# lucidrains/vit-pytorch

Hardware: AMD Instinct MI355X
Metric: images/sec (fwd+bwd) ViT-B/16 224^2 bf16 (higher is better)
Workload: dtype bf16

## Files before the change

### vit_pytorch_amd/csrc/gemm_bf16.hip

```cpp
#include "common.h"
#include <atomic>
#include "gemm_nt_plan.h"
#include <stdlib.h>

namespace {

constexpr int BM = 128, BN = 128;
constexpr int NT_BK = 32;
constexpr int NT_TILE_BYTES = 128 * NT_BK * 2;
constexpr int NT_STAGE_BYTES = 2 * NT_TILE_BYTES;
constexpr int NXCD = 8;

__device__ __forceinline__ int xcd_swizzle(int b, int nwg) {
    const int q = nwg / NXCD, r = nwg % NXCD;
    const int xcd = b % NXCD, idx = b / NXCD;
    return (xcd < r ? xcd * (q + 1) : r * (q + 1) + (xcd - r) * q) + idx;
}

__device__ __forceinline__ void grouped_tile(int wg, int tiles_m, int tiles_n, int gn, int& tm, int& tn) {
    const int per_group = gn * tiles_m;
    const int g = wg / per_group;
    const int r = wg - g * per_group;
    const int rem = tiles_n - g * gn;
    const int w = rem < gn ? rem : gn;
    tm = r / w;
    tn = g * gn + (r - tm * w);
}

__device__ __forceinline__ int swz_f(int x) { return (0x1320 >> (4 * (x & 3))) & 3; }

template <int EPI>
__global__ __launch_bounds__(256) void gemm_nt_kernel(
    const __bf16* __restrict__ A, long long lda, const __bf16* __restrict__ W, long long ldw,
    void* __restrict__ Cv, long long ldc, int M, int N, int K,
    const __bf16* __restrict__ bias, const float* __restrict__ resid, __bf16* __restrict__ aux,
    int tiles_n, int nwg) {
    __shared__ __attribute__((aligned(16))) char lds[2 * NT_STAGE_BYTES];

    const int tid = threadIdx.x;
    const int lane = tid & 63;
    const int wave = tid >> 6;
    const int wm = wave >> 1, wn = wave & 1;
    const int wg = xcd_swizzle(blockIdx.x, nwg);
    const int tm = wg / tiles_n, tn = wg % tiles_n;
    const int m0 = tm * BM, n0 = tn * BN;

    const int srow = lane >> 2;
    const int spos = lane & 3;
    const int schunk = spos ^ swz_f(lane >> 4);
    const __bf16* a_src[2];
    const __bf16* w_src[2];
#pragma unroll
    for (int j = 0; j < 2; ++j) {
        const int rg = wave * 2 + j;
        int ar = m0 + rg * 16 + srow; ar = ar < M ? ar : M - 1;
        int wr = n0 + rg * 16 + srow; wr = wr < N ? wr : N - 1;
        a_src[j] = A + (long long)ar * lda + schunk * 8;
        w_src[j] = W + (long long)wr * ldw + schunk * 8;
    }
    auto stage = [&](int buf, int kt) {
        char* base = lds + buf * NT_STAGE_BYTES;
#pragma unroll
        for (int j = 0; j < 2; ++j) {
            const int rg = wave * 2 + j;
            __builtin_amdgcn_global_load_lds((const void __attribute__((address_space(1)))*)(a_src[j] + kt * NT_BK),
                                             (void __attribute__((address_space(3)))*)(base + rg * 1024), 16, 0, 0);
            __builtin_amdgcn_global_load_lds((const void __attribute__((address_space(1)))*)(w_src[j] + kt * NT_BK),
                                             (void __attribute__((address_space(3)))*)(base + NT_TILE_BYTES + rg * 1024), 16, 0, 0);
        }
    };

    const int fi = lane & 15, fg = lane >> 4;
    const int fpos = fg ^ swz_f(fi >> 2);
    const int a_off = (wm * 64 + fi) * 64 + fpos * 16;
    const int w_off = NT_TILE_BYTES + (wn * 64 + fi) * 64 + fpos * 16;

    f32x4 acc[4][4];
#pragma unroll
    for (int i = 0; i < 4; ++i)
#pragma unroll
        for (int j = 0; j < 4; ++j) acc[i][j] = f32x4{0.f, 0.f, 0.f, 0.f};

    const int nt = K / NT_BK;
    stage(0, 0);
    for (int t = 0; t < nt; ++t) {
        __syncthreads();
        if (t + 1 < nt) stage((t + 1) & 1, t + 1);
        const char* base = lds + (t & 1) * NT_STAGE_BYTES;
        bf16x8 xf[4], wf[4];
#pragma unroll
        for (int f = 0; f < 4; ++f) {
            xf[f] = *reinterpret_cast<const bf16x8*>(base + a_off + f * 1024);
            wf[f] = *reinterpret_cast<const bf16x8*>(base + w_off + f * 1024);
        }
#pragma unroll
        for (int fn = 0; fn < 4; ++fn)
#pragma unroll
            for (int fm = 0; fm < 4; ++fm)
                acc[fn][fm] = __builtin_amdgcn_mfma_f32_16x16x32_bf16(wf[fn], xf[fm], acc[fn][fm], 0, 0, 0);
    }

#pragma unroll
    for (int fm = 0; fm < 4; ++fm) {
        const int m = m0 + wm * 64 + fm * 16 + fi;
        if (m >= M) continue;
#pragma unroll
        for (int fn = 0; fn < 4; ++fn) {
            const int n = n0 + wn * 64 + fn * 16 + 4 * fg;
            if (n >= N) continue;
            f32x4 v = acc[fn][fm];
            const long long o = (long long)m * ldc + n;
            if constexpr (EPI == VITK_EPI_BIAS || EPI == VITK_EPI_BIAS_GELU) {
                v += load4<__bf16>(bias + n);
            }
            if constexpr (EPI == VITK_EPI_NONE || EPI == VITK_EPI_BIAS) {
                store4<__bf16>(reinterpret_cast<__bf16*>(Cv) + o, v);
            } else if constexpr (EPI == VITK_EPI_BIAS_GELU) {
                store4<__bf16>(aux + o, v);
                f32x4 gq;
#pragma unroll
                for (int e = 0; e < 4; ++e) gq[e] = gelu_erf(v[e]);
                store4<__bf16>(reinterpret_cast<__bf16*>(Cv) + o, gq);
            } else if constexpr (EPI == VITK_EPI_RESID) {
                if (bias) v += load4<__bf16>(bias + n);
                v += *reinterpret_cast<const f32x4*>(resid + o);
                *reinterpret_cast<f32x4*>(reinterpret_cast<float*>(Cv) + o) = v;
            } else if constexpr (EPI == VITK_EPI_GELU_BWD) {
                const f32x4 h = load4<__bf16>(aux + o);
#pragma unroll
                for (int e = 0; e < 4; ++e) v[e] *= gelu_erf_grad(h[e]);
                store4<__bf16>(reinterpret_cast<__bf16*>(Cv) + o, v);
            }
        }
    }
}

constexpr int TN_BKM = 32;
constexpr int TN_LD = 288;
constexpr int TN_TILE_BYTES = TN_BKM * TN_LD;
constexpr int TN_STAGE_BYTES = 2 * TN_TILE_BYTES;

__device__ __forceinline__ bf16x8 tr_frag(const char* tile, int off) {
    const s16x4 lo = __builtin_amdgcn_ds_read_tr16_b64_v4i16((s16x4 __attribute__((address_space(3)))*)(tile + off));
    const s16x4 hi = __builtin_amdgcn_ds_read_tr16_b64_v4i16((s16x4 __attribute__((address_space(3)))*)(tile + off + 16 * TN_LD));
    const s16x8 v = {lo[0], lo[1], lo[2], lo[3], hi[0], hi[1], hi[2], hi[3]};
    return __builtin_bit_cast(bf16x8, v);
}

__global__ __launch_bounds__(256) void gemm_tn_kernel(
    const __bf16* __restrict__ dY, long long ldy, const __bf16* __restrict__ X, long long ldx,
    float* __restrict__ ws, int M, int N, int K, int rows_per_split, int tiles_k, int nwg) {
    __shared__ __attribute__((aligned(16))) char lds[2 * TN_STAGE_BYTES];
    const int tid = threadIdx.x;
    const int lane = tid & 63;
    const int wave = tid >> 6;
    const int wn = wave >> 1, wk = wave & 1;
    const int lin = xcd_swizzle(blockIdx.x, (int)gridDim.x);
    const int split = lin / nwg;
    const int wg = lin % nwg;
    const int tn = wg / tiles_k, tk = wg % tiles_k;
    const int n0 = tn * BN, k0 = tk * BM;
    const int mbeg = split * rows_per_split;
    int mend = mbeg + rows_per_split; mend = mend < M ? mend : M;

    int srow[2], scol[2];
#pragma unroll
    for (int j = 0; j < 2; ++j) { const int c = tid + 256 * j; srow[j] = c >> 4; scol[j] = (c & 15) * 8; }
    const bf16x8 zero8 = {0, 0, 0, 0, 0, 0, 0, 0};
    bf16x8 ry[2], rx[2];
    auto gload = [&](int mb) {
#pragma unroll
        for (int j = 0; j < 2; ++j) {
            const int m = mb + srow[j];
            const bool mv = m < mend;
            ry[j] = (mv && n0 + scol[j] < N) ? *reinterpret_cast<const bf16x8*>(dY + (long long)m * ldy + n0 + scol[j]) : zero8;
            rx[j] = (mv && k0 + scol[j] < K) ? *reinterpret_cast<const bf16x8*>(X + (long long)m * ldx + k0 + scol[j]) : zero8;
        }
    };
    auto lstore = [&](int buf) {
        char* base = lds + buf * TN_STAGE_BYTES;
#pragma unroll
        for (int j = 0; j < 2; ++j) {
            *reinterpret_cast<bf16x8*>(base + srow[j] * TN_LD + scol[j] * 2) = ry[j];
            *reinterpret_cast<bf16x8*>(base + TN_TILE_BYTES + srow[j] * TN_LD + scol[j] * 2) = rx[j];
        }
    };

    const int fi = lane & 15, fg = lane >> 4;
    const int tr_off = (4 * fg + (fi >> 2)) * TN_LD + (fi & 3) * 8;
    const int y_off = tr_off + wn * 128;
    const int x_off = TN_TILE_BYTES + tr_off + wk * 128;

    f32x4 acc[4][4];
#pragma unroll
    for (int i = 0; i < 4; ++i)
#pragma unroll
        for (int j = 0; j < 4; ++j) acc[i][j] = f32x4{0.f, 0.f, 0.f, 0.f};

    const int nsteps = (mend - mbeg + TN_BKM - 1) / TN_BKM;
    if (nsteps > 0) {
        gload(mbeg);
        lstore(0);
        __syncthreads();
        for (int t = 0; t < nsteps; ++t) {
            if (t + 1 < nsteps) gload(mbeg + (t + 1) * TN_BKM);
            const char* base = lds + (t & 1) * TN_STAGE_BYTES;
            bf16x8 yf[4], xf[4];
#pragma unroll
            for (int f = 0; f < 4; ++f) {
                yf[f] = tr_frag(base, y_off + f * 32);
                xf[f] = tr_frag(base, x_off + f * 32);
            }
#pragma unroll
            for (int fn = 0; fn < 4; ++fn)
#pragma unroll
                for (int fk = 0; fk < 4; ++fk)
                    acc[fn][fk] = __builtin_amdgcn_mfma_f32_16x16x32_bf16(yf[fn], xf[fk], acc[fn][fk], 0, 0, 0);
            if (t + 1 < nsteps) lstore((t + 1) & 1);
            __syncthreads();
        }
    }
    float* out = ws + (long long)split * N * K;
#pragma unroll
    for (int fn = 0; fn < 4; ++fn)
#pragma unroll
        for (int r = 0; r < 4; ++r) {
            const int n = n0 + wn * 64 + fn * 16 + 4 * fg + r;
            if (n >= N) continue;
#pragma unroll
            for (int fk = 0; fk < 4; ++fk) {
                const int k = k0 + wk * 64 + fk * 16 + fi;
                if (k < K) out[(long long)n * K + k] = acc[fn][fk][r];
            }
        }
}

template <typename OT>
__global__ __launch_bounds__(256) void tn_reduce_kernel(const float* __restrict__ ws, int splits, long long NK, int K,
                                                         OT* __restrict__ out, long long ldo, int accumulate, long long slab_stride) {
    const long long i4 = ((long long)blockIdx.x * 256 + threadIdx.x) * 4;
    if (i4 >= NK) return;
    f32x4 s = *reinterpret_cast<const f32x4*>(ws + i4);
    for (int p = 1; p < splits; ++p) s += *reinterpret_cast<const f32x4*>(ws + (long long)p * slab_stride + i4);
    const long long n = i4 / K, k = i4 % K;
    OT* o = out + n * ldo + k;
    if (accumulate) s += load4<OT>(o);
    store4<OT>(o, s);
}


constexpr int L_BN = 256, L_BK = 64;

constexpr int P_BK = 32, P_STAGES = 4;
constexpr int P_TILE_BYTES = 256 * P_BK * 2;
constexpr int P_STAGE_BYTES = 2 * P_TILE_BYTES;
constexpr int P_LDS_BYTES = P_STAGES * P_STAGE_BYTES;

#define PP_BARRIER() do { __builtin_amdgcn_sched_barrier(0); __builtin_amdgcn_s_barrier(); __builtin_amdgcn_sched_barrier(0); } while (0)

template <int EPI, int FM, int EB = 2, int F8 = 0>
__global__ __launch_bounds__(512) void gemm_nt256pp_kernel(
    const void* __restrict__ Av, long long lda, const void* __restrict__ Wv, long long ldw,
    void* __restrict__ Cv, long long ldc, int M, int N, int K,
    const __bf16* __restrict__ bias, const float* __restrict__ resid, __bf16* __restrict__ aux,
    int tiles_n, int nwg, int group_n, float* __restrict__ csum, float alpha, unsigned drop_t, unsigned drop_seed, float inv_keep,
    const float* __restrict__ alpha_a, const float* __restrict__ alpha_w, F8Out f8) {
    const char* A = reinterpret_cast<const char*>(Av);
    const char* W = reinterpret_cast<const char*>(Wv);
    extern __shared__ __attribute__((aligned(16))) char lds[];
    const int tid = threadIdx.x;
    const int lane = tid & 63;
    const int wave = __builtin_amdgcn_readfirstlane(tid >> 6);
    const int wm = wave >> 2, wn = wave & 3;
    const bool grp_b = wave >= 4;
    const int wg = xcd_swizzle(blockIdx.x, nwg);
    int tm, tn;
    grouped_tile(wg, nwg / tiles_n, tiles_n, group_n, tm, tn);
    constexpr int WROWS = 16 * FM;
    const int m0 = tm * (2 * WROWS), n0 = tn * L_BN;

    const int srow = lane >> 2, spos = lane & 3;
    const int schunk = spos ^ swz_f(lane >> 4);
    const char* a_src[2];
    const char* w_src[2];
#pragma unroll
    for (int j = 0; j < 2; ++j) {
        int ar = m0 + (wave * 2 + j) * 16 + srow; ar = ar < M ? ar : M - 1;
        int wr = n0 + (wave * 2 + j) * 16 + srow; wr = wr < N ? wr : N - 1;
        a_src[j] = A + (long long)ar * lda * EB + schunk * 16;
        w_src[j] = W + (long long)wr * ldw * EB + schunk * 16;
    }
    auto stage_a = [&](int kt) {
        char* base = lds + (kt & 3) * P_STAGE_BYTES + wave * 2048;
#pragma unroll
        for (int j = 0; j < 2; ++j)
            __builtin_amdgcn_global_load_lds((const void __attribute__((address_space(1)))*)(a_src[j] + kt * 64),
                                             (void __attribute__((address_space(3)))*)(base + j * 1024), 16, 0, 0);
    };
    auto stage_w = [&](int kt) {
        char* base = lds + (kt & 3) * P_STAGE_BYTES + P_TILE_BYTES + wave * 2048;
#pragma unroll
        for (int j = 0; j < 2; ++j)
            __builtin_amdgcn_global_load_lds((const void __attribute__((address_space(1)))*)(w_src[j] + kt * 64),
                                             (void __attribute__((address_space(3)))*)(base + j * 1024), 16, 0, 0);
    };
    auto mma = [&](const bf16x8& wfr, const bf16x8& xfr, f32x4 c) -> f32x4 {
        if constexpr (EB == 2) {
            return __builtin_amdgcn_mfma_f32_16x16x32_bf16(wfr, xfr, c, 0, 0, 0);
        } else {
            typedef long l2 __attribute__((ext_vector_type(2)));
            const l2 w2 = __builtin_bit_cast(l2, wfr), x2 = __builtin_bit_cast(l2, xfr);
            if constexpr (F8 & 1) {
                c = __builtin_amdgcn_mfma_f32_16x16x32_fp8_bf8(w2[0], x2[0], c, 0, 0, 0);
                return __builtin_amdgcn_mfma_f32_16x16x32_fp8_bf8(w2[1], x2[1], c, 0, 0, 0);
            } else {
                c = __builtin_amdgcn_mfma_f32_16x16x32_fp8_fp8(w2[0], x2[0], c, 0, 0, 0);
                return __builtin_amdgcn_mfma_f32_16x16x32_fp8_fp8(w2[1], x2[1], c, 0, 0, 0);
            }
        }
    };
    auto mma128 = [&](const bf16x8& w0, const bf16x8& w1, const bf16x8& x0, const bf16x8& x1, f32x4 c) -> f32x4 {
        typedef int i4 __attribute__((ext_vector_type(4)));
        typedef int i8 __attribute__((ext_vector_type(8)));
        const i8 a = __builtin_shufflevector(__builtin_bit_cast(i4, w0), __builtin_bit_cast(i4, w1), 0, 1, 2, 3, 4, 5, 6, 7);
        const i8 b = __builtin_shufflevector(__builtin_bit_cast(i4, x0), __builtin_bit_cast(i4, x1), 0, 1, 2, 3, 4, 5, 6, 7);
        return __builtin_amdgcn_mfma_scale_f32_16x16x128_f8f6f4(a, b, c, 0 , (F8 & 1) ? 1 : 0 , 0, 0, 0, 0);
    };
    static_assert(F8 == 0 || EB == 1, "the e5m2 / K = 128 flavours are fp8 flavours");

    const int fi = lane & 15, fg = lane >> 4;
    const int fpos = fg ^ swz_f(fi >> 2);
    const int a_off = (wm * WROWS + fi) * 64 + fpos * 16;
    const int w_off = P_TILE_BYTES + (wn * 64 + fi) * 64 + fpos * 16;

    f32x4 acc[4][FM];
#pragma unroll
    for (int i = 0; i < 4; ++i)
#pragma unroll
        for (int j = 0; j < FM; ++j) acc[i][j] = f32x4{0.f, 0.f, 0.f, 0.f};

    const int nt = K * EB / 64;
    stage_a(0); stage_w(0);
    if (nt > 1) { stage_a(1); stage_w(1); }
    if (nt > 2) { stage_a(2); stage_w(2); }
    if (nt > 2) asm volatile("s_waitcnt vmcnt(8)" ::: "memory");
    else if (nt > 1) asm volatile("s_waitcnt vmcnt(4)" ::: "memory");
    else asm volatile("s_waitcnt vmcnt(0)" ::: "memory");
    PP_BARRIER();
    if (grp_b) PP_BARRIER();

    if constexpr ((F8 & 2) != 0) {
        bf16x8 hw[4], hx[FM];
        for (int j = 0; j < nt; ++j) {
            const char* base = lds + (j & 3) * P_STAGE_BYTES;
            const bool more = j + 3 < nt;
            const bool odd = (j & 1) != 0;
            bf16x8 wf[4], xf[4];
#pragma unroll
            for (int f = 0; f < 4; ++f) wf[f] = *reinterpret_cast<const bf16x8*>(base + w_off + f * 1024);
#pragma unroll
            for (int f = 0; f < 4; ++f) xf[f] = *reinterpret_cast<const bf16x8*>(base + a_off + f * 1024);
            if (more) stage_a(j + 3);
            asm volatile("s_waitcnt lgkmcnt(0)" ::: "memory");
            PP_BARRIER();
            if (odd) {
                __builtin_amdgcn_s_setprio(1);
#pragma unroll
                for (int fn = 0; fn < 4; ++fn)
#pragma unroll
                    for (int f = 0; f < 4; ++f)
                        acc[fn][f] = mma128(hw[fn], wf[fn], hx[f], xf[f], acc[fn][f]);
                __builtin_amdgcn_s_setprio(0);
            } else {
#pragma unroll
                for (int f = 0; f < 4; ++f) { hw[f] = wf[f]; hx[f] = xf[f]; }
            }
            PP_BARRIER();
#pragma unroll
            for (int f = 0; f < FM - 4; ++f) xf[f] = *reinterpret_cast<const bf16x8*>(base + a_off + (4 + f) * 1024);
            if (more) stage_w(j + 3);
            if (more) asm volatile("s_waitcnt vmcnt(8)" ::: "memory");
            else if (j + 2 < nt) asm volatile("s_waitcnt vmcnt(4)" ::: "memory");
            else asm volatile("s_waitcnt vmcnt(0)" ::: "memory");
            asm volatile("s_waitcnt lgkmcnt(0)" ::: "memory");
            PP_BARRIER();
            if (odd) {
                __builtin_amdgcn_s_setprio(1);
#pragma unroll
                for (int fn = 0; fn < 4; ++fn)
#pragma unroll
                    for (int f = 0; f < FM - 4; ++f)
                        acc[fn][4 + f] = mma128(hw[fn], wf[fn], hx[4 + f], xf[f], acc[fn][4 + f]);
                __builtin_amdgcn_s_setprio(0);
            } else {
#pragma unroll
                for (int f = 0; f < FM - 4; ++f) hx[4 + f] = xf[f];
            }
            PP_BARRIER();
        }
    } else
    for (int j = 0; j < nt; ++j) {
        const char* base = lds + (j & 3) * P_STAGE_BYTES;
        const bool more = j + 3 < nt;
        bf16x8 wf[4], xf[4];
#pragma unroll
        for (int f = 0; f < 4; ++f) wf[f] = *reinterpret_cast<const bf16x8*>(base + w_off + f * 1024);
#pragma unroll
        for (int f = 0; f < 4; ++f) xf[f] = *reinterpret_cast<const bf16x8*>(base + a_off + f * 1024);
        if (more) stage_a(j + 3);
        asm volatile("s_waitcnt lgkmcnt(0)" ::: "memory");
        PP_BARRIER();
        __builtin_amdgcn_s_setprio(1);
#pragma unroll
        for (int fn = 0; fn < 4; ++fn)
#pragma unroll
            for (int f = 0; f < 4; ++f)
                acc[fn][f] = mma(wf[fn], xf[f], acc[fn][f]);
        __builtin_amdgcn_s_setprio(0);
        PP_BARRIER();
#pragma unroll
        for (int f = 0; f < FM - 4; ++f) xf[f] = *reinterpret_cast<const bf16x8*>(base + a_off + (4 + f) * 1024);
        if (more) stage_w(j + 3);
        if (more) asm volatile("s_waitcnt vmcnt(8)" ::: "memory");
        else if (j + 2 < nt) asm volatile("s_waitcnt vmcnt(4)" ::: "memory");
        else asm volatile("s_waitcnt vmcnt(0)" ::: "memory");
        asm volatile("s_waitcnt lgkmcnt(0)" ::: "memory");
        PP_BARRIER();
        __builtin_amdgcn_s_setprio(1);
#pragma unroll
        for (int fn = 0; fn < 4; ++fn)
#pragma unroll
            for (int f = 0; f < FM - 4; ++f)
                acc[fn][4 + f] = mma(wf[fn], xf[f], acc[fn][4 + f]);
        __builtin_amdgcn_s_setprio(0);
        PP_BARRIER();
    }
    if (!grp_b) PP_BARRIER();
    if constexpr (EB == 1) {
        const float al = alpha * (alpha_a ? *alpha_a : 1.0f) * (alpha_w ? *alpha_w : 1.0f);
#pragma unroll
        for (int i = 0; i < 4; ++i)
#pragma unroll
            for (int jj = 0; jj < FM; ++jj) acc[i][jj] *= al;
    }

    __syncthreads();
    char* ep = lds + wave * 16384;
    const int mrow0 = m0 + wm * WROWS, ncol0 = n0 + wn * 64;
    if constexpr (EPI == VITK_EPI_RESID) {
        const int rr = lane >> 4, rc = lane & 15;
        const int ncol = ncol0 + rc * 4;
        f32x4 b4 = {0.f, 0.f, 0.f, 0.f};
        if (bias && ncol < N) b4 = load4<__bf16>(bias + ncol);
        constexpr int NF0 = 4, NF1 = FM - 4;
        f32x4 rpre[2][16];
        auto fetch_resid = [&](int hh) {
            const int nf = hh ? NF1 : NF0;
#pragma unroll
            for (int j = 0; j < 16; ++j) {
                const int m = mrow0 + hh * 64 + j * 4 + rr;
                rpre[hh][j] = f32x4{0.f, 0.f, 0.f, 0.f};
                if (j < nf * 4 && m < M && ncol < N) rpre[hh][j] = *reinterpret_cast<const f32x4*>(resid + (long long)m * ldc + ncol);
            }
        };
        fetch_resid(0);
#pragma unroll
        for (int hh = 0; hh < 2; ++hh) {
            const int nf = hh ? NF1 : NF0;
#pragma unroll
            for (int f4 = 0; f4 < 4; ++f4) {
                if (f4 < nf) {
                    const int row = f4 * 16 + fi;
#pragma unroll
                    for (int fn = 0; fn < 4; ++fn) {
                        const int c16 = fn * 4 + fg;
                        *reinterpret_cast<f32x4*>(ep + row * 256 + ((c16 ^ (row & 15)) * 16)) = acc[fn][hh * 4 + f4 < FM ? hh * 4 + f4 : 0];
                    }
                }
            }
            if (hh == 0) fetch_resid(1);
#pragma unroll
            for (int j = 0; j < 16; ++j) {
                if (j < nf * 4) {
                    const int row = j * 4 + rr;
                    f32x4 v = *reinterpret_cast<const f32x4*>(ep + row * 256 + ((rc ^ (row & 15)) * 16));
                    const int m = mrow0 + hh * 64 + row;
                    if (m < M && ncol < N) {
                        v += b4;
                        if (drop_t) {
                            const unsigned hrow = drop_row((unsigned)m, drop_seed);
#pragma unroll
                            for (int e = 0; e < 4; ++e) v[e] = drop_keep(hrow, (unsigned)(ncol + e), drop_t) ? v[e] * inv_keep : 0.f;
                        }
                        v += rpre[hh][j];
                        *reinterpret_cast<f32x4*>(reinterpret_cast<float*>(Cv) + (long long)m * ldc + ncol) = v;
                    }
                }
            }
        }
    } else {
        f32x4 b4[4];
#pragma unroll
        for (int fn = 0; fn < 4; ++fn) {
            b4[fn] = f32x4{0.f, 0.f, 0.f, 0.f};
            if constexpr (EPI == VITK_EPI_BIAS || EPI == VITK_EPI_BIAS_GELU) {
                const int n = ncol0 + fn * 16 + 4 * fg;
                if (n < N) b4[fn] = load4<__bf16>(bias + n);
            }
        }
        const int rr = lane >> 3, rc = lane & 7;
        const int ncol = ncol0 + rc * 8;
        bf16x8 hpre[2 * FM];
        if constexpr (EPI == VITK_EPI_GELU_BWD) {
#pragma unroll
            for (int j = 0; j < 2 * FM; ++j) {
                const int m = mrow0 + j * 8 + rr;
                hpre[j] = bf16x8{0, 0, 0, 0, 0, 0, 0, 0};
                if (m < M && ncol < N) hpre[j] = *reinterpret_cast<const bf16x8*>(aux + (long long)m * ldc + ncol);
            }
        }
#pragma unroll
        for (int fm = 0; fm < FM; ++fm) {
            const int row = fm * 16 + fi;
#pragma unroll
            for (int fn = 0; fn < 4; ++fn) {
                const int c16 = fn * 2 + (fg >> 1);
                const f32x4 v = acc[fn][fm] + b4[fn];
                const bf16x4 pk = {(__bf16)v[0], (__bf16)v[1], (__bf16)v[2], (__bf16)v[3]};
                *reinterpret_cast<bf16x4*>(ep + row * 128 + ((c16 ^ (row & 7)) * 16) + (((fg & 1) ^ ((row >> 3) & 1)) * 8)) = pk;
            }
        }
        float cs[8] = {0.f, 0.f, 0.f, 0.f, 0.f, 0.f, 0.f, 0.f};
        float f8max = 0.f;
#pragma unroll
        for (int j = 0; j < 2 * FM; ++j) {
            const int row = j * 8 + rr;
            bf16x8 v = *reinterpret_cast<const bf16x8*>(ep + row * 128 + ((rc ^ (row & 7)) * 16));
            if (j & 1) v = bf16x8{v[4], v[5], v[6], v[7], v[0], v[1], v[2], v[3]};
            const int m = mrow0 + row;
            if (m < M && ncol < N) {
                const long long o = (long long)m * ldc + ncol;
                if constexpr (EPI == VITK_EPI_NONE || EPI == VITK_EPI_BIAS) {
                    *reinterpret_cast<bf16x8*>(reinterpret_cast<__bf16*>(Cv) + o) = v;
                } else if constexpr (EPI == VITK_EPI_BIAS_GELU) {
                    *reinterpret_cast<bf16x8*>(aux + o) = v;
                    bf16x8 g8;
#pragma unroll
                    for (int e = 0; e < 8; e += 2) {
                        const f32x2 g2 = gelu_fast2(f32x2{(float)v[e], (float)v[e + 1]});
                        g8[e] = (__bf16)g2[0]; g8[e + 1] = (__bf16)g2[1];
                    }
                    if (drop_t) {
                        const unsigned hrow = drop_row((unsigned)m, drop_seed);
#pragma unroll
                        for (int e = 0; e < 8; ++e)
                            g8[e] = drop_keep(hrow, (unsigned)(ncol + e), drop_t) ? (__bf16)((float)g8[e] * inv_keep) : (__bf16)0.f;
                    }
                    if (Cv) *reinterpret_cast<bf16x8*>(reinterpret_cast<__bf16*>(Cv) + o) = g8;
                    if (f8.p || f8.amax) {
                        const f32x4 lo = {(float)g8[0], (float)g8[1], (float)g8[2], (float)g8[3]};
                        const f32x4 hi = {(float)g8[4], (float)g8[5], (float)g8[6], (float)g8[7]};
                        if (f8.p) {
                            const float sc8 = *f8.scale;
                            unsigned* d8 = reinterpret_cast<unsigned*>(f8.p + o);
                            d8[0] = pack_fp8x4(lo, sc8); d8[1] = pack_fp8x4(hi, sc8);
                        }
                        if (f8.amax) f8max = fmaxf(f8max, fmaxf(absmax4(lo), absmax4(hi)));
                    }
                } else if constexpr (EPI == VITK_EPI_GELU_BWD) {
                    const bf16x8 h8 = hpre[j];
                    bf16x8 g8;
                    float km[8];
                    if (drop_t) {
                        const unsigned hrow = drop_row((unsigned)m, drop_seed);
#pragma unroll
                        for (int e = 0; e < 8; ++e) km[e] = drop_keep(hrow, (unsigned)(ncol + e), drop_t) ? inv_keep : 0.f;
                    } else {
#pragma unroll
                        for (int e = 0; e < 8; ++e) km[e] = 1.f;
                    }
#pragma unroll
                    for (int e = 0; e < 8; e += 2) {
                        const f32x2 g2 = f32x2{(float)v[e], (float)v[e + 1]} * gelu_grad_fast2(f32x2{(float)h8[e], (float)h8[e + 1]}) * f32x2{km[e], km[e + 1]};
                        g8[e] = (__bf16)g2[0]; g8[e + 1] = (__bf16)g2[1];
                        cs[e] += (float)g8[e]; cs[e + 1] += (float)g8[e + 1];
                    }
                    *reinterpret_cast<bf16x8*>(reinterpret_cast<__bf16*>(Cv) + o) = g8;
                    if (f8.p || f8.amax) {
                        const f32x4 lo = {(float)g8[0], (float)g8[1], (float)g8[2], (float)g8[3]};
                        const f32x4 hi = {(float)g8[4], (float)g8[5], (float)g8[6], (float)g8[7]};
                        if (f8.p) {
                            const float sc8 = *f8.scale;
                            unsigned* d8 = reinterpret_cast<unsigned*>(f8.p + o);
                            d8[0] = pack_bf8x4(lo, sc8); d8[1] = pack_bf8x4(hi, sc8);
                        }
                        if (f8.amax) f8max = fmaxf(f8max, fmaxf(absmax4(lo), absmax4(hi)));
                    }
                }
            }
        }
        if constexpr (EPI == VITK_EPI_BIAS_GELU || EPI == VITK_EPI_GELU_BWD) {
            if (f8.amax) {
                f8max = wave_max(f8max);
                __syncthreads();
                float* red = reinterpret_cast<float*>(lds);
                if (lane == 0) red[wave] = f8max;
                __syncthreads();
                if (tid == 0) {
                    float m = red[0];
#pragma unroll
                    for (int k = 1; k < 8; ++k) m = fmaxf(m, red[k]);
                    atomicMax(f8.amax + (blockIdx.x & 63), __builtin_bit_cast(unsigned, m));
                }
            }
        }
        if constexpr (EPI == VITK_EPI_GELU_BWD) {
            if (csum) {
                float* cp = reinterpret_cast<float*>(ep);
#pragma unroll
                for (int e = 0; e < 8; ++e) cp[rr * 64 + rc * 8 + e] = cs[e];
                float t = 0.f;
#pragma unroll
                for (int r8 = 0; r8 < 8; ++r8) t += cp[r8 * 64 + lane];
                const int n = ncol0 + lane;
                if (n < N) csum[(long long)(tm * 2 + wm) * N + n] = t;
            }
        }
    }
}

template <typename Kern>
int set_max_lds(Kern kernel, int bytes) {
    return (int)hipFuncSetAttribute(reinterpret_cast<const void*>(kernel), hipFuncAttributeMaxDynamicSharedMemorySize, bytes);
}

}

namespace {
struct NtPlan { bool large; int fm; };
NtPlan nt_plan(int64_t M, int64_t N, int64_t K, int64_t ldc, const void* aux) {
    NtPlan pl;
    pl.large = (K % L_BK == 0) && M >= 1024 && N >= 256 && (N % 8 == 0) && (ldc % 8 == 0) && (!aux || aligned16(aux));
    pl.fm = 8;
    if (pl.large) {
        const long long tn_ = (N + L_BN - 1) / L_BN;
        const long long t8 = ((M + 255) / 256) * tn_, t7 = ((M + 223) / 224) * tn_;
        const long long cost8 = ((t8 + 255) / 256) * 8, cost7 = ((t7 + 255) / 256) * 7;
        if (cost7 * 10 <= cost8 * 9) pl.fm = 7;
    }
    return pl;
}
int gemm_nt_impl(const void* A, int64_t lda, const void* W, int64_t ldw, void* C, int64_t ldc, int64_t M, int64_t N, int64_t K,
                 int epilogue, const void* bias, const float* resid, void* aux, float* csum, void* stream, bool fp8 = false,
                 float alpha = 1.0f, float drop_p = 0.f, unsigned drop_seed = 0u, const float* alpha_a = nullptr,
                 const float* alpha_w = nullptr, F8Out f8 = F8Out{nullptr, nullptr, nullptr}, int f8kind = 0);
}

extern "C" int vitk_gemm_nt_bf16(const void* A, int64_t lda, const void* W, int64_t ldw, void* C, int64_t ldc, int64_t M,
                                 int64_t N, int64_t K, int epilogue, const void* bias, const float* resid, void* aux,
                                 void* stream) {
    return gemm_nt_impl(A, lda, W, ldw, C, ldc, M, N, K, epilogue, bias, resid, aux, nullptr, stream);
}

extern "C" int vitk_gemm_nt_bf16_drop(const void* A, int64_t lda, const void* W, int64_t ldw, void* C, int64_t ldc, int64_t M, int64_t N,
                                      int64_t K, int epilogue, const void* bias, const float* resid, void* aux, float* colsum_partials,
                                      float drop_p, uint32_t drop_seed, void* stream) {
    if (colsum_partials && (epilogue != VITK_EPI_GELU_BWD || vitk_gemm_nt_colsum_rows(M, N, K, ldc) == 0))
        VITK_FAIL(VITK_E_SHAPE, "gemm_nt_bf16_drop: column sums come with the GELU_BWD epilogue of the 256-row kernel only");
    return gemm_nt_impl(A, lda, W, ldw, C, ldc, M, N, K, epilogue, bias, resid, aux, colsum_partials, stream, false, 1.0f, drop_p, drop_seed);
}

extern "C" int vitk_gemm_nt_fp8_ex(const void* A, int64_t lda, int a_is_fp8, const void* W, int64_t ldw, void* C, int64_t ldc, int64_t M,
                                   int64_t N, int64_t K, int epilogue, const void* bias, const float* resid, void* aux, float alpha,
                                   const float* alpha_a, const float* alpha_w, void* c8, const float* c8_scale, uint32_t* c8_amax64,
                                   void* stream) {
    const F8Out f8{(unsigned char*)c8, c8_scale, (unsigned*)c8_amax64};
    return gemm_nt_impl(A, lda, W, ldw, C, ldc, M, N, K, epilogue, bias, resid, aux, nullptr, stream, a_is_fp8 != 0, alpha, 0.f, 0u,
                        alpha_a, alpha_w, f8);
}

extern "C" int vitk_gemm_nt_fp8(const void* A, int64_t lda, const void* W, int64_t ldw, void* C, int64_t ldc, int64_t M, int64_t N,
                               int64_t K, int epilogue, const void* bias, const float* resid, void* aux, float alpha, void* stream) {
    return gemm_nt_impl(A, lda, W, ldw, C, ldc, M, N, K, epilogue, bias, resid, aux, nullptr, stream, true, alpha);
}

extern "C" int vitk_gemm_nt_fp8_v2(const void* A, int64_t lda, int a_kind, const void* W, int64_t ldw, void* C, int64_t ldc, int64_t M,
                                   int64_t N, int64_t K, int epilogue, const void* bias, const float* resid, void* aux,
                                   float* colsum_partials, float alpha, const float* alpha_a, const float* alpha_w, void* c8,
                                   const float* c8_scale, uint32_t* c8_amax64, int flags, void* stream) {
    if (a_kind < 0 || a_kind > 2) VITK_FAIL(VITK_E_ARG, "gemm_nt_fp8_v2: a_kind is 0 (16-bit), 1 (e4m3) or 2 (e5m2), got %d", a_kind);
    if (flags & ~1) VITK_FAIL(VITK_E_ARG, "gemm_nt_fp8_v2: unknown flags 0x%x", (unsigned)flags);
    if (a_kind == 0 && (flags & 1)) VITK_FAIL(VITK_E_ARG, "gemm_nt_fp8_v2: the K = 128 instruction takes 1-byte operands");
    if ((flags & 1) && (K % 128)) VITK_FAIL(VITK_E_SHAPE, "gemm_nt_fp8_v2: the K = 128 flavour needs K %% 128 == 0 (K = %lld)", (long long)K);
    if (colsum_partials && (epilogue != VITK_EPI_GELU_BWD || vitk_gemm_nt_fp8_colsum_rows(M, N, K, ldc) == 0))
        VITK_FAIL(VITK_E_SHAPE, "gemm_nt_fp8_v2: column sums come with the GELU_BWD epilogue of the 256-row kernel only");
    const F8Out f8{(unsigned char*)c8, c8_scale, (unsigned*)c8_amax64};
    return gemm_nt_impl(A, lda, W, ldw, C, ldc, M, N, K, epilogue, bias, resid, aux, colsum_partials, stream, a_kind != 0, alpha, 0.f, 0u,
                        alpha_a, alpha_w, f8, (a_kind == 2 ? 1 : 0) | ((flags & 1) ? 2 : 0));
}

extern "C" int64_t vitk_gemm_nt_fp8_colsum_rows(int64_t M, int64_t N, int64_t K, int64_t ldc) {
    if (M <= 0 || N <= 0 || K <= 0 || (K % 64)) return 0;
    const NtPlan pl = nt_plan(M, N, K, ldc, nullptr);
    if (!pl.large) return 0;
    return 2 * ((M + 32 * pl.fm - 1) / (32 * pl.fm));
}

static int64_t nt_persist_colsum_rows(const NtpPlan& q, int64_t M, int64_t N, int64_t K, int64_t ldc);
extern "C" int64_t vitk_gemm_nt_colsum_rows(int64_t M, int64_t N, int64_t K, int64_t ldc) {
    if (M <= 0 || N <= 0 || K <= 0) return 0;
    const NtpPlan q = ntp_plan(M, N, K, ldc, nullptr);
    if (q.ok) return nt_persist_colsum_rows(q, M, N, K, ldc);
    const NtPlan pl = nt_plan(M, N, K, ldc, nullptr);
    if (!pl.large) return 0;
    return 2 * ((M + 32 * pl.fm - 1) / (32 * pl.fm));
}

extern "C" int vitk_gemm_nt_plan(int64_t M, int64_t N, int64_t K, int64_t ldc, int32_t* out5) {
    if (!out5) VITK_FAIL(VITK_E_ARG, "gemm_nt_plan: null output");
    for (int i = 0; i < 5; ++i) out5[i] = 0;
    if (M <= 0 || N <= 0 || K <= 0) return 0;
    const NtpPlan q = ntp_plan(M, N, K, ldc, nullptr);
    if (q.ok) { out5[0] = 1; out5[1] = q.tm_main; out5[2] = q.tail_tm; out5[3] = q.grid; out5[4] = q.tiles_n; }
    return 0;
}

extern "C" int vitk_gemm_nt_bf16_gelu_bwd_colsum(const void* A, int64_t lda, const void* W, int64_t ldw, void* C, int64_t ldc,
                                                 int64_t M, int64_t N, int64_t K, void* aux, float* colsum_partials, void* stream) {
    if (!colsum_partials) VITK_FAIL(VITK_E_ARG, "gemm_nt_bf16_gelu_bwd_colsum: null partials");
    if (vitk_gemm_nt_colsum_rows(M, N, K, ldc) == 0 || (aux && !aligned16(aux)))
        VITK_FAIL(VITK_E_SHAPE, "gemm_nt_bf16_gelu_bwd_colsum: shape not served by the 256-row kernel (vitk_gemm_nt_colsum_rows() == 0)");
    return gemm_nt_impl(A, lda, W, ldw, C, ldc, M, N, K, VITK_EPI_GELU_BWD, nullptr, nullptr, aux, colsum_partials, stream);
}

extern "C" int vitk_gemm_nt_bf16_mul_aux_colsum(const void* A, int64_t lda, const void* W, int64_t ldw, void* C, int64_t ldc, int64_t M,
                                                int64_t N, int64_t K, const void* aux, float* colsum_partials, void* stream) {
    if (!aux) VITK_FAIL(VITK_E_ARG, "gemm_nt_bf16_mul_aux_colsum: null pointer");
    if (colsum_partials && vitk_gemm_nt_colsum_rows(M, N, K, ldc) == 0)
        VITK_FAIL(VITK_E_SHAPE, "gemm_nt_bf16_mul_aux_colsum: shape not served by the persistent kernel (vitk_gemm_nt_colsum_rows() == 0)");
    return gemm_nt_impl(A, lda, W, ldw, C, ldc, M, N, K, VITK_EPI_MUL_AUX, nullptr, nullptr, const_cast<void*>(aux), colsum_partials, stream);
}

extern "C" int vitk_gemm_nt_bf16_mul_aux8_colsum(const void* A, int64_t lda, const void* W, int64_t ldw, void* C, int64_t ldc, int64_t M,
                                                 int64_t N, int64_t K, const void* aux8, float* colsum_partials, void* stream) {
    if (!aux8) VITK_FAIL(VITK_E_ARG, "gemm_nt_bf16_mul_aux8_colsum: null pointer");
    if (colsum_partials && vitk_gemm_nt_colsum_rows(M, N, K, ldc) == 0)
        VITK_FAIL(VITK_E_SHAPE, "gemm_nt_bf16_mul_aux8_colsum: shape not served by the persistent kernel (vitk_gemm_nt_colsum_rows() == 0)");
    return gemm_nt_impl(A, lda, W, ldw, C, ldc, M, N, K, VITK_EPI_MUL_AUX8, nullptr, nullptr, const_cast<void*>(aux8), colsum_partials, stream);
}

constexpr unsigned NTW_EPIS = 0xffu;
static int ntw_tiles_m(const NtpPlan& q, int64_t M, int64_t N, int64_t K, int epilogue, int grid = 0) {
    if (epilogue == VITK_EPI_BIAS_GELU_DG8) epilogue = VITK_EPI_BIAS_GELU_DG;
    if (epilogue == VITK_EPI_MUL_AUX8) epilogue = VITK_EPI_MUL_AUX;
    const char* e = vitk_switch("VITK_NT_W128");
    const unsigned mask = e ? (unsigned)strtoul(e, nullptr, 0) : NTW_EPIS;
    if (!q.ok || !((mask >> epilogue) & 1u) || !gemm_ntw_serves(M, N, K)) return 0;
    return gemm_ntw_split(M, N, K, grid > 0 ? grid : q.grid);
}
static int64_t nt_persist_colsum_rows(const NtpPlan& q, int64_t M, int64_t N, int64_t K, int64_t ldc) {
    const int tmw = ntw_tiles_m(q, M, N, K, VITK_EPI_MUL_AUX);
    if (tmw == 0) return ntp_colsum_rows(q);
    const int64_t rest = M - 256LL * tmw;
    return 2LL * tmw + (rest > 0 ? ntp_colsum_rows(ntp_plan(rest, N, K, ldc, nullptr)) : 0);
}
static int nt_persist_dispatch(const NtpPlan& q, const void* A, int64_t lda, const void* W, int64_t ldw, void* C, int64_t ldc, int64_t M, int64_t N,
                               int64_t K, int epilogue, const void* bias, const float* resid, void* aux, float* csum, unsigned drop_t,
                               unsigned drop_seed, float inv_keep, void* stream) {
    const int reserve = vitk_get_cu_reserve();
    int grid_w = q.grid - (reserve + 7) / 8 * 8;
    if (grid_w < q.grid / 4) grid_w = q.grid / 4 / 8 * 8;
    const int tmw = ntw_tiles_m(q, M, N, K, epilogue == VITK_EPI_GELU_BWD ? VITK_EPI_MUL_AUX : epilogue, csum ? 0 : grid_w);
    const int64_t asz = (epilogue == VITK_EPI_BIAS_GELU_DG8 || epilogue == VITK_EPI_MUL_AUX8) ? 1 : 2;
    if (tmw == 0 || (drop_t && !(epilogue == VITK_EPI_GELU_BWD && csum)))
        return gemm_ntp_launch(q, A, lda, W, ldw, C, ldc, M, N, K, epilogue, bias, resid, aux, csum, drop_t, drop_seed, inv_keep, stream);
    const int64_t rows_w = 256LL * tmw, rest = M - rows_w;
    int rc;
    if (drop_t) {
        NtpPlan q1 = q;
        q1.tm_main = tmw; q1.tail_tm = 0; q1.n_main = tmw * q1.tiles_n; q1.n_tail = 0;
        rc = gemm_ntp_launch(q1, A, lda, W, ldw, C, ldc, rows_w, N, K, epilogue, bias, resid, aux, csum, drop_t, drop_seed, inv_keep, stream);
    } else {
        if (256LL * (lda > ldw ? lda : ldw) * 2 + K * 2 >= (1LL << 31)) VITK_FAIL(VITK_E_SHAPE, "gemm_nt_bf16: row stride too large (lda %lld, ldw %lld)", (long long)lda, (long long)ldw);
        rc = gemm_ntw_launch(tmw, grid_w, A, lda, W, ldw, C, ldc, N, K, epilogue, bias, resid, aux, csum, 0, 0, stream);
    }
    if (rc != 0 || rest <= 0) return rc;
    const NtpPlan q2 = ntp_plan(rest, N, K, ldc, aux);
    if (!q2.ok) VITK_FAIL(VITK_E_SHAPE, "gemm_nt_bf16: internal: the row split left %lld rows the persistent kernel does not take", (long long)rest);
    const int64_t csz = epilogue == VITK_EPI_RESID ? 4 : 2;
    return gemm_ntp_launch(q2, (const char*)A + rows_w * lda * 2, lda, W, ldw, (char*)C + rows_w * ldc * csz, ldc, rest, N, K, epilogue, bias,
                           resid ? (const float*)((const char*)resid + rows_w * ldc * csz) : nullptr, aux ? (char*)aux + rows_w * ldc * asz : nullptr,
                           csum ? csum + 2LL * tmw * N : nullptr, drop_t, drop_seed, inv_keep, stream, (unsigned)rows_w);
}

namespace {
int gemm_nt_impl(const void* A, int64_t lda, const void* W, int64_t ldw, void* C, int64_t ldc, int64_t M, int64_t N, int64_t K,
                 int epilogue, const void* bias, const float* resid, void* aux, float* csum, void* stream, bool fp8, float alpha,
                 float drop_p, unsigned drop_seed, const float* alpha_a, const float* alpha_w, F8Out f8, int f8kind) {
    if (f8kind && !fp8) VITK_FAIL(VITK_E_ARG, "gemm_nt: e5m2 / K = 128 flavours need 1-byte operands");
    if ((f8kind & 1) && epilogue != VITK_EPI_NONE && epilogue != VITK_EPI_GELU_BWD)
        VITK_FAIL(VITK_E_ARG, "gemm_nt_fp8: e5m2 operands (gradients) come with the NONE and GELU_BWD epilogues only (got %d)", epilogue);
    if ((f8.p || f8.amax) && epilogue != VITK_EPI_BIAS_GELU && epilogue != VITK_EPI_GELU_BWD)
        VITK_FAIL(VITK_E_ARG, "gemm_nt: the fp8 side output exists in the BIAS_GELU (e4m3) and GELU_BWD (e5m2) epilogues only");
    if (f8.p && (!f8.scale || (ldc & 7))) VITK_FAIL(VITK_E_ARG, "gemm_nt: fp8 side output needs a scale and ldc %% 8 == 0");
    const bool c_optional = fp8 && epilogue == VITK_EPI_BIAS_GELU && f8.p;
    if (!A || !W || (!C && !c_optional)) VITK_FAIL(VITK_E_ARG, "gemm_nt_bf16: null pointer");
    if (!(drop_p >= 0.f && drop_p < 1.f)) VITK_FAIL(VITK_E_ARG, "gemm_nt_bf16: dropout p must be in [0, 1) (got %g)", (double)drop_p);
    const unsigned drop_t = drop_thresh(drop_p);
    const float inv_keep = 1.0f / (1.0f - drop_p);
    if (fp8 && ((lda & 15) || (ldw & 15) || (K % 64)))
        VITK_FAIL(VITK_E_ALIGN, "gemm_nt_fp8: K %% 64 == 0 and lda, ldw %% 16 == 0 required");
    if (M <= 0 || N <= 0 || K <= 0 || (K % NT_BK) || (N & 3) || M > (1 << 30) || N > (1 << 30))
        VITK_FAIL(VITK_E_SHAPE, "gemm_nt_bf16: need K %% 32 == 0 and N %% 4 == 0 (M=%lld N=%lld K=%lld)", (long long)M, (long long)N, (long long)K);
    if ((lda & 7) || (ldw & 7) || (ldc & 3) || !aligned16(A) || !aligned16(W) || !aligned16(C) || (bias && !aligned8(bias)) ||
        (resid && !aligned16(resid)) || (aux && !aligned8(aux)))
        VITK_FAIL(VITK_E_ALIGN, "gemm_nt_bf16: lda/ldw %% 8, ldc %% 4 and 16-byte aligned pointers required");
    if (ldw == 0 && (fp8 || f8.p || f8.amax)) VITK_FAIL(VITK_E_ARG, "gemm_nt: a K-blocked W (ldw == 0) goes with 16-bit operands only");
    if (!fp8 && !f8.p && !f8.amax) {
        const NtpPlan q = ntp_plan(M, N, K, ldc, aux);
        const unsigned epis = vitk_exp("VITK_NTP_EPIS") ? (unsigned)atoi(vitk_exp("VITK_NTP_EPIS")) : 0x1fu;
        const bool dg_out = epilogue == VITK_EPI_BIAS_GELU_DG || epilogue == VITK_EPI_BIAS_GELU_DG8;
        if (dg_out || epilogue == VITK_EPI_MUL_AUX || epilogue == VITK_EPI_MUL_AUX8) {
            if (!q.ok) VITK_FAIL(VITK_E_SHAPE, "gemm_nt_bf16: EPI_BIAS_GELU_DG(8) / EPI_MUL_AUX(8) are served by the persistent kernel only (vitk_gemm_nt_plan() says which shapes)");
            if (!aux || drop_t || (dg_out && !bias)) VITK_FAIL(VITK_E_ARG, "gemm_nt_bf16: EPI_BIAS_GELU_DG(8) needs bias and aux, EPI_MUL_AUX(8) aux; no fused dropout");
            return nt_persist_dispatch(q, A, lda, W, ldw, C, ldc, M, N, K, epilogue, bias, resid, aux, csum, 0u, 0u, 1.0f, stream);
        }
        if (epilogue == VITK_EPI_RESID16) {
            if (!q.ok) VITK_FAIL(VITK_E_SHAPE, "gemm_nt_bf16: EPI_RESID16 is served by the persistent kernel only (vitk_gemm_nt_plan() says which shapes)");
            if (!resid || !aligned8(resid) || drop_t) VITK_FAIL(VITK_E_ARG, "gemm_nt_bf16: EPI_RESID16 needs an 8-byte aligned 16-bit resid and no dropout");
            return nt_persist_dispatch(q, A, lda, W, ldw, C, ldc, M, N, K, epilogue, bias, resid, aux, csum, 0u, 0u, 1.0f, stream);
        }
        if (q.ok && epilogue >= 0 && epilogue <= 4 && (((epis >> epilogue) & 1u) || epilogue == VITK_EPI_GELU_BWD)) {
            switch (epilogue) {
                case VITK_EPI_NONE: break;
                case VITK_EPI_BIAS: if (!bias) VITK_FAIL(VITK_E_ARG, "gemm_nt_bf16: EPI_BIAS needs bias"); break;
                case VITK_EPI_BIAS_GELU: if (!bias || !aux) VITK_FAIL(VITK_E_ARG, "gemm_nt_bf16: EPI_BIAS_GELU needs bias and aux"); break;
                case VITK_EPI_RESID: if (!resid) VITK_FAIL(VITK_E_ARG, "gemm_nt_bf16: EPI_RESID needs resid"); break;
                case VITK_EPI_GELU_BWD: if (!aux) VITK_FAIL(VITK_E_ARG, "gemm_nt_bf16: EPI_GELU_BWD needs aux"); break;
                default: VITK_FAIL(VITK_E_ARG, "gemm_nt_bf16: bad epilogue %d", epilogue);
            }
            if (drop_t && epilogue != VITK_EPI_RESID && epilogue != VITK_EPI_BIAS_GELU && epilogue != VITK_EPI_GELU_BWD)
                VITK_FAIL(VITK_E_SHAPE, "gemm_nt_bf16: fused dropout exists for the RESID / BIAS_GELU / GELU_BWD epilogues only");
            return nt_persist_dispatch(q, A, lda, W, ldw, C, ldc, M, N, K, epilogue, bias, resid, aux, csum, drop_t, drop_seed, inv_keep, stream);
        }
    }
    if (ldw == 0) VITK_FAIL(VITK_E_SHAPE, "gemm_nt_bf16: a K-blocked W (ldw == 0, vitk_pack_w_nt) is read by the persistent kernel only (vitk_gemm_nt_plan() says which shapes it serves)");
    const NtPlan pl = nt_plan(M, N, K, ldc, aux);
    const bool large = pl.large;
    const int fm = pl.fm;
    if (fp8 && !large) VITK_FAIL(VITK_E_SHAPE, "gemm_nt_fp8: served by the 256-row kernel only (M >= 1024, N >= 256, N %% 8 == 0)");
    if ((f8.p || f8.amax) && !large) VITK_FAIL(VITK_E_SHAPE, "gemm_nt: the fp8 side output is served by the 256-row kernel only");
    if (drop_t && (!large || (epilogue != VITK_EPI_RESID && epilogue != VITK_EPI_BIAS_GELU && epilogue != VITK_EPI_GELU_BWD)))
        VITK_FAIL(VITK_E_SHAPE, "gemm_nt_bf16: fused dropout exists in the 256-row kernel for the RESID / BIAS_GELU / GELU_BWD epilogues only");
    const int tbm = large ? 32 * fm : BM, tbn = large ? L_BN : BN;
    const int tiles_m = (int)((M + tbm - 1) / tbm), tiles_n = (int)((N + tbn - 1) / tbn);
    const long long nwg = (long long)tiles_m * tiles_n;
    if (nwg > 0x7fffffffLL) VITK_FAIL(VITK_E_SHAPE, "gemm_nt_bf16: grid too large");
    hipStream_t st = (hipStream_t)stream;
    int group_n = tiles_n;
    if (large && tiles_n > 8) group_n = (tiles_n + (tiles_n + 5) / 6 - 1) / ((tiles_n + 5) / 6);
    if (vitk_exp("VITK_GROUP_N")) group_n = atoi(vitk_exp("VITK_GROUP_N")) > 0 ? atoi(vitk_exp("VITK_GROUP_N")) : tiles_n;
    if (group_n > tiles_n) group_n = tiles_n;
#define NT_LAUNCH_F8(E, F, FK) do { \
            static const int rc8__ = set_max_lds(gemm_nt256pp_kernel<E, F, 1, FK>, P_LDS_BYTES); \
            if (rc8__ != 0) VITK_FAIL(rc8__, "gemm_nt_fp8: cannot enable %d B of LDS", P_LDS_BYTES); \
            hipLaunchKernelGGL((gemm_nt256pp_kernel<E, F, 1, FK>), dim3((unsigned)nwg), dim3(512), P_LDS_BYTES, st, A, (long long)lda, \
                W, (long long)ldw, C, (long long)ldc, (int)M, (int)N, (int)K, (const __bf16*)bias, resid, (__bf16*)aux, tiles_n, (int)nwg, group_n, csum, alpha, drop_t, drop_seed, inv_keep, alpha_a, alpha_w, f8); \
        } while (0)
#define NT_LAUNCH_PP(E, F) do { \
        if (fp8) { \
            if constexpr (E == VITK_EPI_NONE || E == VITK_EPI_GELU_BWD) { \
                if (f8kind == 1) NT_LAUNCH_F8(E, F, 1); else if (f8kind == 3) NT_LAUNCH_F8(E, F, 3); \
                else if (f8kind == 2) NT_LAUNCH_F8(E, F, 2); else NT_LAUNCH_F8(E, F, 0); \
            } else { \
                if (f8kind == 2) NT_LAUNCH_F8(E, F, 2); else NT_LAUNCH_F8(E, F, 0); \
            } \
        } else { \
            static const int rc__ = set_max_lds(gemm_nt256pp_kernel<E, F, 2>, P_LDS_BYTES); \
            if (rc__ != 0) VITK_FAIL(rc__, "gemm_nt_bf16: cannot enable %d B of LDS", P_LDS_BYTES); \
            hipLaunchKernelGGL((gemm_nt256pp_kernel<E, F, 2>), dim3((unsigned)nwg), dim3(512), P_LDS_BYTES, st, A, (long long)lda, \
                W, (long long)ldw, C, (long long)ldc, (int)M, (int)N, (int)K, (const __bf16*)bias, resid, (__bf16*)aux, tiles_n, (int)nwg, group_n, csum, 1.0f, drop_t, drop_seed, inv_keep, nullptr, nullptr, f8); \
        } \
    } while (0)
#define NT_LAUNCH(E) do { \
    if (large && fm == 7) NT_LAUNCH_PP(E, 7); \
    else if (large) NT_LAUNCH_PP(E, 8); \
    else { \
        hipLaunchKernelGGL((gemm_nt_kernel<E>), dim3((unsigned)nwg), dim3(256), 0, st, (const __bf16*)A, (long long)lda, \
            (const __bf16*)W, (long long)ldw, C, (long long)ldc, (int)M, (int)N, (int)K, (const __bf16*)bias, resid, (__bf16*)aux, tiles_n, (int)nwg); \
    } } while (0)
    switch (epilogue) {
        case VITK_EPI_NONE: NT_LAUNCH(VITK_EPI_NONE); break;
        case VITK_EPI_BIAS:
            if (!bias) VITK_FAIL(VITK_E_ARG, "gemm_nt_bf16: EPI_BIAS needs bias");
            NT_LAUNCH(VITK_EPI_BIAS); break;
        case VITK_EPI_BIAS_GELU:
            if (!bias || !aux) VITK_FAIL(VITK_E_ARG, "gemm_nt_bf16: EPI_BIAS_GELU needs bias and aux");
            NT_LAUNCH(VITK_EPI_BIAS_GELU); break;
        case VITK_EPI_RESID:
            if (!resid) VITK_FAIL(VITK_E_ARG, "gemm_nt_bf16: EPI_RESID needs resid");
            NT_LAUNCH(VITK_EPI_RESID); break;
        case VITK_EPI_GELU_BWD:
            if (!aux) VITK_FAIL(VITK_E_ARG, "gemm_nt_bf16: EPI_GELU_BWD needs aux");
            NT_LAUNCH(VITK_EPI_GELU_BWD); break;
        default: VITK_FAIL(VITK_E_ARG, "gemm_nt_bf16: bad epilogue %d", epilogue);
    }
#undef NT_LAUNCH
#undef NT_LAUNCH_PP
#undef NT_LAUNCH_F8
    VITK_CHECK_LAUNCH("gemm_nt_bf16");
    return 0;
}
}


bool gemm_tn_w128_serves(int64_t M, int64_t N, int64_t K, int64_t ldy, int64_t ldx, int64_t splits);
int gemm_tn_w128_launch2(const void* dY0, int64_t ldy0, const void* X0, int64_t ldx0, int64_t N0, int64_t K0, const void* dY1, int64_t ldy1,
                         const void* X1, int64_t ldx1, int64_t N1, int64_t K1, float* ws, int64_t M, int64_t splits, void* stream);
int gemm_tn_w128_launch(const void* dY, int64_t ldy, const void* X, int64_t ldx, float* ws, int64_t M, int64_t N, int64_t K,
                        int64_t splits, void* stream);

static bool tn_large(int64_t M, int64_t N, int64_t K) { return M >= 4096 && N >= 256 && K >= 256; }

static std::atomic<int> g_cu_reserve{0};
extern "C" int vitk_set_cu_reserve(int cus) {
    if (cus < 0 || cus > 192) VITK_FAIL(VITK_E_ARG, "set_cu_reserve: 0 .. 192 (got %d)", cus);
    g_cu_reserve.store(cus);
    return 0;
}
extern "C" int vitk_get_cu_reserve(void) { return g_cu_reserve.load(); }

int64_t tn_pick_splits(int64_t tiles, int64_t M, int cus, long long slab_elems, double us_per_row, int64_t min_rows) {
    const int64_t max_by_rows = (M + min_rows - 1) / min_rows;
    int64_t best = 1;
    double best_c = 1e30;
    for (int64_t s = 1; s <= 64 && s <= max_by_rows; ++s) {
        const int64_t rounds = (tiles * s + cus - 1) / cus;
        const double job = (double)M / (double)s * us_per_row + 8.0;
        const double fold = (double)s * (double)slab_elems * 8.0 / 5.0e6;
        const double c = (double)rounds * job + fold;
        if (c < best_c - 1e-9) { best_c = c; best = s; }
    }
    return best;
}

extern "C" int64_t vitk_gemm_tn_splits(int64_t M, int64_t N, int64_t K) {
    if (tn_large(M, N, K)) {
        const int64_t tiles = ((N + 255) / 256) * ((K + 255) / 256);
        return tn_pick_splits(tiles, M, 256 - g_cu_reserve.load(), (long long)N * K, 0.024, 512);
    }
    const int64_t tiles = ((N + BN - 1) / BN) * ((K + BM - 1) / BM);
    int64_t s = (768 + tiles - 1) / tiles;
    const int64_t max_by_rows = (M + 255) / 256;
    if (s > max_by_rows) s = max_by_rows;
    if (s > 64) s = 64;
    if (s < 1) s = 1;
    return s;
}

extern "C" int vitk_gemm_tn_bf16(const void* dY, int64_t ldy, const void* X, int64_t ldx, void* dW, int odt, int64_t ldo,
                                 int accumulate, int64_t M, int64_t N, int64_t K, float* ws, int64_t splits, void* stream) {
    if (!dY || !X || !dW || !ws) VITK_FAIL(VITK_E_ARG, "gemm_tn_bf16: null pointer");
    if (M <= 0 || N <= 0 || K <= 0 || (N & 7) || (K & 7) || splits < 1 || splits > 65535 || M > (1 << 30))
        VITK_FAIL(VITK_E_SHAPE, "gemm_tn_bf16: need N %% 8 == 0, K %% 8 == 0 (M=%lld N=%lld K=%lld)", (long long)M, (long long)N, (long long)K);
    if ((ldy & 7) || (ldx & 7) || (ldo & 3) || !aligned16(dY) || !aligned16(X) || !aligned16(dW) || !aligned16(ws))
        VITK_FAIL(VITK_E_ALIGN, "gemm_tn_bf16: ldy/ldx %% 8, ldo %% 4 and 16-byte aligned pointers required");
    hipStream_t st = (hipStream_t)stream;
    if (tn_large(M, N, K) && gemm_tn_w128_serves(M, N, K, ldy, ldx, splits)) {
        const int rc = gemm_tn_w128_launch(dY, ldy, X, ldx, ws, M, N, K, splits, stream);
        if (rc != 0) return rc;
    } else {
        const int tiles_n = (int)((N + BN - 1) / BN), tiles_k = (int)((K + BM - 1) / BM);
        const int nwg = tiles_n * tiles_k;
        long long rps = (M + splits - 1) / splits;
        rps = (rps + TN_BKM - 1) / TN_BKM * TN_BKM;
        hipLaunchKernelGGL(gemm_tn_kernel, dim3((unsigned)(nwg * splits)), dim3(256), 0, st, (const __bf16*)dY, (long long)ldy,
                           (const __bf16*)X, (long long)ldx, ws, (int)M, (int)N, (int)K, (int)rps, tiles_k, nwg);
    }
    VITK_CHECK_LAUNCH("gemm_tn_bf16");
    const long long NK = (long long)N * K;
    const unsigned blocks = (unsigned)((NK / 4 + 255) / 256);
    VITK_DISPATCH_DT(odt, OT, hipLaunchKernelGGL((tn_reduce_kernel<OT>), dim3(blocks), dim3(256), 0, st, ws, (int)splits, NK, (int)K,
                                                  (OT*)dW, (long long)ldo, accumulate, NK));
    VITK_CHECK_LAUNCH("gemm_tn_reduce");
    return 0;
}

extern "C" int64_t vitk_gemm_tn_pair_splits(int64_t M, int64_t N0, int64_t K0, int64_t N1, int64_t K1) {
    if (!tn_large(M, N0, K0) || !tn_large(M, N1, K1) || (N0 & 7) || (K0 & 7) || (N1 & 7) || (K1 & 7)) return 0;
    if (vitk_switch("VITK_TN_PAIR") && atoi(vitk_switch("VITK_TN_PAIR")) == 0) return 0;
    const int64_t tiles = ((N0 + 255) / 256) * ((K0 + 255) / 256) + ((N1 + 255) / 256) * ((K1 + 255) / 256);
    const int64_t s = tn_pick_splits(tiles, M, 256 - g_cu_reserve.load(), (long long)N0 * K0 + (long long)N1 * K1, 0.024, 512);
    const int64_t ldmax = (N0 > K0 ? N0 : K0) > (N1 > K1 ? N1 : K1) ? (N0 > K0 ? N0 : K0) : (N1 > K1 ? N1 : K1);
    if (!gemm_tn_w128_serves(M, N0, K0, ldmax, ldmax, s)) return 0;
    return s;
}

extern "C" int vitk_gemm_tn_bf16_pair(const void* dY0, int64_t ldy0, const void* X0, int64_t ldx0, void* dW0, int64_t ldo0, int accumulate0,
                                      int64_t N0, int64_t K0, const void* dY1, int64_t ldy1, const void* X1, int64_t ldx1, void* dW1,
                                      int64_t ldo1, int accumulate1, int64_t N1, int64_t K1, int odt, int64_t M, float* ws, int64_t splits,
                                      void* stream) {
    if (!dY0 || !X0 || !dW0 || !dY1 || !X1 || !dW1 || !ws) VITK_FAIL(VITK_E_ARG, "gemm_tn_bf16_pair: null pointer");
    if (splits < 1 || splits != vitk_gemm_tn_pair_splits(M, N0, K0, N1, K1))
        VITK_FAIL(VITK_E_SHAPE, "gemm_tn_bf16_pair: splits must be vitk_gemm_tn_pair_splits(M, N0, K0, N1, K1) (0 = pair not served)");
    if ((ldy0 & 7) || (ldx0 & 7) || (ldo0 & 3) || (ldy1 & 7) || (ldx1 & 7) || (ldo1 & 3) || !aligned16(dY0) || !aligned16(X0) || !aligned16(dW0) ||
        !aligned16(dY1) || !aligned16(X1) || !aligned16(dW1) || !aligned16(ws))
        VITK_FAIL(VITK_E_ALIGN, "gemm_tn_bf16_pair: ldy/ldx %% 8, ldo %% 4 and 16-byte aligned pointers required");
    if (!gemm_tn_w128_serves(M, N0, K0, ldy0 > ldy1 ? ldy0 : ldy1, ldx0 > ldx1 ? ldx0 : ldx1, splits))
        VITK_FAIL(VITK_E_SHAPE, "gemm_tn_bf16_pair: row strides beyond the kernel's 32-bit offsets");
    const int rc = gemm_tn_w128_launch2(dY0, ldy0, X0, ldx0, N0, K0, dY1, ldy1, X1, ldx1, N1, K1, ws, M, splits, stream);
    if (rc != 0) return rc;
    hipStream_t st = (hipStream_t)stream;
    const long long NK0 = (long long)N0 * K0, NK1 = (long long)N1 * K1, stride = NK0 + NK1;
    VITK_DISPATCH_DT(odt, OT, hipLaunchKernelGGL((tn_reduce_kernel<OT>), dim3((unsigned)((NK0 / 4 + 255) / 256)), dim3(256), 0, st, ws, (int)splits, NK0,
                                                  (int)K0, (OT*)dW0, (long long)ldo0, accumulate0, stride));
    VITK_DISPATCH_DT(odt, OT, hipLaunchKernelGGL((tn_reduce_kernel<OT>), dim3((unsigned)((NK1 / 4 + 255) / 256)), dim3(256), 0, st, ws + NK0, (int)splits, NK1,
                                                  (int)K1, (OT*)dW1, (long long)ldo1, accumulate1, stride));
    VITK_CHECK_LAUNCH("gemm_tn_pair_reduce");
    return 0;
}
```

### vit_pytorch_amd/csrc/gemm_nt_persist.hip

```cpp
#include "common.h"
#include "gemm_nt_plan.h"
#include "gemm_nt_epi.h"
#include <stdlib.h>
#include <atomic>
#include <mutex>
#include <unordered_map>
#include <type_traits>

namespace {

constexpr int Q_TILE_BYTES = 256 * 64;
constexpr int Q_STAGE_BYTES = 2 * Q_TILE_BYTES;
constexpr int Q_LDS_BYTES = 4 * Q_STAGE_BYTES;
constexpr int Q_LDS_MAX = Q_LDS_BYTES + 32768;
constexpr int Q_TK_LINE = 32;
constexpr int Q_TK_SLOT_WORDS = 32 * Q_TK_LINE;

#define QQ_BARRIER() do { __builtin_amdgcn_sched_barrier(0); __builtin_amdgcn_s_barrier(); __builtin_amdgcn_sched_barrier(0); } while (0)

__device__ __forceinline__ int q_swz(int x) { return (0x1320 >> (4 * (x & 3))) & 3; }

__device__ __forceinline__ void q_grouped_tile(int t, int tiles_m, int tiles_n, int gn, int& tm, int& tn) {
    const int per_group = gn * tiles_m;
    const int g = t / per_group;
    const int r = t - g * per_group;
    const int rem = tiles_n - g * gn;
    const int w = rem < gn ? rem : gn;
    tm = r / w;
    tn = g * gn + (r - tm * w);
}

struct NtpArgs {
    const char* A; long long lda;
    const char* W; long long ldw;
    void* C; long long ldc;
    int M, N, K;
    const __bf16* bias; const float* resid; __bf16* aux; float* csum;
    int tiles_n, group_n, tm_main, tail_tm, n_main, n_tail, nt;
    unsigned drop_t, drop_seed; float inv_keep;
    unsigned drop_m0;
    int tail_first;
    unsigned* tickets;
    int dbg;
    long long* stamps;
};

__device__ __forceinline__ unsigned q_satomic_add(unsigned* p, unsigned v) {
    asm volatile("s_atomic_add %0, %1, 0x0 glc\n\ts_waitcnt lgkmcnt(0)" : "+s"(v) : "s"(p) : "memory");
    return v;
}

template <int N_> __device__ __forceinline__ void q_wait_vm() {
    if constexpr (N_ == 0) asm volatile("s_waitcnt vmcnt(0)" ::: "memory");
    else if constexpr (N_ == 4) asm volatile("s_waitcnt vmcnt(4)" ::: "memory");
    else if constexpr (N_ == 8) asm volatile("s_waitcnt vmcnt(8)" ::: "memory");
    else if constexpr (N_ == 12) asm volatile("s_waitcnt vmcnt(12)" ::: "memory");
    else static_assert(N_ < 0, "unsupported vmcnt");
}


template <int EPI, bool DYN>
__global__ __launch_bounds__(512) void gemm_ntp_kernel(const NtpArgs p) {
    extern __shared__ __attribute__((aligned(16))) char lds[];
    constexpr bool F32OUT = (EPI == VITK_EPI_RESID);
    const int tid = threadIdx.x;
    const int lane = tid & 63;
    const int wave = __builtin_amdgcn_readfirstlane(tid >> 6);
    const int wm = wave >> 2, wn = wave & 3;

    const int xcd = blockIdx.x & 7, l0 = blockIdx.x >> 3, L = gridDim.x >> 3;
    auto q_geom = [&](int q, int& ms_, int& cm_, int& ts_, int& ct_) {
        ms_ = (int)(((long long)q * p.n_main) >> 3); cm_ = (int)(((long long)(q + 1) * p.n_main) >> 3) - ms_;
        ts_ = (int)(((long long)q * p.n_tail) >> 3); ct_ = (int)(((long long)(q + 1) * p.n_tail) >> 3) - ts_;
    };
    int ms, cm, ts, ct;
    q_geom(xcd, ms, cm, ts, ct);
    const int count = cm + ct;
    constexpr bool dyn = DYN;
    if (!dyn && l0 >= count) return;
    const int ntiles = dyn ? 0 : (count - l0 + L - 1) / L;
    const int total_steps = ntiles * p.nt;
    const int c_first = p.tail_first ? ct : cm;
    int* const tk_slots = reinterpret_cast<int*>(lds + Q_LDS_BYTES + p.tiles_n * 512);
    int my_q = xcd;
    bool dry = false;
    auto pop_ticket = [&]() -> int {
        if (dry) return -1;
        int q = my_q;
        for (int tries = 0; tries < 8; ++tries) {
            int a, b, c, d;
            q_geom(q, a, b, c, d);
            const unsigned v = q_satomic_add(p.tickets + q * Q_TK_LINE, 1u);
            if ((int)v < b + d) { my_q = q; return (q << 24) | (int)v; }
            q = (q + 1) & 7;
        }
        dry = true;
        return -1;
    };
    auto leave = [&]() {
        if (wave == 0) {
            const unsigned per_xcd = (gridDim.x >> 3) + (((int)gridDim.x & 7) > xcd ? 1u : 0u);
            if (q_satomic_add(p.tickets + (8 + xcd) * Q_TK_LINE, 1u) == per_xcd - 1) {
                if (q_satomic_add(p.tickets + 16 * Q_TK_LINE, 1u) == 7u && lane < 17) p.tickets[lane * Q_TK_LINE] = 0;
            }
        }
    };

    auto decode = [&](int tk, int& m0, int& half, int& n0, int& mt) {
        int qms = ms, qcm = cm, qts = ts, qct = ct, idx = tk;
        if (dyn) { q_geom(tk >> 24, qms, qcm, qts, qct); idx = tk & 0xffffff; }
        int tm, tn;
        bool is_tail; int k;
        if (p.tail_first == 2) {
            const int h1 = (qct + 1) >> 1;
            if (idx < h1) { is_tail = true; k = idx; }
            else if (idx < h1 + qcm) { is_tail = false; k = idx - h1; }
            else { is_tail = true; k = idx - qcm; }
        } else {
            const int first = p.tail_first ? qct : qcm;
            const bool lead = idx < first;
            k = lead ? idx : idx - first;
            is_tail = lead == (p.tail_first != 0);
        }
        if (!is_tail) {
            q_grouped_tile(qms + k, p.tm_main, p.tiles_n, p.group_n, tm, tn);
            m0 = tm * 256; half = 0; mt = tm;
        } else {
            q_grouped_tile(qts + k, p.tail_tm, p.tiles_n, p.group_n, tm, tn);
            m0 = p.tm_main * 256 + tm * 128; half = 1; mt = p.tm_main + tm;
        }
        n0 = tn * 256;
    };
    (void)c_first;

    const int srow = lane >> 2, spos = lane & 3;
    const int schunk = spos ^ q_swz(lane >> 4);
    const char* a_src[2];
    const char* w_src[2];
    int p_idx = l0, p_kt = 0, p_g = 0;
    int p_n = 0;
    bool p_more = true;
    auto next_ticket = [&](int n) -> int {
        return __builtin_amdgcn_readfirstlane(*reinterpret_cast<volatile int*>(tk_slots + (n & 3)));
    };
    auto setup_src = [&](int idx) {
        int m0, half, n0, mt;
        decode(idx, m0, half, n0, mt);
        int mlast = m0 + (half ? 128 : 256);
        mlast = (mlast < p.M ? mlast : p.M) - 1;
#pragma unroll
        for (int j = 0; j < 2; ++j) {
            const int rg = wave * 2 + j;
            int ar = m0 + rg * 16 + srow; ar = ar < mlast ? ar : mlast;
            int wr = n0 + (rg >> 2) * 64 + 4 * srow + (rg & 3); wr = wr < p.N ? wr : p.N - 1;
            a_src[j] = p.A + (long long)ar * p.lda * 2 + schunk * 16;
            w_src[j] = p.W + (long long)wr * p.ldw * 2 + schunk * 16;
            if (p.ldw == 0) w_src[j] = p.W + (long long)(n0 >> 8) * p.nt * Q_TILE_BYTES + rg * 1024 + lane * 16;
        }
    };
    const int w_kstride = p.ldw == 0 ? Q_TILE_BYTES : 64;
    auto issue4 = [&]() __attribute__((always_inline)) {
        char* base = lds + (p_g & 3) * Q_STAGE_BYTES + wave * 2048;
#pragma unroll
        for (int j = 0; j < 2; ++j) {
            __builtin_amdgcn_global_load_lds((const void __attribute__((address_space(1)))*)(a_src[j] + p_kt * 64),
                                             (void __attribute__((address_space(3)))*)(base + j * 1024), 16, 0, 0);
            __builtin_amdgcn_global_load_lds((const void __attribute__((address_space(1)))*)(w_src[j] + p_kt * w_kstride),
                                             (void __attribute__((address_space(3)))*)(base + Q_TILE_BYTES + j * 1024), 16, 0, 0);
        }
    };
    auto advance4 = [&]() __attribute__((always_inline)) {
        ++p_g;
        if (!p_more) return;
        if (++p_kt == p.nt) {
            bool more;
            if (dyn) { p_idx = next_ticket(++p_n); more = p_idx >= 0; }
            else { p_idx += L; more = p_idx < count; }
            if (more) { p_kt = 0; setup_src(p_idx); }
            else { p_more = false; p_kt = p.nt - 1; }
        }
    };

    const char* bias_lds = lds + Q_LDS_BYTES;
    if constexpr (q_has_bias<EPI>()) {
        const int ncols = p.tiles_n * 256;
        for (int i = tid * 8; i < ncols; i += 512 * 8) {
            bf16x8 v = bf16x8{0, 0, 0, 0, 0, 0, 0, 0};
            if (p.bias && i < p.N) v = *reinterpret_cast<const bf16x8*>(p.bias + i);
            *reinterpret_cast<bf16x8*>(lds + Q_LDS_BYTES + i * 2) = v;
        }
        asm volatile("s_waitcnt lgkmcnt(0)" ::: "memory");
    }

    const int fi = lane & 15, fg = lane >> 4;
    const int fpos = fg ^ q_swz(fi >> 2);
    const int a_off8 = (wm * 128 + fi) * 64 + fpos * 16;
    const int a_off4 = (wm * 64 + fi) * 64 + fpos * 16;
    const int w_off = Q_TILE_BYTES + (wn * 64 + fi) * 64 + fpos * 16;

    int c_g = 0;
#ifdef Q_TIMELINE
    const bool tl_on = p.stamps && blockIdx.x == 137 && lane == 0 && wave == (p.dbg >> 8);
    unsigned long long* const tl = reinterpret_cast<unsigned long long*>(lds + Q_LDS_BYTES + 8192);
    int tl_n = 0;
#define Q_TL(tag) do { if (tl_on && tl_n < 2040) { tl[tl_n++] = ((unsigned long long)__builtin_readcyclecounter() << 4) | (unsigned)(tag); } } while (0)
#else
#define Q_TL(tag) do { } while (0)
#endif
    auto run_tile = [&](auto fmw_c, int m0, int n0, int mt) {
        constexpr int FMW = decltype(fmw_c)::value;
        const int a_off = FMW == 8 ? a_off8 : a_off4;
        f32x4 acc[4][FMW];
#pragma unroll
        for (int i = 0; i < 4; ++i)
#pragma unroll
            for (int j = 0; j < FMW; ++j) acc[i][j] = f32x4{0.f, 0.f, 0.f, 0.f};

        {
            bf16x8 f0w[4], f0x[4], f1w[4], f1x[4], xg[4];
            {
                const char* base = lds + (c_g & 3) * Q_STAGE_BYTES;
#pragma unroll
                for (int f = 0; f < 4; ++f) f0w[f] = *reinterpret_cast<const bf16x8*>(base + w_off + f * 1024);
#pragma unroll
                for (int f = 0; f < 4; ++f) f0x[f] = *reinterpret_cast<const bf16x8*>(base + a_off + f * 1024);
                asm volatile("s_waitcnt lgkmcnt(0)" ::: "memory");
                __builtin_amdgcn_sched_barrier(0);
            }
            auto kstep = [&](bf16x8 (&wf)[4], bf16x8 (&xf)[4], bf16x8 (&wn_)[4], bf16x8 (&xn_)[4]) __attribute__((always_inline)) {
                Q_TL(1);
                const char* base = lds + (c_g & 3) * Q_STAGE_BYTES;
                const char* nbase = lds + ((c_g + 1) & 3) * Q_STAGE_BYTES;
                if constexpr (FMW == 8) {
#pragma unroll
                    for (int f = 0; f < 4; ++f) xg[f] = *reinterpret_cast<const bf16x8*>(base + a_off + (4 + f) * 1024);
#pragma unroll
                    for (int fn = 0; fn < 4; ++fn)
#pragma unroll
                        for (int f = 0; f < 4; ++f)
                            acc[fn][f] = __builtin_amdgcn_mfma_f32_16x16x32_bf16(xf[f], wf[fn], acc[fn][f], 0, 0, 0);
#pragma unroll
                    for (int i = 0; i < 4; ++i) { __builtin_amdgcn_sched_group_barrier(0x008, 4, 0); __builtin_amdgcn_sched_group_barrier(0x100, 1, 0); }
                    __builtin_amdgcn_sched_barrier(0);
                    asm volatile("s_waitcnt lgkmcnt(0)" ::: "memory");
                    q_wait_vm<8>();
                    QQ_BARRIER();
#pragma unroll
                    for (int f = 0; f < 4; ++f) wn_[f] = *reinterpret_cast<const bf16x8*>(nbase + w_off + f * 1024);
#pragma unroll
                    for (int f = 0; f < 4; ++f) xn_[f] = *reinterpret_cast<const bf16x8*>(nbase + a_off + f * 1024);
                    issue4();
#pragma unroll
                    for (int fn = 0; fn < 4; ++fn)
#pragma unroll
                        for (int f = 0; f < 4; ++f)
                            acc[fn][4 + f] = __builtin_amdgcn_mfma_f32_16x16x32_bf16(xg[f], wf[fn], acc[fn][4 + f], 0, 0, 0);
                } else {
                    q_wait_vm<8>();
                    QQ_BARRIER();
#pragma unroll
                    for (int f = 0; f < 4; ++f) wn_[f] = *reinterpret_cast<const bf16x8*>(nbase + w_off + f * 1024);
#pragma unroll
                    for (int f = 0; f < 4; ++f) xn_[f] = *reinterpret_cast<const bf16x8*>(nbase + a_off + f * 1024);
                    issue4();
#pragma unroll
                    for (int fn = 0; fn < 4; ++fn)
#pragma unroll
                        for (int f = 0; f < 4; ++f)
                            acc[fn][f] = __builtin_amdgcn_mfma_f32_16x16x32_bf16(xf[f], wf[fn], acc[fn][f], 0, 0, 0);
                }
#pragma unroll
                for (int i = 0; i < 8; ++i) {
                    __builtin_amdgcn_sched_group_barrier(0x008, 1, 0);
                    __builtin_amdgcn_sched_group_barrier(0x100, 1, 0);
                    __builtin_amdgcn_sched_group_barrier(0x008, 1, 0);
                    if (i & 1) __builtin_amdgcn_sched_group_barrier(0x020, 1, 0);
                }
                __builtin_amdgcn_sched_barrier(0);
                asm volatile("s_waitcnt lgkmcnt(0)" ::: "memory");
                __builtin_amdgcn_sched_barrier(0);
                advance4();
                ++c_g;
            };
            int kt = 0;
            for (; kt + 1 < p.nt; kt += 2) { kstep(f0w, f0x, f1w, f1x); kstep(f1w, f1x, f0w, f0x); }
            if (kt < p.nt) kstep(f0w, f0x, f1w, f1x);
        }

        const int mrow0 = m0 + wm * (16 * FMW) + 4 * fg;
        if (p.dbg & 1) {
#pragma unroll
            for (int i = 0; i < 4; ++i)
#pragma unroll
                for (int j = 0; j < FMW; ++j) asm volatile("" :: "v"(acc[i][j]));
            return;
        }
        Q_TL(2);
        const bool interior = (m0 + 32 * FMW <= p.M) && (n0 + 256 <= p.N);
        auto body = [&](auto int_c) {
            constexpr bool INT = decltype(int_c)::value;
            const int ncol4 = n0 + wn * 64 + 4 * fi;
            f32x4 b4 = f32x4{0.f, 0.f, 0.f, 0.f};
            if constexpr (q_has_bias<EPI>()) {
                const bf16x4 bb = *reinterpret_cast<const bf16x4*>(bias_lds + ncol4 * 2);
                b4 = f32x4{(float)bb[0], (float)bb[1], (float)bb[2], (float)bb[3]};
            }
            if constexpr (F32OUT) {
                const bool colok = INT || ncol4 < p.N;
                float* Cf = reinterpret_cast<float*>(p.C);
                if constexpr (INT && Q_EPI_ASM_RESID) {
                    constexpr int D = Q_EPI_DEPTH_RESID;
                    f32x4 r[D][4];
                    const float* rp = p.resid + (long long)mrow0 * p.ldc + ncol4;
                    auto fetch = [&](int f, f32x4 (&dst)[4]) {
#pragma unroll
                        for (int j = 0; j < 4; ++j) q_gload_f32x4(dst[j], rp + (long long)(f * 16 + j) * p.ldc);
                    };
#pragma unroll
                    for (int f = 0; f < D; ++f) fetch(f, r[f]);
                    auto row = [&](auto fc) {
                        constexpr int f = decltype(fc)::value;
                        f32x4 (&rr)[4] = r[f % D];
                        q_wait_regs4<q_epi_younger(f, FMW, D, 4)>(rr[0], rr[1], rr[2], rr[3]);
#pragma unroll
                        for (int j = 0; j < 4; ++j) {
                            const int m = mrow0 + f * 16 + j;
                            f32x4 v = f32x4{acc[0][f][j], acc[1][f][j], acc[2][f][j], acc[3][f][j]} + b4;
                            if (p.drop_t) {
                                const unsigned hrow = drop_row((unsigned)m + p.drop_m0, p.drop_seed);
#pragma unroll
                                for (int e = 0; e < 4; ++e) v[e] = drop_keep(hrow, (unsigned)(ncol4 + e), p.drop_t) ? v[e] * p.inv_keep : 0.f;
                            }
                            v += rr[j];
                            *reinterpret_cast<f32x4*>(Cf + (long long)m * p.ldc + ncol4) = v;
                        }
                        if constexpr (f + D < FMW) fetch(f + D, rr);
                    };
                    row(std::integral_constant<int, 0>{}); row(std::integral_constant<int, 1>{});
                    row(std::integral_constant<int, 2>{}); row(std::integral_constant<int, 3>{});
                    if constexpr (FMW == 8) {
                        row(std::integral_constant<int, 4>{}); row(std::integral_constant<int, 5>{});
                        row(std::integral_constant<int, 6>{}); row(std::integral_constant<int, 7>{});
                    }
                } else {
                    f32x4 r[2][4];
                    auto fetch = [&](int f, f32x4 (&dst)[4]) {
    #pragma unroll
                        for (int j = 0; j < 4; ++j) {
                            int m = mrow0 + f * 16 + j;
                            if (!INT) m = m < p.M ? m : p.M - 1;
                            dst[j] = f32x4{0.f, 0.f, 0.f, 0.f};
                            if (colok) dst[j] = *reinterpret_cast<const f32x4*>(p.resid + (long long)m * p.ldc + ncol4);
                        }
                    };
                    fetch(0, r[0]);
                    fetch(1, r[1]);
    #pragma unroll
                    for (int f = 0; f < FMW; ++f) {
    #pragma unroll
                        for (int j = 0; j < 4; ++j) {
                            const int m = mrow0 + f * 16 + j;
                            f32x4 v = f32x4{acc[0][f][j], acc[1][f][j], acc[2][f][j], acc[3][f][j]} + b4;
                            if (p.drop_t) {
                                const unsigned hrow = drop_row((unsigned)m + p.drop_m0, p.drop_seed);
    #pragma unroll
                                for (int e = 0; e < 4; ++e) v[e] = drop_keep(hrow, (unsigned)(ncol4 + e), p.drop_t) ? v[e] * p.inv_keep : 0.f;
                            }
                            v += r[f & 1][j];
                            if (INT || (m < p.M && colok)) *reinterpret_cast<f32x4*>(Cf + (long long)m * p.ldc + ncol4) = v;
                        }
                        if (f + 2 < FMW) fetch(f + 2, r[f & 1]);
                    }
                }
            } else if constexpr (EPI == VITK_EPI_RESID16) {
                const bool colok = INT || ncol4 < p.N;
                __bf16* Cb = reinterpret_cast<__bf16*>(p.C);
                const __bf16* Rb = reinterpret_cast<const __bf16*>(p.resid);
                bf16x4 r[2][4];
                auto fetch = [&](int f, bf16x4 (&dst)[4]) {
#pragma unroll
                    for (int j = 0; j < 4; ++j) {
                        int m = mrow0 + f * 16 + j;
                        if (!INT) m = m < p.M ? m : p.M - 1;
                        dst[j] = bf16x4{0, 0, 0, 0};
                        if (colok) dst[j] = *reinterpret_cast<const bf16x4*>(Rb + (long long)m * p.ldc + ncol4);
                    }
                };
                fetch(0, r[0]);
                fetch(1, r[1]);
#pragma unroll
                for (int f = 0; f < FMW; ++f) {
#pragma unroll
                    for (int j = 0; j < 4; ++j) {
                        const int m = mrow0 + f * 16 + j;
                        f32x4 v = f32x4{acc[0][f][j], acc[1][f][j], acc[2][f][j], acc[3][f][j]} + b4;
                        const bf16x4 rr = r[f & 1][j];
                        v += f32x4{(float)rr[0], (float)rr[1], (float)rr[2], (float)rr[3]};
                        if (INT || (m < p.M && colok)) store4<__bf16>(Cb + (long long)m * p.ldc + ncol4, v);
                    }
                    if (f + 2 < FMW) fetch(f + 2, r[f & 1]);
                }
            } else {
                const int odd = fi & 1;
                const int ncol8 = n0 + wn * 64 + 8 * (fi >> 1);
                const bool colok = INT || ncol8 < p.N;
                __bf16* Cb = reinterpret_cast<__bf16*>(p.C);
                constexpr bool AUX_IN = q_aux_in<EPI>();
                constexpr bool AUX8 = (EPI == VITK_EPI_MUL_AUX8);
                constexpr bool ASM_PRE = AUX_IN && INT && Q_EPI_ASM_PRE;
                constexpr int DP = ASM_PRE ? Q_EPI_DEPTH_PRE : 2;
                using HPre = std::conditional_t<AUX8, q_u32x2, bf16x8>;
                HPre hpre[DP][2];
                auto fetch_pre = [&](int f, HPre (&dst)[2]) {
#pragma unroll
                    for (int pr = 0; pr < 2; ++pr) {
                        int m = mrow0 + f * 16 + 2 * pr + odd;
                        if constexpr (AUX8) {
                            const unsigned char* a8 = reinterpret_cast<const unsigned char*>(p.aux);
                            if constexpr (ASM_PRE) q_gload_u32x2(dst[pr], a8 + (long long)m * p.ldc + ncol8);
                            else {
                                if (!INT) m = m < p.M ? m : p.M - 1;
                                dst[pr] = q_u32x2{0u, 0u};
                                if (colok) dst[pr] = *reinterpret_cast<const q_u32x2*>(a8 + (long long)m * p.ldc + ncol8);
                            }
                        } else if constexpr (ASM_PRE) q_gload_bf16x8(dst[pr], p.aux + (long long)m * p.ldc + ncol8);
                        else {
                            if (!INT) m = m < p.M ? m : p.M - 1;
                            dst[pr] = bf16x8{0, 0, 0, 0, 0, 0, 0, 0};
                            if (colok) dst[pr] = *reinterpret_cast<const bf16x8*>(p.aux + (long long)m * p.ldc + ncol8);
                        }
                    }
                };
                if constexpr (AUX_IN) {
#pragma unroll
                    for (int f = 0; f < DP; ++f) fetch_pre(f, hpre[f]);
                }
                float cs[8];
#pragma unroll
                for (int e = 0; e < 8; ++e) cs[e] = 0.f;
                auto frow = [&](auto fc) {
                    constexpr int f = decltype(fc)::value;
                    if constexpr (ASM_PRE) q_wait_regs2<q_epi_younger(f, FMW, DP, 2)>(hpre[f % DP][0], hpre[f % DP][1]);
#pragma unroll
                    for (int pr = 0; pr < 2; ++pr) {
                        const int j0 = 2 * pr;
                        const unsigned a0 = q_pack2b<q_has_bias<EPI>()>(acc[0][f][j0], acc[1][f][j0], b4[0], b4[1]);
                        const unsigned a1 = q_pack2b<q_has_bias<EPI>()>(acc[2][f][j0], acc[3][f][j0], b4[2], b4[3]);
                        const unsigned c0 = q_pack2b<q_has_bias<EPI>()>(acc[0][f][j0 + 1], acc[1][f][j0 + 1], b4[0], b4[1]);
                        const unsigned c1 = q_pack2b<q_has_bias<EPI>()>(acc[2][f][j0 + 1], acc[3][f][j0 + 1], b4[2], b4[3]);
                        const unsigned r0 = q_dpp_xor1(odd ? a0 : c0), r1 = q_dpp_xor1(odd ? a1 : c1);
                        const unsigned k0 = odd ? c0 : a0, k1 = odd ? c1 : a1;
                        const q_u32x4 w4 = odd ? q_u32x4{r0, r1, k0, k1} : q_u32x4{k0, k1, r0, r1};
                        const bf16x8 v = __builtin_bit_cast(bf16x8, w4);
                        const int m = mrow0 + f * 16 + j0 + odd;
                        const bool ok = INT || (m < p.M && colok);
                        const long long o = (long long)m * p.ldc + ncol8;
                        if constexpr (EPI == VITK_EPI_NONE || EPI == VITK_EPI_BIAS) {
                            if (ok) *reinterpret_cast<bf16x8*>(Cb + o) = v;
                        } else if constexpr (EPI == VITK_EPI_BIAS_GELU) {
                            if (ok) *reinterpret_cast<bf16x8*>(p.aux + o) = v;
                            bf16x8 g8 = q_narrow8(q_gelu8(q_widen8(v)));
                            if (p.drop_t) {
                                const unsigned hrow = drop_row((unsigned)m + p.drop_m0, p.drop_seed);
#pragma unroll
                                for (int e = 0; e < 8; ++e)
                                    g8[e] = drop_keep(hrow, (unsigned)(ncol8 + e), p.drop_t) ? (__bf16)((float)g8[e] * p.inv_keep) : (__bf16)0.f;
                            }
                            if (ok) *reinterpret_cast<bf16x8*>(Cb + o) = g8;
                        } else if constexpr (EPI == VITK_EPI_BIAS_GELU_DG || EPI == VITK_EPI_BIAS_GELU_DG8) {
                            q_f32x8 gl, dgl;
                            q_gelu_both8(q_widen8(v), gl, dgl);
                            if constexpr (EPI == VITK_EPI_BIAS_GELU_DG8) {
                                if (ok) *reinterpret_cast<q_u32x2*>(reinterpret_cast<unsigned char*>(p.aux) + o) = q_dg_encode8(dgl);
                            } else {
                                if (ok) *reinterpret_cast<bf16x8*>(p.aux + o) = q_narrow8(dgl);
                            }
                            if (ok) *reinterpret_cast<bf16x8*>(Cb + o) = q_narrow8(gl);
                        } else if constexpr (AUX_IN) {
                            q_f32x8 fac;
                            if constexpr (AUX8) fac = q_dg_decode8(hpre[f % DP][pr]);
                            else if constexpr (EPI == VITK_EPI_MUL_AUX) fac = q_widen8(hpre[f % DP][pr]);
                            else fac = q_gelu_grad8(q_widen8(hpre[f % DP][pr]));
                            q_f32x8 g = q_widen8(v) * fac;
                            if (p.drop_t) {
                                const unsigned hrow = drop_row((unsigned)m + p.drop_m0, p.drop_seed);
#pragma unroll
                                for (int e = 0; e < 8; ++e) g[e] *= drop_keep(hrow, (unsigned)(ncol8 + e), p.drop_t) ? p.inv_keep : 0.f;
                            }
                            const bf16x8 g8 = q_narrow8(g);
                            if (ok) {
                                *reinterpret_cast<bf16x8*>(Cb + o) = g8;
                                q_cs_add8(cs, g8);
                            }
                        }
                    }
                    if constexpr (AUX_IN) {
                        if constexpr (f + DP < FMW) fetch_pre(f + DP, hpre[f % DP]);
                    }
                };
                frow(std::integral_constant<int, 0>{}); frow(std::integral_constant<int, 1>{});
                frow(std::integral_constant<int, 2>{}); frow(std::integral_constant<int, 3>{});
                if constexpr (FMW == 8) {
                    frow(std::integral_constant<int, 4>{}); frow(std::integral_constant<int, 5>{});
                    frow(std::integral_constant<int, 6>{}); frow(std::integral_constant<int, 7>{});
                }
                if constexpr (AUX_IN) {
                    if (p.csum) {
#pragma unroll
                        for (int e = 0; e < 8; ++e) {
                            float v = cs[e];
                            v += __builtin_bit_cast(float, q_dpp_xor1(__builtin_bit_cast(unsigned, v)));
                            unsigned u = __builtin_bit_cast(unsigned, v);
                            auto a = __builtin_amdgcn_permlane16_swap(u, u, false, false);
                            v = __builtin_bit_cast(float, (unsigned)a[0]) + __builtin_bit_cast(float, (unsigned)a[1]);
                            u = __builtin_bit_cast(unsigned, v);
                            auto b = __builtin_amdgcn_permlane32_swap(u, u, false, false);
                            cs[e] = __builtin_bit_cast(float, (unsigned)b[0]) + __builtin_bit_cast(float, (unsigned)b[1]);
                        }
                        if (fg == 0 && !odd && colok) {
                            float* cp = p.csum + (long long)(2 * mt + wm) * p.N + ncol8;
                            *reinterpret_cast<f32x4*>(cp) = f32x4{cs[0], cs[1], cs[2], cs[3]};
                            *reinterpret_cast<f32x4*>(cp + 4) = f32x4{cs[4], cs[5], cs[6], cs[7]};
                        }
                    }
                }
            }
        };
        if (interior) body(std::integral_constant<bool, true>{});
        else body(std::integral_constant<bool, false>{});
        Q_TL(3);
    };

    if (dyn) {
        if (wave == 0) {
            int t0, t1;
            const unsigned v = q_satomic_add(p.tickets + xcd * Q_TK_LINE, 2u);
            if ((int)v + 1 < count) { t0 = (xcd << 24) | (int)v; t1 = t0 + 1; }
            else if ((int)v < count) { t0 = (xcd << 24) | (int)v; t1 = pop_ticket(); }
            else { t0 = pop_ticket(); t1 = t0 >= 0 ? pop_ticket() : -1; }
            if (lane == 0) { tk_slots[0] = t0; tk_slots[1] = t1; }
        }
        __syncthreads();
        p_idx = next_ticket(0);
        if (p_idx < 0) { leave(); return; }
    }
    setup_src(p_idx);
    issue4(); advance4(); issue4(); advance4(); issue4(); advance4(); issue4(); advance4();
    q_wait_vm<12>();
    QQ_BARRIER();

    if (dyn) {
        int n = 0;
        for (int cur = next_ticket(0); cur >= 0; cur = next_ticket(++n)) {
            int m0, half, n0, mt;
            decode(cur, m0, half, n0, mt);
            if (half) run_tile(std::integral_constant<int, 4>{}, m0, n0, mt);
            else run_tile(std::integral_constant<int, 8>{}, m0, n0, mt);
            if (wave == 0) {
                const int t = pop_ticket();
                if (lane == 0) tk_slots[(n + 2) & 3] = t;
            }
        }
        leave();
    } else {
        for (int idx = l0; idx < count; idx += L) {
            int m0, half, n0, mt;
            decode(idx, m0, half, n0, mt);
            if (half) run_tile(std::integral_constant<int, 4>{}, m0, n0, mt);
            else run_tile(std::integral_constant<int, 8>{}, m0, n0, mt);
        }
    }
    q_wait_vm<0>();
#ifdef Q_TIMELINE
    if (tl_on) {
        p.stamps[0] = tl_n;
        for (int i = 0; i < tl_n; ++i) p.stamps[1 + i] = (long long)tl[i];
    }
#endif
}

__device__ unsigned q_ticket_pool[64 * Q_TK_SLOT_WORDS];
unsigned* q_ticket_slot(hipStream_t st) {
    static std::mutex mu;
    static unsigned* bases[64] = {};
    static std::atomic<unsigned> seq{0};
    int dev = 0;
    if (hipGetDevice(&dev) != hipSuccess || dev < 0 || dev >= 64) return nullptr;
    unsigned* base;
    {
        std::lock_guard<std::mutex> g(mu);
        if (!bases[dev]) {
            void* ptr = nullptr;
            if (hipGetSymbolAddress(&ptr, HIP_SYMBOL(q_ticket_pool)) != hipSuccess) return nullptr;
            bases[dev] = (unsigned*)ptr;
        }
        base = bases[dev];
    }
    (void)st;
    return base + (seq.fetch_add(1) & 63) * Q_TK_SLOT_WORDS;
}

template <typename Kern>
int q_set_max_lds(Kern kernel, int bytes) {
    return (int)hipFuncSetAttribute(reinterpret_cast<const void*>(kernel), hipFuncAttributeMaxDynamicSharedMemorySize, bytes);
}

int q_num_cus() {
    static const int n = [] {
        int dev = 0, v = 0;
        if (hipGetDevice(&dev) != hipSuccess) return 256;
        if (hipDeviceGetAttribute(&v, hipDeviceAttributeMultiprocessorCount, dev) != hipSuccess || v < 8) return 256;
        return v;
    }();
    return n;
}

long long q_makespan(int n_main, int n_tail, int L, long long c_full, long long c_half) {
    long long worst = 0;
    for (int x = 0; x < 8; ++x) {
        const int cm = (int)(((long long)(x + 1) * n_main) >> 3) - (int)(((long long)x * n_main) >> 3);
        const int ct = (int)(((long long)(x + 1) * n_tail) >> 3) - (int)(((long long)x * n_tail) >> 3);
        const int cnt = cm + ct;
        for (int l = 0; l < L && l < cnt; ++l) {
            const int nall = (cnt - l + L - 1) / L;
            const int nm = l < cm ? (cm - l + L - 1) / L : 0;
            const long long c = nm * c_full + (nall - nm) * c_half;
            if (c > worst) worst = c;
        }
    }
    return worst;
}

}

NtpPlan ntp_plan(int64_t M, int64_t N, int64_t K, int64_t ldc, const void* aux) {
    NtpPlan pl{};
    pl.ok = (K % 32 == 0) && M >= 1024 && N >= 256 && (N % 8 == 0) && (ldc % 8 == 0) && (!aux || aligned16(aux)) &&
            M < (1 << 30) && N <= 16128  && !vitk_exp("VITK_NO_PERSIST");
    if (!pl.ok) return pl;
    struct Key { int64_t m, n, k; bool operator==(const Key& o) const { return m == o.m && n == o.n && k == o.k; } };
    struct KeyHash { size_t operator()(const Key& k) const { return (size_t)(k.m * 1000003 + k.n * 10007 + k.k); } };
    static std::mutex mu;
    static std::unordered_map<Key, NtpPlan, KeyHash> cache;
    const Key key{M, N, K};
    {
        std::lock_guard<std::mutex> g(mu);
        auto it = cache.find(key);
        if (it != cache.end()) return it->second;
    }
    pl.tiles_n = (int)((N + 255) / 256);
    pl.group_n = pl.tiles_n;
    if (pl.tiles_n > 8) pl.group_n = (pl.tiles_n + (pl.tiles_n + 5) / 6 - 1) / ((pl.tiles_n + 5) / 6);
    if (vitk_exp("VITK_GROUP_N")) pl.group_n = atoi(vitk_exp("VITK_GROUP_N")) > 0 ? atoi(vitk_exp("VITK_GROUP_N")) : pl.tiles_n;
    if (pl.group_n > pl.tiles_n) pl.group_n = pl.tiles_n;
    pl.nt = (int)(K / 32);
    pl.grid = q_num_cus() / 8 * 8;
    const int L = pl.grid / 8;
    const long long e_full = vitk_exp("VITK_NTP_EFULL") ? atoll(vitk_exp("VITK_NTP_EFULL")) : 16;
    const long long e_half = vitk_exp("VITK_NTP_EHALF") ? atoll(vitk_exp("VITK_NTP_EHALF")) : 12;
    const long long c_full = 4LL * pl.nt + e_full, c_half = 2LL * pl.nt + e_half;
    const int full_tm = (int)(M / 256);
    int best_tm = (int)((M + 255) / 256), best_tail = 0;
    long long best = q_makespan(best_tm * pl.tiles_n, 0, L, c_full, c_half);
    const int dmax = full_tm < 512 ? full_tm : 512;
    for (int d = 0; d <= dmax; ++d) {
        const int tm_main = full_tm - d;
        const int64_t rows_tail = M - 256LL * tm_main;
        if (rows_tail <= 0) continue;
        const int tail_tm = (int)((rows_tail + 127) / 128);
        const long long c = q_makespan(tm_main * pl.tiles_n, tail_tm * pl.tiles_n, L, c_full, c_half);
        if (c < best) { best = c; best_tm = tm_main; best_tail = tail_tm; }
    }
    if (vitk_exp("VITK_NTP_TAIL")) {
        const int d = atoi(vitk_exp("VITK_NTP_TAIL"));
        if (d < 0) { best_tm = (int)((M + 255) / 256); best_tail = 0; }
        else {
            best_tm = full_tm - d < 0 ? 0 : full_tm - d;
            best_tail = (int)((M - 256LL * best_tm + 127) / 128);
        }
    }
    pl.tm_main = best_tm;
    pl.tail_tm = best_tail;
    pl.n_main = pl.tm_main * pl.tiles_n;
    pl.n_tail = pl.tail_tm * pl.tiles_n;
    {
        std::lock_guard<std::mutex> g(mu);
        cache.emplace(key, pl);
    }
    return pl;
}

int gemm_ntp_launch(const NtpPlan& pl, const void* A, int64_t lda, const void* W, int64_t ldw, void* C, int64_t ldc, int64_t M,
                    int64_t N, int64_t K, int epilogue, const void* bias, const float* resid, void* aux, float* csum, unsigned drop_t,
                    unsigned drop_seed, float inv_keep, void* stream, unsigned drop_m0) {
    NtpArgs a;
    a.drop_t = drop_t; a.drop_seed = drop_seed; a.inv_keep = inv_keep; a.drop_m0 = drop_m0;
    a.A = (const char*)A; a.lda = lda; a.W = (const char*)W; a.ldw = ldw; a.C = C; a.ldc = ldc;
    a.M = (int)M; a.N = (int)N; a.K = (int)K;
    a.bias = (const __bf16*)bias; a.resid = resid; a.aux = (__bf16*)aux; a.csum = csum;
    a.tiles_n = pl.tiles_n; a.group_n = pl.group_n; a.tm_main = pl.tm_main; a.tail_tm = pl.tail_tm;
    a.n_main = pl.n_main; a.n_tail = pl.n_tail; a.nt = pl.nt;
    static const int tail_env = vitk_exp("VITK_NTP_TAIL_LAST") ? (atoi(vitk_exp("VITK_NTP_TAIL_LAST")) ? 0 : 1) : -1;
    a.tail_first = tail_env >= 0 ? tail_env : ((epilogue == VITK_EPI_BIAS_GELU || epilogue == VITK_EPI_BIAS_GELU_DG || epilogue == VITK_EPI_BIAS_GELU_DG8) ? 0 : 1);
    const char* st_env = vitk_switch("VITK_NTP_STATIC");
    const char* dy_env = vitk_switch("VITK_NTP_DYNAMIC");
    const bool want_dyn = (dy_env && dy_env[0] == '1') || vitk_get_cu_reserve() > 0;
    a.tickets = (pl.nt >= 8 && want_dyn && !(st_env && st_env[0] == '1')) ? q_ticket_slot((hipStream_t)stream) : nullptr;
    if (a.tickets) a.tail_first = vitk_exp("VITK_NTP_DYN_ORDER") ? atoi(vitk_exp("VITK_NTP_DYN_ORDER")) : 0;
    a.dbg = vitk_exp("VITK_NTP_DBG") ? atoi(vitk_exp("VITK_NTP_DBG")) : 0;
    a.stamps = vitk_exp("VITK_NTP_STAMPS") ? (long long*)strtoull(vitk_exp("VITK_NTP_STAMPS"), nullptr, 0) : nullptr;
#ifdef Q_TIMELINE
    const int lds_bytes = Q_LDS_MAX;
#else
    const int lds_bytes = Q_LDS_BYTES + pl.tiles_n * 512 + 16;
#endif
    hipStream_t st = (hipStream_t)stream;
#define NTP_LAUNCH1(E, Dn) do { \
            static const int rc__ = q_set_max_lds(gemm_ntp_kernel<E, Dn>, Q_LDS_MAX); \
            if (rc__ != 0) VITK_FAIL(rc__, "gemm_nt_bf16: cannot enable %d B of LDS", Q_LDS_MAX); \
            hipLaunchKernelGGL((gemm_ntp_kernel<E, Dn>), dim3((unsigned)pl.grid), dim3(512), lds_bytes, st, a); \
        } while (0)
#define NTP_LAUNCH(E) do { \
        if (a.tickets) NTP_LAUNCH1(E, true); \
        else NTP_LAUNCH1(E, false); \
    } while (0)
    switch (epilogue) {
        case VITK_EPI_NONE: NTP_LAUNCH(VITK_EPI_NONE); break;
        case VITK_EPI_BIAS: NTP_LAUNCH(VITK_EPI_BIAS); break;
        case VITK_EPI_BIAS_GELU: NTP_LAUNCH(VITK_EPI_BIAS_GELU); break;
        case VITK_EPI_RESID: NTP_LAUNCH(VITK_EPI_RESID); break;
        case VITK_EPI_GELU_BWD: NTP_LAUNCH(VITK_EPI_GELU_BWD); break;
        case VITK_EPI_BIAS_GELU_DG: NTP_LAUNCH(VITK_EPI_BIAS_GELU_DG); break;
        case VITK_EPI_MUL_AUX: NTP_LAUNCH(VITK_EPI_MUL_AUX); break;
        case VITK_EPI_BIAS_GELU_DG8: NTP_LAUNCH(VITK_EPI_BIAS_GELU_DG8); break;
        case VITK_EPI_MUL_AUX8: NTP_LAUNCH(VITK_EPI_MUL_AUX8); break;
        case VITK_EPI_RESID16: NTP_LAUNCH(VITK_EPI_RESID16); break;
        default: VITK_FAIL(VITK_E_ARG, "gemm_nt_bf16: bad epilogue %d", epilogue);
    }
#undef NTP_LAUNCH
#undef NTP_LAUNCH1
    VITK_CHECK_LAUNCH("gemm_nt_bf16 (persistent)");
    return 0;
}

namespace {
__device__ __forceinline__ void pack_w_chunk(const __bf16* __restrict__ W, long long ldw, int N, int K, char* __restrict__ out, bool TR, long long chunk) {
    const int rows = TR ? K : N, red = TR ? N : K;
    const int nt = red >> 5;
    const long long total = (long long)((rows + 255) >> 8) * nt * 1024;
    if (chunk >= total) return;
    const int spos = (int)(chunk & 3), R = (int)((chunk >> 2) & 255);
    const long long blk = chunk >> 10;
    const int kt = (int)(blk % nt), tn = (int)(blk / nt);
    int n = tn * 256 + (R >> 6) * 64 + 4 * (R & 15) + ((R >> 4) & 3);
    n = n < rows ? n : rows - 1;
    const int k0 = kt * 32 + 8 * (spos ^ q_swz(R >> 2));
    bf16x8 v;
    if (!TR) v = *reinterpret_cast<const bf16x8*>(W + (long long)n * ldw + k0);
    else {
#pragma unroll
        for (int e = 0; e < 8; ++e) v[e] = W[(long long)(k0 + e) * ldw + n];
    }
    *reinterpret_cast<bf16x8*>(out + chunk * 16) = v;
}
template <bool TR>
__global__ __launch_bounds__(256) void pack_w_kernel(const __bf16* __restrict__ W, long long ldw, int N, int K, char* __restrict__ out) {
    pack_w_chunk(W, ldw, N, K, out, TR, (long long)blockIdx.x * 256 + threadIdx.x);
}
}

namespace {
constexpr int PM_MAX = 96;
struct PackMany { const __bf16* W[PM_MAX]; char* out[PM_MAX]; int ldw[PM_MAX], N[PM_MAX], K[PM_MAX]; int blk0[PM_MAX + 1]; int count; unsigned tr[PM_MAX / 32]; };
__global__ __launch_bounds__(256) void pack_w_many_kernel(PackMany a) {
    int lo = 0, hi = a.count;
    while (hi - lo > 1) { const int mid = (lo + hi) >> 1; if ((int)blockIdx.x >= a.blk0[mid]) lo = mid; else hi = mid; }
    const bool tr = (a.tr[lo >> 5] >> (lo & 31)) & 1u;
    pack_w_chunk(a.W[lo], a.ldw[lo], a.N[lo], a.K[lo], a.out[lo], tr, (long long)((int)blockIdx.x - a.blk0[lo]) * 256 + threadIdx.x);
}
}

extern "C" int64_t vitk_pack_w_nt_bytes(int64_t rows, int64_t red) {
    if (rows <= 0 || red <= 0 || (red & 31)) return 0;
    return ((rows + 255) / 256) * 256 * red * 2;
}

extern "C" int vitk_pack_w_nt(const void* W, int64_t ldw, int64_t N, int64_t K, void* out, void* out_t, void* stream) {
    if (!W || (!out && !out_t)) VITK_FAIL(VITK_E_ARG, "pack_w_nt: null pointer");
    if (N <= 0 || K <= 0 || ldw < K || (ldw & 7) || N > (1 << 24) || K > (1 << 24)) VITK_FAIL(VITK_E_SHAPE, "pack_w_nt: bad shape N=%lld K=%lld ldw=%lld", (long long)N, (long long)K, (long long)ldw);
    if ((out && (K & 31)) || (out_t && (N & 31))) VITK_FAIL(VITK_E_SHAPE, "pack_w_nt: the reduction dimension must be a multiple of 32");
    if (!aligned16(W) || (out && !aligned16(out)) || (out_t && !aligned16(out_t))) VITK_FAIL(VITK_E_ALIGN, "pack_w_nt: 16-byte aligned pointers required");
    hipStream_t st = (hipStream_t)stream;
    if (out) {
        const long long chunks = vitk_pack_w_nt_bytes(N, K) / 16;
        hipLaunchKernelGGL((pack_w_kernel<false>), dim3((unsigned)((chunks + 255) / 256)), dim3(256), 0, st, (const __bf16*)W, (long long)ldw, (int)N, (int)K, (char*)out);
    }
    if (out_t) {
        const long long chunks = vitk_pack_w_nt_bytes(K, N) / 16;
        hipLaunchKernelGGL((pack_w_kernel<true>), dim3((unsigned)((chunks + 255) / 256)), dim3(256), 0, st, (const __bf16*)W, (long long)ldw, (int)N, (int)K, (char*)out_t);
    }
    VITK_CHECK_LAUNCH("pack_w_nt");
    return 0;
}

extern "C" int vitk_pack_w_nt_many(const void* const* W, const int64_t* ldw, const int64_t* N, const int64_t* K, void* const* out,
                                   void* const* out_t, int64_t count, void* stream) {
    if (count <= 0) return 0;
    if (!W || !ldw || !N || !K || !out || !out_t) VITK_FAIL(VITK_E_ARG, "pack_w_nt_many: null table");
    hipStream_t st = (hipStream_t)stream;
    PackMany a;
    a.count = 0; a.blk0[0] = 0;
    for (int i = 0; i < PM_MAX / 32; ++i) a.tr[i] = 0u;
    auto flush = [&]() -> int {
        if (a.count == 0) return 0;
        hipLaunchKernelGGL(pack_w_many_kernel, dim3((unsigned)a.blk0[a.count]), dim3(256), 0, st, a);
        VITK_CHECK_LAUNCH("pack_w_nt_many");
        a.count = 0; a.blk0[0] = 0;
        for (int i = 0; i < PM_MAX / 32; ++i) a.tr[i] = 0u;
        return 0;
    };
    for (int64_t t = 0; t < count; ++t) {
        if (!W[t] || (!out[t] && !out_t[t])) VITK_FAIL(VITK_E_ARG, "pack_w_nt_many: null pointer in row %lld", (long long)t);
        if (N[t] <= 0 || K[t] <= 0 || ldw[t] < K[t] || (ldw[t] & 7) || N[t] > (1 << 24) || K[t] > (1 << 24))
            VITK_FAIL(VITK_E_SHAPE, "pack_w_nt_many: bad shape N=%lld K=%lld ldw=%lld", (long long)N[t], (long long)K[t], (long long)ldw[t]);
        if ((out[t] && (K[t] & 31)) || (out_t[t] && (N[t] & 31))) VITK_FAIL(VITK_E_SHAPE, "pack_w_nt_many: the reduction dimension must be a multiple of 32");
        if (!aligned16(W[t]) || (out[t] && !aligned16(out[t])) || (out_t[t] && !aligned16(out_t[t]))) VITK_FAIL(VITK_E_ALIGN, "pack_w_nt_many: 16-byte aligned pointers required");
        for (int tr = 0; tr < 2; ++tr) {
            void* o = tr ? out_t[t] : out[t];
            if (!o) continue;
            const long long chunks = (tr ? vitk_pack_w_nt_bytes(K[t], N[t]) : vitk_pack_w_nt_bytes(N[t], K[t])) / 16;
            const long long blocks = (chunks + 255) / 256;
            if (a.count == PM_MAX || a.blk0[a.count] + blocks > 0x3fffffff) { if (int rc = flush()) return rc; }
            const int j = a.count;
            a.W[j] = (const __bf16*)W[t]; a.out[j] = (char*)o; a.ldw[j] = (int)ldw[t]; a.N[j] = (int)N[t]; a.K[j] = (int)K[t];
            if (tr) a.tr[j >> 5] |= 1u << (j & 31);
            a.blk0[j + 1] = a.blk0[j] + (int)blocks;
            ++a.count;
        }
    }
    return flush();
}
```

### vit_pytorch_amd/csrc/gemm_nt_plan.h

```cpp
#pragma once
#include <stdint.h>

struct NtpPlan {
    bool ok;
    int tiles_n;
    int group_n;
    int tm_main;
    int tail_tm;
    int n_main, n_tail;
    int nt;
    int grid;
};

NtpPlan ntp_plan(int64_t M, int64_t N, int64_t K, int64_t ldc, const void* aux);
static inline int64_t ntp_colsum_rows(const NtpPlan& pl) { return 2 * ((int64_t)pl.tm_main + pl.tail_tm); }

int gemm_ntp_launch(const NtpPlan& pl, const void* A, int64_t lda, const void* W, int64_t ldw, void* C, int64_t ldc, int64_t M,
                    int64_t N, int64_t K, int epilogue, const void* bias, const float* resid, void* aux, float* csum, unsigned drop_t, unsigned drop_seed,
                    float inv_keep, void* stream, unsigned drop_m0 = 0);

bool gemm_ntw_serves(int64_t M, int64_t N, int64_t K);
int gemm_ntw_split(int64_t M, int64_t N, int64_t K, int grid);
int gemm_ntw_launch(int tiles_m, int grid, const void* A, int64_t lda, const void* W, int64_t ldw, void* C, int64_t ldc,
                    int64_t N, int64_t K, int epilogue, const void* bias, const void* resid, void* aux, float* csum, int abl, int dbg, void* stream);
```

### vit_pytorch_amd/csrc/gemm_nt_w128.hip

```cpp
#include "common.h"
#include "gemm_nt_plan.h"
#include "gemm_nt_epi.h"
#include <stdlib.h>
#include <type_traits>

#ifdef VITK_HALF_IS_F16
#define NTW_MFMA_ASM "v_mfma_f32_16x16x32_f16"
#else
#define NTW_MFMA_ASM "v_mfma_f32_16x16x32_bf16"
#endif

namespace {

constexpr int V_TILE = 256 * 64;
constexpr int V_STAGE = 2 * V_TILE;
constexpr int V_RING = 4 * V_STAGE;
constexpr int V_LDS_MAX = V_RING + 32768;
constexpr int X_ASLOT = 256 * 128;
constexpr int X_WBASE = 3 * X_ASLOT;
constexpr int X_LDS = X_WBASE + 4 * V_TILE;

#define V_PIN() __builtin_amdgcn_sched_barrier(0)

__device__ __forceinline__ int v_swz(int x) { return (0x1320 >> (4 * (x & 3))) & 3; }

__device__ __forceinline__ void v_grouped_tile(int t, int tiles_m, int tiles_n, int gn, int& tm, int& tn) {
    const int per_group = gn * tiles_m;
    const int g = t / per_group;
    const int r = t - g * per_group;
    const int rem = tiles_n - g * gn;
    const int w = rem < gn ? rem : gn;
    tm = r / w;
    tn = g * gn + (r - tm * w);
}

struct NtwArgs {
    const char* A; long long lda;
    const char* W; long long ldw;
    void* C; long long ldc;
    int M, N, K;
    const __bf16* bias; const void* resid; __bf16* aux; float* csum;
    int tiles_n, group_n, tiles_m, n_tiles, nt;
    int dbg;
};

template <int OFF> __device__ __forceinline__ bf16x8 v_rd(unsigned lds_addr) {
    bf16x8 v;
    asm volatile("ds_read_b128 %0, %1 offset:%2" : "=v"(v) : "v"(lds_addr), "n"(OFF) : "memory");
    return v;
}
#ifdef NTW_PROBE
typedef float v_f32x16 __attribute__((ext_vector_type(16)));
#ifdef VITK_HALF_IS_F16
#define NTW_MFMA32_ASM "v_mfma_f32_32x32x16_f16"
#else
#define NTW_MFMA32_ASM "v_mfma_f32_32x32x16_bf16"
#endif
__device__ __forceinline__ void v_mfma32(v_f32x16& c, const bf16x8& a, const bf16x8& b) {
    asm volatile("" NTW_MFMA32_ASM " %0, %1, %2, %0" : "+a"(c) : "v"(a), "v"(b));
}
#endif
template <bool Z> __device__ __forceinline__ void v_mfma(f32x4& c, const bf16x8& a, const bf16x8& b) {
    if constexpr (Z) asm volatile("" NTW_MFMA_ASM " %0, %1, %2, 0" : "=a"(c) : "v"(a), "v"(b));
    else asm volatile("" NTW_MFMA_ASM " %0, %1, %2, %0" : "+a"(c) : "v"(a), "v"(b));
}

__device__ __forceinline__ void v_gload_bf16x4(bf16x4& d, const __bf16* p) { asm volatile("global_load_dwordx2 %0, %1, off" : "=v"(d) : "v"(p) : "memory"); }

template <int EPI, int ABL, int AW>
__global__ __launch_bounds__(256) void gemm_ntw_kernel(const NtwArgs p) {
    extern __shared__ __attribute__((aligned(16))) char lds[];
    constexpr bool F32OUT = (EPI == VITK_EPI_RESID);
    const int tid = threadIdx.x;
    const int lane = tid & 63;
    const int wave = __builtin_amdgcn_readfirstlane(tid >> 6);
    const int wm = wave >> 1, wn = wave & 1;

    const int xcd = blockIdx.x & 7, l0 = blockIdx.x >> 3, L = gridDim.x >> 3;
    const int ms = (int)(((long long)xcd * p.n_tiles) >> 3), count = (int)(((long long)(xcd + 1) * p.n_tiles) >> 3) - ms;
    if (l0 >= count) return;
    if ((p.dbg >> 8) && (l0 & 1)) { for (int i = (p.dbg >> 8) & 0xff; i > 0; --i) __builtin_amdgcn_s_sleep(127); }
    auto decode = [&](int idx, int& m0, int& n0, int& mt) {
        int tn;
        v_grouped_tile(ms + idx, p.tiles_m, p.tiles_n, p.group_n, mt, tn);
        m0 = mt * 256; n0 = tn * 256;
    };

    const int srow = lane >> 2, spos = lane & 3;
    const int schunk = spos ^ v_swz(lane >> 4);
    int avo[4], wvo[4];
#pragma unroll
    for (int j = 0; j < 4; ++j) {
        if constexpr (AW) avo[j] = (int)(((long long)(64 * wave + (lane >> 3)) * p.lda + (((lane & 7) ^ (4 * (j & 1) + (lane >> 4))) * 8)) * 2);
        else avo[j] = (int)(((long long)(64 * wave + 16 * j + srow) * p.lda + schunk * 8) * 2);
        wvo[j] = p.ldw == 0 ? (4 * wave + j) * 1024 + lane * 16 : (int)(((long long)(64 * wave + 4 * srow + j) * p.ldw + schunk * 8) * 2);
    }
    const int a_rows8 = (int)(p.lda * 16);
    const int w_kstride = p.ldw == 0 ? V_TILE : 64;
    __amdgpu_buffer_rsrc_t a_rs, w_rs;
    int a_so = 0, w_so = 0;
    auto setup_a = [&](int idx) __attribute__((always_inline)) {
        if (idx < count) {
            int m0, n0, mt;
            decode(idx, m0, n0, mt);
            const long long abytes = (255LL * p.lda + p.K) * 2;
            a_rs = __builtin_amdgcn_make_buffer_rsrc((void*)(p.A + (long long)m0 * p.lda * 2), 0, (int)abytes, 0x00020000);
        } else a_rs = __builtin_amdgcn_make_buffer_rsrc((void*)p.A, 0, 0, 0x00020000);
        a_so = 0;
    };
    auto setup_w = [&](int idx) __attribute__((always_inline)) {
        if (idx < count) {
            int m0, n0, mt;
            decode(idx, m0, n0, mt);
            if (p.ldw == 0) {
                w_rs = __builtin_amdgcn_make_buffer_rsrc((void*)(p.W + (long long)(n0 >> 8) * p.nt * V_TILE), 0, p.nt * V_TILE, 0x00020000);
            } else {
                const long long wbytes = (255LL * p.ldw + p.K) * 2;
                w_rs = __builtin_amdgcn_make_buffer_rsrc((void*)(p.W + (long long)n0 * p.ldw * 2), 0, (int)wbytes, 0x00020000);
            }
        } else w_rs = __builtin_amdgcn_make_buffer_rsrc((void*)p.W, 0, 0, 0x00020000);
        w_so = 0;
    };
    auto setup_src = [&](int idx) { setup_a(idx); setup_w(idx); };
    auto dma = [&](int stg, int q) __attribute__((always_inline)) {
        char* dst = lds + stg * V_STAGE + (q >= 4 ? V_TILE : 0) + (wave * 4 + (q & 3)) * 1024;
        if (q < 4) __builtin_amdgcn_raw_ptr_buffer_load_lds(a_rs, (void __attribute__((address_space(3)))*)dst, 16, avo[q & 3], a_so, 0, 0);
        else __builtin_amdgcn_raw_ptr_buffer_load_lds(w_rs, (void __attribute__((address_space(3)))*)dst, 16, wvo[q & 3], w_so, 0, 0);
    };
    auto advance = [&]() __attribute__((always_inline)) { a_so += 64; w_so += w_kstride; };
    auto next_src = [&](int idx) __attribute__((always_inline)) { setup_src(idx); };
    auto dma_a = [&](int slot, int i) __attribute__((always_inline)) {
        char* dst = lds + slot * X_ASLOT + (wave * 8 + i) * 1024;
        __builtin_amdgcn_raw_ptr_buffer_load_lds(a_rs, (void __attribute__((address_space(3)))*)dst, 16, avo[i & 1], a_so + i * a_rows8, 0, 0);
    };
    auto dma_w = [&](int stg, int j) __attribute__((always_inline)) {
        char* dst = lds + X_WBASE + stg * V_TILE + (wave * 4 + j) * 1024;
        __builtin_amdgcn_raw_ptr_buffer_load_lds(w_rs, (void __attribute__((address_space(3)))*)dst, 16, wvo[j], w_so, 0, 0);
    };

    const char* bias_lds = lds + V_RING;
    if constexpr (q_has_bias<EPI>() && !AW) {
        const int ncols = p.tiles_n * 256;
        for (int i = tid * 8; i < ncols; i += 256 * 8) {
            bf16x8 v = bf16x8{0, 0, 0, 0, 0, 0, 0, 0};
            if (p.bias && i < p.N) v = *reinterpret_cast<const bf16x8*>(p.bias + i);
            *reinterpret_cast<bf16x8*>(lds + V_RING + i * 2) = v;
        }
        asm volatile("s_waitcnt lgkmcnt(0)" ::: "memory");
    }

    const unsigned lds_base = (unsigned)(uintptr_t)((__attribute__((address_space(3))) char*)lds);
    unsigned a_rd, w_rd;
    unsigned a_rd1 = 0;
    {
        const int fi = lane & 15, fg = lane >> 4;
        const int fpos = fg ^ v_swz(fi >> 2);
        if constexpr (AW) {
            const int xpos = fg ^ ((fi >> 1) & 7);
            a_rd = lds_base + (wm * 128 + fi) * 128 + xpos * 16;
            a_rd1 = lds_base + (wm * 128 + fi) * 128 + (xpos ^ 4) * 16;
            w_rd = lds_base + X_WBASE + (wn * 128 + fi) * 64 + fpos * 16;
        } else {
            a_rd = lds_base + (wm * 128 + fi) * 64 + fpos * 16;
            w_rd = lds_base + V_TILE + (wn * 128 + fi) * 64 + fpos * 16;
        }
    }
    constexpr int A_FRAG = AW ? 2048 : 1024;
    int sp = 0;

    int stg = 0;
    bf16x8 xa[8], wa[8], xb[8], wb[8];
    f32x4 acc[8][8];
#ifdef NTW_PROBE
    v_f32x16 acc32[16];
    if constexpr (ABL & 8) {
#pragma unroll
        for (int i = 0; i < 16; ++i) acc32[i] = v_f32x16{0.f, 0.f, 0.f, 0.f, 0.f, 0.f, 0.f, 0.f, 0.f, 0.f, 0.f, 0.f, 0.f, 0.f, 0.f, 0.f};
    }
#endif

#ifdef NTW_PROBE
#define V_MFMA32(G, I_, XC, WC) do { if constexpr (!(ABL & 4) && (ABL & 8)) v_mfma32(acc32[(2 * (G) + (I_)) & 15], XC[(G) >> 1], WC[((G) & 1) * 4 + (I_)]); } while (0)
#else
#define V_MFMA32(G, I_, XC, WC) do { } while (0)
#endif
#define V_GROUP(G, Z, XC, WC, XN, WN) do { \
        constexpr int fm_ = (G) >> 1, h_ = ((G) & 1) * 4; \
        if constexpr (!(ABL & 4) && !(ABL & 8)) v_mfma<Z>(acc[h_ + 0][fm_], XC[fm_], WC[h_ + 0]); \
        V_MFMA32(G, 0, XC, WC); \
        if constexpr (!(ABL & 2)) { if constexpr ((G) < 8) XN[(G)] = v_rd<(G) * A_FRAG>(rdA); else WN[(G) - 8] = v_rd<((G) - 8) * 1024>(rdW); } \
        if constexpr (!(ABL & 4) && !(ABL & 8)) v_mfma<Z>(acc[h_ + 1][fm_], XC[fm_], WC[h_ + 1]); \
        if constexpr (!(ABL & 4) && !(ABL & 8)) v_mfma<Z>(acc[h_ + 2][fm_], XC[fm_], WC[h_ + 2]); \
        if constexpr (!(ABL & 1) && ((G) & 1)) { V_PIN(); if constexpr (AW) { if constexpr ((G) < 8) dma_a(dslot_, di0_ + ((G) >> 1)); else dma_w(stg, ((G) >> 1) - 4); } else dma(stg, (G) >> 1); V_PIN(); } \
        V_MFMA32(G, 1, XC, WC); \
        if constexpr (!(ABL & 4) && !(ABL & 8)) v_mfma<Z>(acc[h_ + 3][fm_], XC[fm_], WC[h_ + 3]); \
    } while (0)
#define V_STEP(Z, XC, WC, XN, WN, WAIT, H) do { \
        const unsigned soff_ = ((stg + 1) & 3) * (AW ? V_TILE : V_STAGE); \
        const int sp1_ = sp == 2 ? 0 : sp + 1; \
        const int dslot_ = (H) ? sp : (sp == 0 ? 2 : sp - 1); \
        constexpr int di0_ = (H) ? 0 : 4; \
        const unsigned rdA = AW ? ((H) ? a_rd + sp1_ * X_ASLOT : a_rd1 + sp * X_ASLOT) : a_rd + soff_; \
        const unsigned rdW = w_rd + soff_; \
        __builtin_amdgcn_s_setprio(1); \
        V_GROUP(0, Z, XC, WC, XN, WN); V_GROUP(1, Z, XC, WC, XN, WN); V_GROUP(2, Z, XC, WC, XN, WN); V_GROUP(3, Z, XC, WC, XN, WN); \
        V_GROUP(4, Z, XC, WC, XN, WN); V_GROUP(5, Z, XC, WC, XN, WN); V_GROUP(6, Z, XC, WC, XN, WN); V_GROUP(7, Z, XC, WC, XN, WN); \
        V_GROUP(8, Z, XC, WC, XN, WN); V_GROUP(9, Z, XC, WC, XN, WN); V_GROUP(10, Z, XC, WC, XN, WN); V_GROUP(11, Z, XC, WC, XN, WN); \
        V_GROUP(12, Z, XC, WC, XN, WN); V_GROUP(13, Z, XC, WC, XN, WN); V_GROUP(14, Z, XC, WC, XN, WN); V_GROUP(15, Z, XC, WC, XN, WN); \
        __builtin_amdgcn_s_setprio(0); \
        asm volatile("s_waitcnt lgkmcnt(0)" ::: "memory");       \
        if constexpr (!(ABL & 1)) { WAIT; } \
        V_PIN(); \
        __builtin_amdgcn_s_barrier();            \
        V_PIN(); \
        if constexpr (!(ABL & 1)) { if constexpr (AW) { w_so += w_kstride; if constexpr (!(H)) a_so += 128; } else advance(); } \
        if constexpr (AW && (H)) sp = sp1_; \
        stg = (stg + 1) & 3; \
    } while (0)
#define V_WAIT16 asm volatile("s_waitcnt vmcnt(16)" ::: "memory")
    bf16x4 bq[2] = {bf16x4{0, 0, 0, 0}, bf16x4{0, 0, 0, 0}};
    auto epilogue = [&](int m0, int n0, int mt) __attribute__((always_inline)) {
        constexpr int NR = 16;
#ifdef NTW_PROBE
        if constexpr (ABL & 8) {
#pragma unroll
            for (int i = 0; i < 16; ++i) asm volatile("" :: "a"(acc32[i]));
            return;
        }
#endif
        if (p.dbg & 1) {
#pragma unroll
            for (int i = 0; i < 8; ++i)
#pragma unroll
                for (int j = 0; j < 8; ++j) asm volatile("" :: "a"(acc[i][j]));
            return;
        }
        int elane;
        asm volatile("v_mbcnt_lo_u32_b32 %0, -1, 0\n\tv_mbcnt_hi_u32_b32 %0, -1, %0" : "=v"(elane));
        int fi = elane & 15, fg = elane >> 4, ewm = wm, ewn = wn;
        asm volatile("" : "+v"(fi), "+v"(fg), "+s"(ewm), "+s"(ewn));
        const int mrow0 = m0 + ewm * 128 + 4 * fg;
        const int ncolw = n0 + ewn * 128;
        const long long obase4 = (long long)mrow0 * p.ldc + ncolw + 4 * fi;
        f32x4 b4[2] = {f32x4{0.f, 0.f, 0.f, 0.f}, f32x4{0.f, 0.f, 0.f, 0.f}};
        if constexpr (q_has_bias<EPI>()) {
            if constexpr (AW) asm volatile("" : "+v"(bq[0]), "+v"(bq[1]));
#pragma unroll
            for (int qq = 0; qq < 2; ++qq) {
                bf16x4 bb;
                if constexpr (AW) bb = bq[qq];
                else bb = *reinterpret_cast<const bf16x4*>(bias_lds + (ncolw + qq * 64 + 4 * fi) * 2);
                b4[qq] = f32x4{(float)bb[0], (float)bb[1], (float)bb[2], (float)bb[3]};
            }
        }
        if constexpr (F32OUT) {
            float* Cf = reinterpret_cast<float*>(p.C);
            const float* Rf = reinterpret_cast<const float*>(p.resid);
            constexpr int D = 4;
            f32x4 r[D][4];
            auto fetch = [&](int rr_, f32x4 (&dst)[4]) __attribute__((always_inline)) {
                const int f = rr_ >> 1, qq = rr_ & 1;
                long long orow = obase4 + (long long)(f * 16) * p.ldc + qq * 64;
                asm volatile("" : "+v"(orow));
                const float* rp = Rf + orow;
#pragma unroll
                for (int j = 0; j < 4; ++j) q_gload_f32x4(dst[j], rp + (long long)j * p.ldc);
            };
#pragma unroll
            for (int i = 0; i < D; ++i) fetch(i, r[i]);
            auto row = [&](auto rc) __attribute__((always_inline)) {
                constexpr int R_ = decltype(rc)::value;
                constexpr int f = R_ >> 1, qq = R_ & 1;
                V_PIN();
                asm volatile("" : "+a"(acc[4 * qq + 0][f]), "+a"(acc[4 * qq + 1][f]), "+a"(acc[4 * qq + 2][f]), "+a"(acc[4 * qq + 3][f]));
                f32x4 (&rr)[4] = r[R_ % D];
                q_wait_regs4<q_epi_younger(R_, NR, D, 4)>(rr[0], rr[1], rr[2], rr[3]);
                long long ocp = obase4 + (long long)(f * 16) * p.ldc + qq * 64;
                asm volatile("" : "+v"(ocp));
                float* cp = Cf + ocp;
#pragma unroll
                for (int j = 0; j < 4; ++j) {
                    f32x4 v = f32x4{acc[4 * qq + 0][f][j], acc[4 * qq + 1][f][j], acc[4 * qq + 2][f][j], acc[4 * qq + 3][f][j]} + b4[qq];
                    v += rr[j];
                    *reinterpret_cast<f32x4*>(cp + (long long)j * p.ldc) = v;
                }
                if constexpr (R_ + D < NR) fetch(R_ + D, rr);
            };
            row(std::integral_constant<int, 0>{}); row(std::integral_constant<int, 1>{}); row(std::integral_constant<int, 2>{}); row(std::integral_constant<int, 3>{});
            row(std::integral_constant<int, 4>{}); row(std::integral_constant<int, 5>{}); row(std::integral_constant<int, 6>{}); row(std::integral_constant<int, 7>{});
            row(std::integral_constant<int, 8>{}); row(std::integral_constant<int, 9>{}); row(std::integral_constant<int, 10>{}); row(std::integral_constant<int, 11>{});
            row(std::integral_constant<int, 12>{}); row(std::integral_constant<int, 13>{}); row(std::integral_constant<int, 14>{}); row(std::integral_constant<int, 15>{});
        } else if constexpr (EPI == VITK_EPI_RESID16) {
            __bf16* Cb = reinterpret_cast<__bf16*>(p.C);
            const __bf16* Rb = reinterpret_cast<const __bf16*>(p.resid);
            constexpr int D = 6;
            bf16x4 r[D][4];
            auto fetch = [&](int rr_, bf16x4 (&dst)[4]) __attribute__((always_inline)) {
                const int f = rr_ >> 1, qq = rr_ & 1;
                long long orow = obase4 + (long long)(f * 16) * p.ldc + qq * 64;
                asm volatile("" : "+v"(orow));
                const __bf16* rp = Rb + orow;
#pragma unroll
                for (int j = 0; j < 4; ++j) v_gload_bf16x4(dst[j], rp + (long long)j * p.ldc);
            };
#pragma unroll
            for (int i = 0; i < D; ++i) fetch(i, r[i]);
            auto row = [&](auto rc) __attribute__((always_inline)) {
                constexpr int R_ = decltype(rc)::value;
                constexpr int f = R_ >> 1, qq = R_ & 1;
                V_PIN();
                asm volatile("" : "+a"(acc[4 * qq + 0][f]), "+a"(acc[4 * qq + 1][f]), "+a"(acc[4 * qq + 2][f]), "+a"(acc[4 * qq + 3][f]));
                bf16x4 (&rr)[4] = r[R_ % D];
                q_wait_regs4<q_epi_younger(R_, NR, D, 4)>(rr[0], rr[1], rr[2], rr[3]);
                long long ocp = obase4 + (long long)(f * 16) * p.ldc + qq * 64;
                asm volatile("" : "+v"(ocp));
                __bf16* cp = Cb + ocp;
#pragma unroll
                for (int j = 0; j < 4; ++j) {
                    f32x4 v = f32x4{acc[4 * qq + 0][f][j], acc[4 * qq + 1][f][j], acc[4 * qq + 2][f][j], acc[4 * qq + 3][f][j]} + b4[qq];
                    const bf16x4 q4 = rr[j];
                    v += f32x4{(float)q4[0], (float)q4[1], (float)q4[2], (float)q4[3]};
                    store4<__bf16>(cp + (long long)j * p.ldc, v);
                }
                if constexpr (R_ + D < NR) fetch(R_ + D, rr);
            };
            row(std::integral_constant<int, 0>{}); row(std::integral_constant<int, 1>{}); row(std::integral_constant<int, 2>{}); row(std::integral_constant<int, 3>{});
            row(std::integral_constant<int, 4>{}); row(std::integral_constant<int, 5>{}); row(std::integral_constant<int, 6>{}); row(std::integral_constant<int, 7>{});
            row(std::integral_constant<int, 8>{}); row(std::integral_constant<int, 9>{}); row(std::integral_constant<int, 10>{}); row(std::integral_constant<int, 11>{});
            row(std::integral_constant<int, 12>{}); row(std::integral_constant<int, 13>{}); row(std::integral_constant<int, 14>{}); row(std::integral_constant<int, 15>{});
        } else {
            const int odd = fi & 1;
            __bf16* Cb = reinterpret_cast<__bf16*>(p.C);
            const long long obase = (long long)(mrow0 + odd) * p.ldc + ncolw + 8 * (fi >> 1);
            constexpr bool AUX_IN = q_aux_in<EPI>();
            constexpr bool AUX8 = (EPI == VITK_EPI_MUL_AUX8);
            constexpr int DP = AUX8 ? 4 : 6;
            using HPre = std::conditional_t<AUX8, q_u32x2, bf16x8>;
            HPre hpre[DP][2];
            auto fetch_pre = [&](int rr_, HPre (&dst)[2]) __attribute__((always_inline)) {
                const int f = rr_ >> 1, qq = rr_ & 1;
                long long oa = obase + (long long)(f * 16) * p.ldc + qq * 64;
                asm volatile("" : "+v"(oa));
#pragma unroll
                for (int pr = 0; pr < 2; ++pr) {
                    if constexpr (AUX8) q_gload_u32x2(dst[pr], reinterpret_cast<const unsigned char*>(p.aux) + oa + (long long)(2 * pr) * p.ldc);
                    else q_gload_bf16x8(dst[pr], p.aux + oa + (long long)(2 * pr) * p.ldc);
                }
            };
            if constexpr (AUX_IN) {
#pragma unroll
                for (int i = 0; i < DP; ++i) fetch_pre(i, hpre[i]);
            }
            float cs[2][8];
#pragma unroll
            for (int e = 0; e < 8; ++e) { cs[0][e] = 0.f; cs[1][e] = 0.f; }
            auto frow = [&](auto rc) __attribute__((always_inline)) {
                constexpr int R_ = decltype(rc)::value;
                constexpr int f = R_ >> 1, qq = R_ & 1;
                V_PIN();
                asm volatile("" : "+a"(acc[4 * qq + 0][f]), "+a"(acc[4 * qq + 1][f]), "+a"(acc[4 * qq + 2][f]), "+a"(acc[4 * qq + 3][f]));
                if constexpr (AUX_IN) q_wait_regs2<q_epi_younger(R_, NR, DP, 2)>(hpre[R_ % DP][0], hpre[R_ % DP][1]);
                long long o0 = obase + (long long)(f * 16) * p.ldc + qq * 64;
                asm volatile("" : "+v"(o0));
#pragma unroll
                for (int pr = 0; pr < 2; ++pr) {
                    const int j0 = 2 * pr;
                    const f32x4 bq = b4[qq];
                    const unsigned a0 = q_pack2b<q_has_bias<EPI>()>(acc[4 * qq + 0][f][j0], acc[4 * qq + 1][f][j0], bq[0], bq[1]);
                    const unsigned a1 = q_pack2b<q_has_bias<EPI>()>(acc[4 * qq + 2][f][j0], acc[4 * qq + 3][f][j0], bq[2], bq[3]);
                    const unsigned c0 = q_pack2b<q_has_bias<EPI>()>(acc[4 * qq + 0][f][j0 + 1], acc[4 * qq + 1][f][j0 + 1], bq[0], bq[1]);
                    const unsigned c1 = q_pack2b<q_has_bias<EPI>()>(acc[4 * qq + 2][f][j0 + 1], acc[4 * qq + 3][f][j0 + 1], bq[2], bq[3]);
                    const unsigned r0 = q_dpp_xor1(odd ? a0 : c0), r1 = q_dpp_xor1(odd ? a1 : c1);
                    const unsigned k0 = odd ? c0 : a0, k1 = odd ? c1 : a1;
                    const q_u32x4 w4 = odd ? q_u32x4{r0, r1, k0, k1} : q_u32x4{k0, k1, r0, r1};
                    const bf16x8 v = __builtin_bit_cast(bf16x8, w4);
                    const long long o = o0 + (long long)j0 * p.ldc;
                    if constexpr (EPI == VITK_EPI_NONE || EPI == VITK_EPI_BIAS) {
                        *reinterpret_cast<bf16x8*>(Cb + o) = v;
                    } else if constexpr (EPI == VITK_EPI_BIAS_GELU) {
                        *reinterpret_cast<bf16x8*>(p.aux + o) = v;
                        *reinterpret_cast<bf16x8*>(Cb + o) = q_narrow8(q_gelu8(q_widen8(v)));
                    } else if constexpr (EPI == VITK_EPI_BIAS_GELU_DG || EPI == VITK_EPI_BIAS_GELU_DG8) {
                        q_f32x8 gl, dgl;
#ifdef NTW_PROBE
                        if (p.dbg & 32) { gl = q_widen8(v); dgl = gl; } else
#endif
                        q_gelu_both8(q_widen8(v), gl, dgl);
#ifdef NTW_PROBE
                        if (p.dbg & 64) { const bf16x8 t0 = q_narrow8(gl); const q_u32x2 t1 = q_dg_encode8(dgl); asm volatile("" :: "v"(t0), "v"(t1)); continue; }
#endif
                        if constexpr (EPI == VITK_EPI_BIAS_GELU_DG8) *reinterpret_cast<q_u32x2*>(reinterpret_cast<unsigned char*>(p.aux) + o) = q_dg_encode8(dgl);
                        else *reinterpret_cast<bf16x8*>(p.aux + o) = q_narrow8(dgl);
                        *reinterpret_cast<bf16x8*>(Cb + o) = q_narrow8(gl);
                    } else if constexpr (AUX_IN) {
                        q_f32x8 fac;
                        if constexpr (AUX8) fac = q_dg_decode8(hpre[R_ % DP][pr]);
                        else if constexpr (EPI == VITK_EPI_MUL_AUX) fac = q_widen8(hpre[R_ % DP][pr]);
                        else fac = q_gelu_grad8(q_widen8(hpre[R_ % DP][pr]));
                        const q_f32x8 g = q_widen8(v) * fac;
                        const bf16x8 g8 = q_narrow8(g);
#ifdef NTW_PROBE
                        if (p.dbg & 64) asm volatile("" :: "v"(g8)); else
#endif
                        *reinterpret_cast<bf16x8*>(Cb + o) = g8;
                        q_cs_add8(cs[qq], g8);
                    }
                }
                if constexpr (AUX_IN) {
                    if constexpr (R_ + DP < NR) fetch_pre(R_ + DP, hpre[R_ % DP]);
                }
            };
            frow(std::integral_constant<int, 0>{}); frow(std::integral_constant<int, 1>{}); frow(std::integral_constant<int, 2>{}); frow(std::integral_constant<int, 3>{});
            frow(std::integral_constant<int, 4>{}); frow(std::integral_constant<int, 5>{}); frow(std::integral_constant<int, 6>{}); frow(std::integral_constant<int, 7>{});
            frow(std::integral_constant<int, 8>{}); frow(std::integral_constant<int, 9>{}); frow(std::integral_constant<int, 10>{}); frow(std::integral_constant<int, 11>{});
            frow(std::integral_constant<int, 12>{}); frow(std::integral_constant<int, 13>{}); frow(std::integral_constant<int, 14>{}); frow(std::integral_constant<int, 15>{});
            if constexpr (AUX_IN) {
                if (p.csum) {
#pragma unroll
                    for (int qq = 0; qq < 2; ++qq) {
#pragma unroll
                        for (int e = 0; e < 8; ++e) {
                            float v = cs[qq][e];
                            v += __builtin_bit_cast(float, q_dpp_xor1(__builtin_bit_cast(unsigned, v)));
                            unsigned u = __builtin_bit_cast(unsigned, v);
                            auto a = __builtin_amdgcn_permlane16_swap(u, u, false, false);
                            v = __builtin_bit_cast(float, (unsigned)a[0]) + __builtin_bit_cast(float, (unsigned)a[1]);
                            u = __builtin_bit_cast(unsigned, v);
                            auto b = __builtin_amdgcn_permlane32_swap(u, u, false, false);
                            cs[qq][e] = __builtin_bit_cast(float, (unsigned)b[0]) + __builtin_bit_cast(float, (unsigned)b[1]);
                        }
                        if (fg == 0 && !odd) {
                            float* cp = p.csum + (long long)(2 * mt + ewm) * p.N + ncolw + qq * 64 + 8 * (fi >> 1);
                            *reinterpret_cast<f32x4*>(cp) = f32x4{cs[qq][0], cs[qq][1], cs[qq][2], cs[qq][3]};
                            *reinterpret_cast<f32x4*>(cp + 4) = f32x4{cs[qq][4], cs[qq][5], cs[qq][6], cs[qq][7]};
                        }
                    }
                }
            }
        }
    };

    setup_src(l0);
    if constexpr (!(ABL & 1)) {
        if constexpr (AW) {
#pragma unroll
            for (int pr = 0; pr < 2; ++pr) {
#pragma unroll
                for (int i = 0; i < 8; ++i) dma_a(pr, i);
                a_so += 128;
#pragma unroll
                for (int k = 0; k < 2; ++k) {
#pragma unroll
                    for (int j = 0; j < 4; ++j) dma_w(2 * pr + k, j);
                    w_so += w_kstride;
                }
            }
#pragma unroll
            for (int i = 0; i < 4; ++i) dma_a(2, i);
            asm volatile("s_waitcnt vmcnt(20)" ::: "memory");
        } else {
#pragma unroll
            for (int s = 0; s < 4; ++s) {
#pragma unroll
                for (int q = 0; q < 8; ++q) dma(s, q);
                advance();
            }
            asm volatile("s_waitcnt vmcnt(16)" ::: "memory");
        }
    }
    V_PIN();
    __builtin_amdgcn_s_barrier();
    V_PIN();
    {
        const unsigned rdA = a_rd, rdW = w_rd;
        xa[0] = v_rd<0 * A_FRAG>(rdA); xa[1] = v_rd<1 * A_FRAG>(rdA); xa[2] = v_rd<2 * A_FRAG>(rdA); xa[3] = v_rd<3 * A_FRAG>(rdA);
        xa[4] = v_rd<4 * A_FRAG>(rdA); xa[5] = v_rd<5 * A_FRAG>(rdA); xa[6] = v_rd<6 * A_FRAG>(rdA); xa[7] = v_rd<7 * A_FRAG>(rdA);
        wa[0] = v_rd<0 * 1024>(rdW); wa[1] = v_rd<1 * 1024>(rdW); wa[2] = v_rd<2 * 1024>(rdW); wa[3] = v_rd<3 * 1024>(rdW);
        wa[4] = v_rd<4 * 1024>(rdW); wa[5] = v_rd<5 * 1024>(rdW); wa[6] = v_rd<6 * 1024>(rdW); wa[7] = v_rd<7 * 1024>(rdW);
        asm volatile("s_waitcnt lgkmcnt(0)" ::: "memory");
    }
    V_PIN();
    __builtin_amdgcn_s_barrier();
    V_PIN();
    if constexpr (ABL & 2) {
#pragma unroll
        for (int f = 0; f < 8; ++f) { xb[f] = xa[f]; wb[f] = wa[f]; }
    }

    constexpr int ST_ROW = (F32OUT || EPI == VITK_EPI_RESID16 || q_two_outputs<EPI>()) ? 4 : 2;
    constexpr int VM_RELAX = 16 + 16 * ST_ROW > 63 ? 63 : 16 + 16 * ST_ROW;
    constexpr bool RELAX_OK = (EPI == VITK_EPI_NONE || (EPI == VITK_EPI_BIAS && !AW));
    bool relax = false;
#define V_WAITR do { \
        if (relax) asm volatile("s_waitcnt vmcnt(%0)" :: "n"(VM_RELAX) : "memory"); \
        else asm volatile("s_waitcnt vmcnt(16)" ::: "memory"); \
    } while (0)

    for (int idx = l0; idx < count; idx += L) {
        int m0, n0, mt;
        decode(idx, m0, n0, mt);
        if constexpr (AW && q_has_bias<EPI>()) {
            if (p.bias) {
                const __bf16* bp = p.bias + n0 + wn * 128 + 4 * (lane & 15);
                v_gload_bf16x4(bq[0], bp);
                v_gload_bf16x4(bq[1], bp + 64);
            }
        }
        V_STEP(true, xa, wa, xb, wb, V_WAITR, 0);
        V_STEP(false, xb, wb, xa, wa, V_WAITR, 1);
        if constexpr (AW) {
            for (int kt = 2; kt + 6 < p.nt; kt += 2) {
                V_STEP(false, xa, wa, xb, wb, V_WAIT16, 0);
                V_STEP(false, xb, wb, xa, wa, V_WAIT16, 1);
            }
            V_STEP(false, xa, wa, xb, wb, V_WAIT16, 0);
            setup_a(idx + L);
            V_STEP(false, xb, wb, xa, wa, V_WAIT16, 1);
            setup_w(idx + L);
            V_STEP(false, xa, wa, xb, wb, V_WAIT16, 0);
            V_STEP(false, xb, wb, xa, wa, V_WAIT16, 1);
            V_STEP(false, xa, wa, xb, wb, V_WAIT16, 0);
            V_STEP(false, xb, wb, xa, wa, V_WAIT16, 1);
        } else {
            for (int kt = 2; kt + 4 < p.nt; kt += 2) {
                V_STEP(false, xa, wa, xb, wb, V_WAIT16, 0);
                V_STEP(false, xb, wb, xa, wa, V_WAIT16, 1);
            }
            next_src(idx + L);
            V_STEP(false, xa, wa, xb, wb, V_WAIT16, 0);
            V_STEP(false, xb, wb, xa, wa, V_WAIT16, 1);
            V_STEP(false, xa, wa, xb, wb, V_WAIT16, 0);
            V_STEP(false, xb, wb, xa, wa, V_WAIT16, 1);
        }
        asm volatile("s_nop 15\n\ts_nop 15" ::: "memory");
        V_PIN();
        epilogue(m0, n0, mt);
        relax = (RELAX_OK || (p.dbg & 16)) && !(p.dbg & 3);
    }
    asm volatile("s_waitcnt vmcnt(0)" ::: "memory");
#undef V_WAITR
#undef V_WAIT16
#undef V_STEP
#undef V_GROUP
#undef V_MFMA32
}

template <typename Kern>
int v_set_max_lds(Kern kernel, int bytes) {
    return (int)hipFuncSetAttribute(reinterpret_cast<const void*>(kernel), hipFuncAttributeMaxDynamicSharedMemorySize, bytes);
}

}

bool gemm_ntw_serves(int64_t M, int64_t N, int64_t K) {
    return !((K % 64) || K < 256 || (N % 256) || M < 256 || N > 16128 || (K / 32) * (long long)V_TILE >= (1LL << 31));
}

int gemm_ntw_split(int64_t M, int64_t N, int64_t K, int grid) {
    const long long tiles_n = N / 256;
    const long long tm_cap = (M % 256 == 0) ? M / 256 : (M - 1024) / 256;
    if (tm_cap <= 0) return 0;
    double second_launch = 14.0 / (0.72 * (double)(K / 32) + 6.0);
    if (const char* e = vitk_exp("VITK_NTW_SPLIT")) second_launch = e[0] == 'r' ? 0.15 : (e[0] == 'n' ? 100.0 : second_launch);
    auto legal = [&](long long tm) { const long long rest = M - 256 * tm; return tm > 0 && tm <= tm_cap && (rest == 0 || rest >= 1024); };
    auto cost = [&](long long tm) -> double {
        const long long rest = M - 256 * tm;
        double c = (double)((tm * tiles_n + grid - 1) / grid);
        if (rest > 0) c += second_launch + 0.6 * (double)((((rest + 127) / 128) * tiles_n + grid - 1) / grid);
        return c;
    };
    long long best_tm = 0;
    double best = 1e30;
    auto consider = [&](long long tm) { if (legal(tm)) { const double c = cost(tm); if (c < best) { best = c; best_tm = tm; } } };
    consider(tm_cap);
    if (M % 256 == 0 && tm_cap > 4) consider(tm_cap - 4);
    const long long k = (tm_cap * tiles_n) / grid;
    if (k >= 1) { long long tm = (k * grid) / tiles_n; consider(tm); while (tm > 0 && !legal(tm)) --tm; consider(tm); }
    if (vitk_exp("VITK_NTW_TM")) { const long long v = atoll(vitk_exp("VITK_NTW_TM")); if (v == 0 || legal(v)) best_tm = v; }
    return (int)best_tm;
}

int gemm_ntw_launch(int tiles_m, int grid, const void* A, int64_t lda, const void* W, int64_t ldw, void* C, int64_t ldc,
                    int64_t N, int64_t K, int epilogue, const void* bias, const void* resid, void* aux, float* csum, int abl, int dbg, void* stream) {
    NtwArgs a;
    a.A = (const char*)A; a.lda = lda; a.W = (const char*)W; a.ldw = ldw; a.C = C; a.ldc = ldc;
    a.M = 256 * tiles_m; a.N = (int)N; a.K = (int)K;
    a.bias = (const __bf16*)bias; a.resid = resid; a.aux = (__bf16*)aux; a.csum = csum;
    a.tiles_n = (int)(N / 256); a.tiles_m = tiles_m; a.n_tiles = a.tiles_m * a.tiles_n; a.nt = (int)(K / 32);
    a.group_n = a.tiles_n;
    if (a.tiles_n > 8) a.group_n = K <= 768 ? 4 : (a.tiles_n + (a.tiles_n + 5) / 6 - 1) / ((a.tiles_n + 5) / 6);
    if (vitk_exp("VITK_GROUP_N")) { const int g = atoi(vitk_exp("VITK_GROUP_N")); a.group_n = g > 0 && g < a.tiles_n ? g : a.tiles_n; }
    a.dbg = dbg;
    if (const char* e = vitk_exp("VITK_NTW_RELAX")) a.dbg |= e[0] == 'a' ? 16 : (e[0] == 'n' ? 2 : 0);
    const int lds_bytes = V_RING + a.tiles_n * 512 + 16;
    hipStream_t st = (hipStream_t)stream;
    if (tiles_m <= 0 || grid < 8) VITK_FAIL(VITK_E_ARG, "gemm_nt_bf16 (w128): nothing to do");
    const char* aw_e = vitk_switch("VITK_NTW_A128");
    const bool a128 = !(aw_e && aw_e[0] == '0');
#define NTW_LAUNCH1(E, AB) do { \
        if (a128) { \
            static const int rc1__ = v_set_max_lds(gemm_ntw_kernel<E, AB, 1>, X_LDS); \
            if (rc1__ != 0) VITK_FAIL(rc1__, "gemm_nt_bf16 (w128): cannot enable %d B of LDS", X_LDS); \
            hipLaunchKernelGGL((gemm_ntw_kernel<E, AB, 1>), dim3((unsigned)grid), dim3(256), X_LDS, st, a); \
        } else { \
            static const int rc__ = v_set_max_lds(gemm_ntw_kernel<E, AB, 0>, V_LDS_MAX); \
            if (rc__ != 0) VITK_FAIL(rc__, "gemm_nt_bf16 (w128): cannot enable %d B of LDS", V_LDS_MAX); \
            hipLaunchKernelGGL((gemm_ntw_kernel<E, AB, 0>), dim3((unsigned)grid), dim3(256), lds_bytes, st, a); \
        } \
    } while (0)
#ifdef NTW_PROBE
#define NTW_LAUNCH_ALL(E) do { \
        switch (abl) { \
            case 0: NTW_LAUNCH1(E, 0); break; case 1: NTW_LAUNCH1(E, 1); break; case 2: NTW_LAUNCH1(E, 2); break; case 3: NTW_LAUNCH1(E, 3); break; \
            case 4: NTW_LAUNCH1(E, 4); break; case 5: NTW_LAUNCH1(E, 5); break; case 6: NTW_LAUNCH1(E, 6); break; case 7: NTW_LAUNCH1(E, 7); break; \
            case 8: NTW_LAUNCH1(E, 8); break; case 10: NTW_LAUNCH1(E, 10); break; case 11: NTW_LAUNCH1(E, 11); break; \
            default: VITK_FAIL(VITK_E_ARG, "gemm_nt_bf16 (w128): bad ablation %d", abl); \
        } } while (0)
#define NTW_LAUNCH(E) do { if (abl == 0) NTW_LAUNCH1(E, 0); else if (abl == 7) NTW_LAUNCH1(E, 7); else VITK_FAIL(VITK_E_ARG, "gemm_nt_bf16 (w128): ablation %d exists for EPI_NONE only", abl); } while (0)
#else
#define NTW_LAUNCH(E) do { if (abl) VITK_FAIL(VITK_E_ARG, "gemm_nt_bf16 (w128): ablations exist in tools/nt_probe.hip only"); NTW_LAUNCH1(E, 0); } while (0)
#define NTW_LAUNCH_ALL(E) NTW_LAUNCH(E)
#endif
    switch (epilogue) {
        case VITK_EPI_NONE: NTW_LAUNCH_ALL(VITK_EPI_NONE); break;
#ifndef NTW_PROBE_LEAN
        case VITK_EPI_BIAS: NTW_LAUNCH(VITK_EPI_BIAS); break;
        case VITK_EPI_BIAS_GELU: NTW_LAUNCH(VITK_EPI_BIAS_GELU); break;
        case VITK_EPI_RESID: NTW_LAUNCH(VITK_EPI_RESID); break;
        case VITK_EPI_GELU_BWD: NTW_LAUNCH(VITK_EPI_GELU_BWD); break;
        case VITK_EPI_BIAS_GELU_DG: NTW_LAUNCH(VITK_EPI_BIAS_GELU_DG); break;
        case VITK_EPI_MUL_AUX: NTW_LAUNCH(VITK_EPI_MUL_AUX); break;
        case VITK_EPI_BIAS_GELU_DG8: NTW_LAUNCH(VITK_EPI_BIAS_GELU_DG8); break;
        case VITK_EPI_MUL_AUX8: NTW_LAUNCH(VITK_EPI_MUL_AUX8); break;
        case VITK_EPI_RESID16: NTW_LAUNCH(VITK_EPI_RESID16); break;
#endif
        default: VITK_FAIL(VITK_E_ARG, "gemm_nt_bf16 (w128): bad epilogue %d", epilogue);
    }
#undef NTW_LAUNCH_ALL
#undef NTW_LAUNCH
#undef NTW_LAUNCH1
    VITK_CHECK_LAUNCH("gemm_nt_bf16 (w128)");
    return 0;
}
```

Measured before the change: 8801.

## Cover GEMM rows with mixed 256-row and 128-row tiles in one persistent launch

Adds a half-height (128-row) tile path to the w128 persistent NT GEMM kernel, so a single launch can cover all of M with full 256-row tiles plus 128-row tail tiles. A makespan model picks how many full tiles to split into halves to balance work across XCDs, and the previous second launch for leftover rows is dropped. It also prefetches the next tile's LDS read bases across the tile boundary. GELU-forward epilogues are excluded. The cost is a more complex kernel with more register pressure, plus a heuristic cost model that could choose a poor split.

```diff
diff --git a/vit_pytorch_amd/csrc/gemm_bf16.hip b/vit_pytorch_amd/csrc/gemm_bf16.hip
--- a/vit_pytorch_amd/csrc/gemm_bf16.hip
+++ b/vit_pytorch_amd/csrc/gemm_bf16.hip
@@ -750,15 +750,24 @@
 }
 
 constexpr unsigned NTW_EPIS = 0xffu;
-static int ntw_tiles_m(const NtpPlan& q, int64_t M, int64_t N, int64_t K, int epilogue, int grid = 0) {
+static bool ntw_takes(const NtpPlan& q, int64_t M, int64_t N, int64_t K, int epilogue) {
     if (epilogue == VITK_EPI_BIAS_GELU_DG8) epilogue = VITK_EPI_BIAS_GELU_DG;
     if (epilogue == VITK_EPI_MUL_AUX8) epilogue = VITK_EPI_MUL_AUX;
     const char* e = vitk_switch("VITK_NT_W128");
     const unsigned mask = e ? (unsigned)strtoul(e, nullptr, 0) : NTW_EPIS;
-    if (!q.ok || !((mask >> epilogue) & 1u) || !gemm_ntw_serves(M, N, K)) return 0;
+    return q.ok && ((mask >> epilogue) & 1u) && gemm_ntw_serves(M, N, K);
+}
+static int ntw_tiles_m(const NtpPlan& q, int64_t M, int64_t N, int64_t K, int epilogue, int grid = 0) {
+    if (!ntw_takes(q, M, N, K, epilogue)) return 0;
     return gemm_ntw_split(M, N, K, grid > 0 ? grid : q.grid);
 }
+static NtwPlan ntw_cover(const NtpPlan& q, int64_t M, int64_t N, int64_t K, int epilogue, int grid) {
+    if (!ntw_takes(q, M, N, K, epilogue) || M % 256) return NtwPlan{0, 0};
+    return gemm_ntw_cover(M, N, K, grid);
+}
 static int64_t nt_persist_colsum_rows(const NtpPlan& q, int64_t M, int64_t N, int64_t K, int64_t ldc) {
+    const NtwPlan cv = ntw_cover(q, M, N, K, VITK_EPI_MUL_AUX, q.grid);
+    if (cv.tm_main + cv.tail_tm > 0) return 2 * (M / 256);
     const int tmw = ntw_tiles_m(q, M, N, K, VITK_EPI_MUL_AUX);
     if (tmw == 0) return ntp_colsum_rows(q);
     const int64_t rest = M - 256LL * tmw;
@@ -770,7 +779,21 @@
     const int reserve = vitk_get_cu_reserve();
     int grid_w = q.grid - (reserve + 7) / 8 * 8;
     if (grid_w < q.grid / 4) grid_w = q.grid / 4 / 8 * 8;
-    const int tmw = ntw_tiles_m(q, M, N, K, epilogue == VITK_EPI_GELU_BWD ? VITK_EPI_MUL_AUX : epilogue, csum ? 0 : grid_w);
+    const int epi_sw = epilogue == VITK_EPI_GELU_BWD ? VITK_EPI_MUL_AUX : epilogue;
+    const bool gelu_fwd = epilogue == VITK_EPI_BIAS_GELU || epilogue == VITK_EPI_BIAS_GELU_DG || epilogue == VITK_EPI_BIAS_GELU_DG8;
+    const NtwPlan cv = gelu_fwd ? NtwPlan{0, 0} : ntw_cover(q, M, N, K, epi_sw, grid_w);
+    if (cv.tm_main + cv.tail_tm > 0) {
+        if (!drop_t) {
+            if (256LL * (lda > ldw ? lda : ldw) * 2 + K * 2 >= (1LL << 31)) VITK_FAIL(VITK_E_SHAPE, "gemm_nt_bf16: row stride too large (lda %lld, ldw %lld)", (long long)lda, (long long)ldw);
+            return gemm_ntw_launch(cv.tm_main, grid_w, A, lda, W, ldw, C, ldc, N, K, epilogue, bias, resid, aux, csum, 0, 0, stream, cv.tail_tm);
+        }
+        if (!(epilogue == VITK_EPI_GELU_BWD && csum))
+            return gemm_ntp_launch(q, A, lda, W, ldw, C, ldc, M, N, K, epilogue, bias, resid, aux, csum, drop_t, drop_seed, inv_keep, stream);
+        NtpPlan q1 = q;
+        q1.tm_main = (int)(M / 256); q1.tail_tm = 0; q1.n_main = q1.tm_main * q1.tiles_n; q1.n_tail = 0;
+        return gemm_ntp_launch(q1, A, lda, W, ldw, C, ldc, M, N, K, epilogue, bias, resid, aux, csum, drop_t, drop_seed, inv_keep, stream);
+    }
+    const int tmw = ntw_tiles_m(q, M, N, K, epi_sw, csum ? 0 : grid_w);
     const int64_t asz = (epilogue == VITK_EPI_BIAS_GELU_DG8 || epilogue == VITK_EPI_MUL_AUX8) ? 1 : 2;
     if (tmw == 0 || (drop_t && !(epilogue == VITK_EPI_GELU_BWD && csum)))
         return gemm_ntp_launch(q, A, lda, W, ldw, C, ldc, M, N, K, epilogue, bias, resid, aux, csum, drop_t, drop_seed, inv_keep, stream);
diff --git a/vit_pytorch_amd/csrc/gemm_nt_persist.hip b/vit_pytorch_amd/csrc/gemm_nt_persist.hip
--- a/vit_pytorch_amd/csrc/gemm_nt_persist.hip
+++ b/vit_pytorch_amd/csrc/gemm_nt_persist.hip
@@ -615,22 +615,6 @@
     return n;
 }
 
-long long q_makespan(int n_main, int n_tail, int L, long long c_full, long long c_half) {
-    long long worst = 0;
-    for (int x = 0; x < 8; ++x) {
-        const int cm = (int)(((long long)(x + 1) * n_main) >> 3) - (int)(((long long)x * n_main) >> 3);
-        const int ct = (int)(((long long)(x + 1) * n_tail) >> 3) - (int)(((long long)x * n_tail) >> 3);
-        const int cnt = cm + ct;
-        for (int l = 0; l < L && l < cnt; ++l) {
-            const int nall = (cnt - l + L - 1) / L;
-            const int nm = l < cm ? (cm - l + L - 1) / L : 0;
-            const long long c = nm * c_full + (nall - nm) * c_half;
-            if (c > worst) worst = c;
-        }
-    }
-    return worst;
-}
-
 }
 
 NtpPlan ntp_plan(int64_t M, int64_t N, int64_t K, int64_t ldc, const void* aux) {
diff --git a/vit_pytorch_amd/csrc/gemm_nt_plan.h b/vit_pytorch_amd/csrc/gemm_nt_plan.h
--- a/vit_pytorch_amd/csrc/gemm_nt_plan.h
+++ b/vit_pytorch_amd/csrc/gemm_nt_plan.h
@@ -19,7 +19,40 @@
                     int64_t N, int64_t K, int epilogue, const void* bias, const float* resid, void* aux, float* csum, unsigned drop_t, unsigned drop_seed,
                     float inv_keep, void* stream, unsigned drop_m0 = 0);
 
+static inline long long q_makespan(int n_main, int n_tail, int L, long long c_full, long long c_half) {
+    long long worst = 0;
+    for (int x = 0; x < 8; ++x) {
+        const int cm = (int)(((long long)(x + 1) * n_main) >> 3) - (int)(((long long)x * n_main) >> 3);
+        const int ct = (int)(((long long)(x + 1) * n_tail) >> 3) - (int)(((long long)x * n_tail) >> 3);
+        const int cnt = cm + ct;
+        for (int l = 0; l < L && l < cnt; ++l) {
+            const int nall = (cnt - l + L - 1) / L;
+            const int nm = l < cm ? (cm - l + L - 1) / L : 0;
+            const long long c = nm * c_full + (nall - nm) * c_half;
+            if (c > worst) worst = c;
+        }
+    }
+    return worst;
+}
+
+struct NtwPlan { int tm_main, tail_tm; };
+constexpr double NTW_HALF_COST = 0.8;
+static inline long long ntw_cost_full_ns(int64_t K) { return (long long)(720.0 * (double)(K / 32) + 6000.0); }
+static inline long long ntw_cost_half_ns(int64_t K) { return (long long)(NTW_HALF_COST * (double)ntw_cost_full_ns(K)); }
+static inline NtwPlan ntw_half_plan(int64_t M, int64_t N, int64_t K, int grid) {
+    const int tiles_n = (int)(N / 256), full_tm = (int)(M / 256), L = grid / 8;
+    const long long cf = ntw_cost_full_ns(K), ch = ntw_cost_half_ns(K);
+    NtwPlan best{full_tm, 0};
+    long long best_c = q_makespan(full_tm * tiles_n, 0, L, cf, ch);
+    for (int d = 1; d <= full_tm; ++d) {
+        const long long c = q_makespan((full_tm - d) * tiles_n, 2 * d * tiles_n, L, cf, ch);
+        if (c < best_c) { best_c = c; best = NtwPlan{full_tm - d, 2 * d}; }
+    }
+    return best;
+}
 bool gemm_ntw_serves(int64_t M, int64_t N, int64_t K);
 int gemm_ntw_split(int64_t M, int64_t N, int64_t K, int grid);
+NtwPlan gemm_ntw_cover(int64_t M, int64_t N, int64_t K, int grid);
 int gemm_ntw_launch(int tiles_m, int grid, const void* A, int64_t lda, const void* W, int64_t ldw, void* C, int64_t ldc,
-                    int64_t N, int64_t K, int epilogue, const void* bias, const void* resid, void* aux, float* csum, int abl, int dbg, void* stream);
+                    int64_t N, int64_t K, int epilogue, const void* bias, const void* resid, void* aux, float* csum, int abl, int dbg, void* stream,
+                    int tail_tm = 0);
diff --git a/vit_pytorch_amd/csrc/gemm_nt_w128.hip b/vit_pytorch_amd/csrc/gemm_nt_w128.hip
--- a/vit_pytorch_amd/csrc/gemm_nt_w128.hip
+++ b/vit_pytorch_amd/csrc/gemm_nt_w128.hip
@@ -2,7 +2,9 @@
 #include "gemm_nt_plan.h"
 #include "gemm_nt_epi.h"
 #include <stdlib.h>
+#include <mutex>
 #include <type_traits>
+#include <unordered_map>
 
 #ifdef VITK_HALF_IS_F16
 #define NTW_MFMA_ASM "v_mfma_f32_16x16x32_f16"
@@ -41,6 +43,7 @@
     int M, N, K;
     const __bf16* bias; const void* resid; __bf16* aux; float* csum;
     int tiles_n, group_n, tiles_m, n_tiles, nt;
+    int tail_tm, n_tail;
     int dbg;
 };
 
@@ -67,9 +70,10 @@
 
 __device__ __forceinline__ void v_gload_bf16x4(bf16x4& d, const __bf16* p) { asm volatile("global_load_dwordx2 %0, %1, off" : "=v"(d) : "v"(p) : "memory"); }
 
-template <int EPI, int ABL, int AW>
-__global__ __launch_bounds__(256) void gemm_ntw_kernel(const NtwArgs p) {
+template <int EPI, int ABL, int AW, bool HT>
+__device__ __forceinline__ void ntw_body(const NtwArgs& p) {
     extern __shared__ __attribute__((aligned(16))) char lds[];
+    constexpr bool HT_ = HT && AW == 1 && ABL == 0;
     constexpr bool F32OUT = (EPI == VITK_EPI_RESID);
     const int tid = threadIdx.x;
     const int lane = tid & 63;
@@ -77,12 +81,21 @@
     const int wm = wave >> 1, wn = wave & 1;
 
     const int xcd = blockIdx.x & 7, l0 = blockIdx.x >> 3, L = gridDim.x >> 3;
-    const int ms = (int)(((long long)xcd * p.n_tiles) >> 3), count = (int)(((long long)(xcd + 1) * p.n_tiles) >> 3) - ms;
+    const int ms = (int)(((long long)xcd * p.n_tiles) >> 3), cm = (int)(((long long)(xcd + 1) * p.n_tiles) >> 3) - ms;
+    const int ts = HT_ ? (int)(((long long)xcd * p.n_tail) >> 3) : 0, ct = HT_ ? (int)(((long long)(xcd + 1) * p.n_tail) >> 3) - ts : 0;
+    const int count = cm + ct, tb = ts - cm;
     if (l0 >= count) return;
     if ((p.dbg >> 8) && (l0 & 1)) { for (int i = (p.dbg >> 8) & 0xff; i > 0; --i) __builtin_amdgcn_s_sleep(127); }
-    auto decode = [&](int idx, int& m0, int& n0, int& mt) {
+    auto decode = [&](int idx, int& m0, int& n0, int& mt, int& hh) {
         int tn;
-        v_grouped_tile(ms + idx, p.tiles_m, p.tiles_n, p.group_n, mt, tn);
+        if (!HT_ || idx < cm) {
+            v_grouped_tile(ms + idx, p.tiles_m, p.tiles_n, p.group_n, mt, tn);
+            hh = -1;
+        } else {
+            int u;
+            v_grouped_tile(tb + idx, p.tail_tm, p.tiles_n, p.group_n, u, tn);
+            mt = p.tiles_m + (u >> 1); hh = u & 1;
+        }
         m0 = mt * 256; n0 = tn * 256;
     };
 
@@ -101,17 +114,18 @@
     int a_so = 0, w_so = 0;
     auto setup_a = [&](int idx) __attribute__((always_inline)) {
         if (idx < count) {
-            int m0, n0, mt;
-            decode(idx, m0, n0, mt);
-            const long long abytes = (255LL * p.lda + p.K) * 2;
-            a_rs = __builtin_amdgcn_make_buffer_rsrc((void*)(p.A + (long long)m0 * p.lda * 2), 0, (int)abytes, 0x00020000);
+            int m0, n0, mt, hh;
+            decode(idx, m0, n0, mt, hh);
+            const long long abytes = ((hh < 0 ? 255LL : 127LL) * p.lda + p.K) * 2;
+            const long long r0 = m0 + (hh > 0 ? 128 : 0);
+            a_rs = __builtin_amdgcn_make_buffer_rsrc((void*)(p.A + r0 * p.lda * 2), 0, (int)abytes, 0x00020000);
         } else a_rs = __builtin_amdgcn_make_buffer_rsrc((void*)p.A, 0, 0, 0x00020000);
         a_so = 0;
     };
     auto setup_w = [&](int idx) __attribute__((always_inline)) {
         if (idx < count) {
-            int m0, n0, mt;
-            decode(idx, m0, n0, mt);
+            int m0, n0, mt, hh;
+            decode(idx, m0, n0, mt, hh);
             if (p.ldw == 0) {
                 w_rs = __builtin_amdgcn_make_buffer_rsrc((void*)(p.W + (long long)(n0 >> 8) * p.nt * V_TILE), 0, p.nt * V_TILE, 0x00020000);
             } else {
@@ -165,6 +179,7 @@
             w_rd = lds_base + V_TILE + (wn * 128 + fi) * 64 + fpos * 16;
         }
     }
+    const int a_hoff = -wm * 16384, w_hoff = (64 * wave - 128 * wn) * 64;
     constexpr int A_FRAG = AW ? 2048 : 1024;
     int sp = 0;
 
@@ -188,25 +203,46 @@
         constexpr int fm_ = (G) >> 1, h_ = ((G) & 1) * 4; \
         if constexpr (!(ABL & 4) && !(ABL & 8)) v_mfma<Z>(acc[h_ + 0][fm_], XC[fm_], WC[h_ + 0]); \
         V_MFMA32(G, 0, XC, WC); \
-        if constexpr (!(ABL & 2)) { if constexpr ((G) < 8) XN[(G)] = v_rd<(G) * A_FRAG>(rdA); else WN[(G) - 8] = v_rd<((G) - 8) * 1024>(rdW); } \
+        if constexpr (!(ABL & 2)) { \
+            if constexpr ((G) < 8) XN[(G)] = v_rd<(G) * A_FRAG>(rdA); \
+            else if constexpr (NX_ && (G) >= 12) WN[(G) - 8] = v_rd<((G) - 12) * 1024>(rdW2); \
+            else WN[(G) - 8] = v_rd<((G) - 8) * 1024>(rdW); } \
         if constexpr (!(ABL & 4) && !(ABL & 8)) v_mfma<Z>(acc[h_ + 1][fm_], XC[fm_], WC[h_ + 1]); \
         if constexpr (!(ABL & 4) && !(ABL & 8)) v_mfma<Z>(acc[h_ + 2][fm_], XC[fm_], WC[h_ + 2]); \
         if constexpr (!(ABL & 1) && ((G) & 1)) { V_PIN(); if constexpr (AW) { if constexpr ((G) < 8) dma_a(dslot_, di0_ + ((G) >> 1)); else dma_w(stg, ((G) >> 1) - 4); } else dma(stg, (G) >> 1); V_PIN(); } \
         V_MFMA32(G, 1, XC, WC); \
         if constexpr (!(ABL & 4) && !(ABL & 8)) v_mfma<Z>(acc[h_ + 3][fm_], XC[fm_], WC[h_ + 3]); \
     } while (0)
-#define V_STEP(Z, XC, WC, XN, WN, WAIT, H) do { \
+#define V_HGROUP(G, Z, XC, WC, XN, WN) do { \
+        v_mfma<Z>(acc[0][(G)], XC[(G)], WC[0]); \
+        XN[(G)] = v_rd<(G) * A_FRAG>(rdA); \
+        v_mfma<Z>(acc[1][(G)], XC[(G)], WC[1]); \
+        if constexpr (!((G) & 1)) WN[(G) >> 1] = v_rd<((G) >> 1) * 1024>(rdW); \
+        else if constexpr (NX_) WN[4 + ((G) >> 1)] = v_rd<((G) >> 1) * 1024>(rdW2); \
+        v_mfma<Z>(acc[2][(G)], XC[(G)], WC[2]); \
+        V_PIN(); if constexpr ((G) < 4) dma_a(dslot_, di0_ + (G)); else dma_w(stg, (G) - 4); V_PIN(); \
+        v_mfma<Z>(acc[3][(G)], XC[(G)], WC[3]); \
+    } while (0)
+#define V_STEP_(Z, XC, WC, XN, WN, WAIT, H, HALF, NX, ARD, ARD1, WRD, WRD2) do { \
         const unsigned soff_ = ((stg + 1) & 3) * (AW ? V_TILE : V_STAGE); \
         const int sp1_ = sp == 2 ? 0 : sp + 1; \
         const int dslot_ = (H) ? sp : (sp == 0 ? 2 : sp - 1); \
         constexpr int di0_ = (H) ? 0 : 4; \
-        const unsigned rdA = AW ? ((H) ? a_rd + sp1_ * X_ASLOT : a_rd1 + sp * X_ASLOT) : a_rd + soff_; \
-        const unsigned rdW = w_rd + soff_; \
+        constexpr bool NX_ = (NX); \
+        const unsigned rdA = AW ? ((H) ? (ARD) + sp1_ * X_ASLOT : (ARD1) + sp * X_ASLOT) : (ARD) + soff_; \
+        const unsigned rdW = (WRD) + soff_; \
+        const unsigned rdW2 = (WRD2) + soff_; \
+        (void)rdW2; \
         __builtin_amdgcn_s_setprio(1); \
-        V_GROUP(0, Z, XC, WC, XN, WN); V_GROUP(1, Z, XC, WC, XN, WN); V_GROUP(2, Z, XC, WC, XN, WN); V_GROUP(3, Z, XC, WC, XN, WN); \
-        V_GROUP(4, Z, XC, WC, XN, WN); V_GROUP(5, Z, XC, WC, XN, WN); V_GROUP(6, Z, XC, WC, XN, WN); V_GROUP(7, Z, XC, WC, XN, WN); \
-        V_GROUP(8, Z, XC, WC, XN, WN); V_GROUP(9, Z, XC, WC, XN, WN); V_GROUP(10, Z, XC, WC, XN, WN); V_GROUP(11, Z, XC, WC, XN, WN); \
-        V_GROUP(12, Z, XC, WC, XN, WN); V_GROUP(13, Z, XC, WC, XN, WN); V_GROUP(14, Z, XC, WC, XN, WN); V_GROUP(15, Z, XC, WC, XN, WN); \
+        if constexpr (HALF) { \
+            V_HGROUP(0, Z, XC, WC, XN, WN); V_HGROUP(1, Z, XC, WC, XN, WN); V_HGROUP(2, Z, XC, WC, XN, WN); V_HGROUP(3, Z, XC, WC, XN, WN); \
+            V_HGROUP(4, Z, XC, WC, XN, WN); V_HGROUP(5, Z, XC, WC, XN, WN); V_HGROUP(6, Z, XC, WC, XN, WN); V_HGROUP(7, Z, XC, WC, XN, WN); \
+        } else { \
+            V_GROUP(0, Z, XC, WC, XN, WN); V_GROUP(1, Z, XC, WC, XN, WN); V_GROUP(2, Z, XC, WC, XN, WN); V_GROUP(3, Z, XC, WC, XN, WN); \
+            V_GROUP(4, Z, XC, WC, XN, WN); V_GROUP(5, Z, XC, WC, XN, WN); V_GROUP(6, Z, XC, WC, XN, WN); V_GROUP(7, Z, XC, WC, XN, WN); \
+            V_GROUP(8, Z, XC, WC, XN, WN); V_GROUP(9, Z, XC, WC, XN, WN); V_GROUP(10, Z, XC, WC, XN, WN); V_GROUP(11, Z, XC, WC, XN, WN); \
+            V_GROUP(12, Z, XC, WC, XN, WN); V_GROUP(13, Z, XC, WC, XN, WN); V_GROUP(14, Z, XC, WC, XN, WN); V_GROUP(15, Z, XC, WC, XN, WN); \
+        } \
         __builtin_amdgcn_s_setprio(0); \
         asm volatile("s_waitcnt lgkmcnt(0)" ::: "memory");       \
         if constexpr (!(ABL & 1)) { WAIT; } \
@@ -217,10 +253,13 @@
         if constexpr (AW && (H)) sp = sp1_; \
         stg = (stg + 1) & 3; \
     } while (0)
+#define V_STEP(Z, XC, WC, XN, WN, WAIT, H) V_STEP_(Z, XC, WC, XN, WN, WAIT, H, false, false, a_rd, a_rd1, w_rd, w_rd)
+#define V_HSTEP(Z, XC, WC, XN, WN, WAIT, H) V_STEP_(Z, XC, WC, XN, WN, WAIT, H, true, false, a_rdh, a_rd1h, w_rdh, w_rdh)
 #define V_WAIT16 asm volatile("s_waitcnt vmcnt(16)" ::: "memory")
     bf16x4 bq[2] = {bf16x4{0, 0, 0, 0}, bf16x4{0, 0, 0, 0}};
-    auto epilogue = [&](int m0, int n0, int mt) __attribute__((always_inline)) {
-        constexpr int NR = 16;
+    auto epilogue = [&](int m0, int n0, int mt, int erow, int ecol, auto qn) __attribute__((always_inline)) {
+        constexpr int QN = decltype(qn)::value;
+        constexpr int NR = 8 * QN;
 #ifdef NTW_PROBE
         if constexpr (ABL & 8) {
 #pragma unroll
@@ -237,16 +276,16 @@
         }
         int elane;
         asm volatile("v_mbcnt_lo_u32_b32 %0, -1, 0\n\tv_mbcnt_hi_u32_b32 %0, -1, %0" : "=v"(elane));
-        int fi = elane & 15, fg = elane >> 4, ewm = wm, ewn = wn;
-        asm volatile("" : "+v"(fi), "+v"(fg), "+s"(ewm), "+s"(ewn));
+        int fi = elane & 15, fg = elane >> 4, ewm = erow, ewc = ecol;
+        asm volatile("" : "+v"(fi), "+v"(fg), "+s"(ewm), "+s"(ewc));
         const int mrow0 = m0 + ewm * 128 + 4 * fg;
-        const int ncolw = n0 + ewn * 128;
+        const int ncolw = n0 + ewc;
         const long long obase4 = (long long)mrow0 * p.ldc + ncolw + 4 * fi;
         f32x4 b4[2] = {f32x4{0.f, 0.f, 0.f, 0.f}, f32x4{0.f, 0.f, 0.f, 0.f}};
         if constexpr (q_has_bias<EPI>()) {
             if constexpr (AW) asm volatile("" : "+v"(bq[0]), "+v"(bq[1]));
 #pragma unroll
-            for (int qq = 0; qq < 2; ++qq) {
+            for (int qq = 0; qq < QN; ++qq) {
                 bf16x4 bb;
                 if constexpr (AW) bb = bq[qq];
                 else bb = *reinterpret_cast<const bf16x4*>(bias_lds + (ncolw + qq * 64 + 4 * fi) * 2);
@@ -259,7 +298,7 @@
             constexpr int D = 4;
             f32x4 r[D][4];
             auto fetch = [&](int rr_, f32x4 (&dst)[4]) __attribute__((always_inline)) {
-                const int f = rr_ >> 1, qq = rr_ & 1;
+                const int f = rr_ / QN, qq = rr_ % QN;
                 long long orow = obase4 + (long long)(f * 16) * p.ldc + qq * 64;
                 asm volatile("" : "+v"(orow));
                 const float* rp = Rf + orow;
@@ -270,7 +309,7 @@
             for (int i = 0; i < D; ++i) fetch(i, r[i]);
             auto row = [&](auto rc) __attribute__((always_inline)) {
                 constexpr int R_ = decltype(rc)::value;
-                constexpr int f = R_ >> 1, qq = R_ & 1;
+                constexpr int f = R_ / QN, qq = R_ % QN;
                 V_PIN();
                 asm volatile("" : "+a"(acc[4 * qq + 0][f]), "+a"(acc[4 * qq + 1][f]), "+a"(acc[4 * qq + 2][f]), "+a"(acc[4 * qq + 3][f]));
                 f32x4 (&rr)[4] = r[R_ % D];
@@ -288,15 +327,17 @@
             };
             row(std::integral_constant<int, 0>{}); row(std::integral_constant<int, 1>{}); row(std::integral_constant<int, 2>{}); row(std::integral_constant<int, 3>{});
             row(std::integral_constant<int, 4>{}); row(std::integral_constant<int, 5>{}); row(std::integral_constant<int, 6>{}); row(std::integral_constant<int, 7>{});
-            row(std::integral_constant<int, 8>{}); row(std::integral_constant<int, 9>{}); row(std::integral_constant<int, 10>{}); row(std::integral_constant<int, 11>{});
-            row(std::integral_constant<int, 12>{}); row(std::integral_constant<int, 13>{}); row(std::integral_constant<int, 14>{}); row(std::integral_constant<int, 15>{});
+            if constexpr (QN == 2) {
+                row(std::integral_constant<int, 8>{}); row(std::integral_constant<int, 9>{}); row(std::integral_constant<int, 10>{}); row(std::integral_constant<int, 11>{});
+                row(std::integral_constant<int, 12>{}); row(std::integral_constant<int, 13>{}); row(std::integral_constant<int, 14>{}); row(std::integral_constant<int, 15>{});
+            }
         } else if constexpr (EPI == VITK_EPI_RESID16) {
             __bf16* Cb = reinterpret_cast<__bf16*>(p.C);
             const __bf16* Rb = reinterpret_cast<const __bf16*>(p.resid);
             constexpr int D = 6;
             bf16x4 r[D][4];
             auto fetch = [&](int rr_, bf16x4 (&dst)[4]) __attribute__((always_inline)) {
-                const int f = rr_ >> 1, qq = rr_ & 1;
+                const int f = rr_ / QN, qq = rr_ % QN;
                 long long orow = obase4 + (long long)(f * 16) * p.ldc + qq * 64;
                 asm volatile("" : "+v"(orow));
                 const __bf16* rp = Rb + orow;
@@ -307,7 +348,7 @@
             for (int i = 0; i < D; ++i) fetch(i, r[i]);
             auto row = [&](auto rc) __attribute__((always_inline)) {
                 constexpr int R_ = decltype(rc)::value;
-                constexpr int f = R_ >> 1, qq = R_ & 1;
+                constexpr int f = R_ / QN, qq = R_ % QN;
                 V_PIN();
                 asm volatile("" : "+a"(acc[4 * qq + 0][f]), "+a"(acc[4 * qq + 1][f]), "+a"(acc[4 * qq + 2][f]), "+a"(acc[4 * qq + 3][f]));
                 bf16x4 (&rr)[4] = r[R_ % D];
@@ -326,8 +367,10 @@
             };
             row(std::integral_constant<int, 0>{}); row(std::integral_constant<int, 1>{}); row(std::integral_constant<int, 2>{}); row(std::integral_constant<int, 3>{});
             row(std::integral_constant<int, 4>{}); row(std::integral_constant<int, 5>{}); row(std::integral_constant<int, 6>{}); row(std::integral_constant<int, 7>{});
-            row(std::integral_constant<int, 8>{}); row(std::integral_constant<int, 9>{}); row(std::integral_constant<int, 10>{}); row(std::integral_constant<int, 11>{});
-            row(std::integral_constant<int, 12>{}); row(std::integral_constant<int, 13>{}); row(std::integral_constant<int, 14>{}); row(std::integral_constant<int, 15>{});
+            if constexpr (QN == 2) {
+                row(std::integral_constant<int, 8>{}); row(std::integral_constant<int, 9>{}); row(std::integral_constant<int, 10>{}); row(std::integral_constant<int, 11>{});
+                row(std::integral_constant<int, 12>{}); row(std::integral_constant<int, 13>{}); row(std::integral_constant<int, 14>{}); row(std::integral_constant<int, 15>{});
+            }
         } else {
             const int odd = fi & 1;
             __bf16* Cb = reinterpret_cast<__bf16*>(p.C);
@@ -338,7 +381,7 @@
             using HPre = std::conditional_t<AUX8, q_u32x2, bf16x8>;
             HPre hpre[DP][2];
             auto fetch_pre = [&](int rr_, HPre (&dst)[2]) __attribute__((always_inline)) {
-                const int f = rr_ >> 1, qq = rr_ & 1;
+                const int f = rr_ / QN, qq = rr_ % QN;
                 long long oa = obase + (long long)(f * 16) * p.ldc + qq * 64;
                 asm volatile("" : "+v"(oa));
 #pragma unroll
@@ -356,7 +399,7 @@
             for (int e = 0; e < 8; ++e) { cs[0][e] = 0.f; cs[1][e] = 0.f; }
             auto frow = [&](auto rc) __attribute__((always_inline)) {
                 constexpr int R_ = decltype(rc)::value;
-                constexpr int f = R_ >> 1, qq = R_ & 1;
+                constexpr int f = R_ / QN, qq = R_ % QN;
                 V_PIN();
                 asm volatile("" : "+a"(acc[4 * qq + 0][f]), "+a"(acc[4 * qq + 1][f]), "+a"(acc[4 * qq + 2][f]), "+a"(acc[4 * qq + 3][f]));
                 if constexpr (AUX_IN) q_wait_regs2<q_epi_younger(R_, NR, DP, 2)>(hpre[R_ % DP][0], hpre[R_ % DP][1]);
@@ -412,12 +455,14 @@
             };
             frow(std::integral_constant<int, 0>{}); frow(std::integral_constant<int, 1>{}); frow(std::integral_constant<int, 2>{}); frow(std::integral_constant<int, 3>{});
             frow(std::integral_constant<int, 4>{}); frow(std::integral_constant<int, 5>{}); frow(std::integral_constant<int, 6>{}); frow(std::integral_constant<int, 7>{});
-            frow(std::integral_constant<int, 8>{}); frow(std::integral_constant<int, 9>{}); frow(std::integral_constant<int, 10>{}); frow(std::integral_constant<int, 11>{});
-            frow(std::integral_constant<int, 12>{}); frow(std::integral_constant<int, 13>{}); frow(std::integral_constant<int, 14>{}); frow(std::integral_constant<int, 15>{});
+            if constexpr (QN == 2) {
+                frow(std::integral_constant<int, 8>{}); frow(std::integral_constant<int, 9>{}); frow(std::integral_constant<int, 10>{}); frow(std::integral_constant<int, 11>{});
+                frow(std::integral_constant<int, 12>{}); frow(std::integral_constant<int, 13>{}); frow(std::integral_constant<int, 14>{}); frow(std::integral_constant<int, 15>{});
+            }
             if constexpr (AUX_IN) {
                 if (p.csum) {
 #pragma unroll
-                    for (int qq = 0; qq < 2; ++qq) {
+                    for (int qq = 0; qq < QN; ++qq) {
 #pragma unroll
                         for (int e = 0; e < 8; ++e) {
                             float v = cs[qq][e];
@@ -472,11 +517,12 @@
     __builtin_amdgcn_s_barrier();
     V_PIN();
     {
-        const unsigned rdA = a_rd, rdW = w_rd;
+        const bool h0 = HT_ && l0 >= cm;
+        const unsigned rdA = a_rd + (h0 ? a_hoff : 0), rdW = w_rd + (h0 ? w_hoff : 0), rdW2 = h0 ? rdW : w_rd + 4096;
         xa[0] = v_rd<0 * A_FRAG>(rdA); xa[1] = v_rd<1 * A_FRAG>(rdA); xa[2] = v_rd<2 * A_FRAG>(rdA); xa[3] = v_rd<3 * A_FRAG>(rdA);
         xa[4] = v_rd<4 * A_FRAG>(rdA); xa[5] = v_rd<5 * A_FRAG>(rdA); xa[6] = v_rd<6 * A_FRAG>(rdA); xa[7] = v_rd<7 * A_FRAG>(rdA);
         wa[0] = v_rd<0 * 1024>(rdW); wa[1] = v_rd<1 * 1024>(rdW); wa[2] = v_rd<2 * 1024>(rdW); wa[3] = v_rd<3 * 1024>(rdW);
-        wa[4] = v_rd<4 * 1024>(rdW); wa[5] = v_rd<5 * 1024>(rdW); wa[6] = v_rd<6 * 1024>(rdW); wa[7] = v_rd<7 * 1024>(rdW);
+        wa[4] = v_rd<0 * 1024>(rdW2); wa[5] = v_rd<1 * 1024>(rdW2); wa[6] = v_rd<2 * 1024>(rdW2); wa[7] = v_rd<3 * 1024>(rdW2);
         asm volatile("s_waitcnt lgkmcnt(0)" ::: "memory");
     }
     V_PIN();
@@ -489,23 +535,67 @@
 
     constexpr int ST_ROW = (F32OUT || EPI == VITK_EPI_RESID16 || q_two_outputs<EPI>()) ? 4 : 2;
     constexpr int VM_RELAX = 16 + 16 * ST_ROW > 63 ? 63 : 16 + 16 * ST_ROW;
+    constexpr int VM_RELAX_H = 16 + 8 * ST_ROW > 63 ? 63 : 16 + 8 * ST_ROW;
     constexpr bool RELAX_OK = (EPI == VITK_EPI_NONE || (EPI == VITK_EPI_BIAS && !AW));
-    bool relax = false;
+    int relax = 0;
 #define V_WAITR do { \
-        if (relax) asm volatile("s_waitcnt vmcnt(%0)" :: "n"(VM_RELAX) : "memory"); \
+        if (relax == 1) asm volatile("s_waitcnt vmcnt(%0)" :: "n"(VM_RELAX) : "memory"); \
+        else if (relax == 2) asm volatile("s_waitcnt vmcnt(%0)" :: "n"(VM_RELAX_H) : "memory"); \
         else asm volatile("s_waitcnt vmcnt(16)" ::: "memory"); \
     } while (0)
 
     for (int idx = l0; idx < count; idx += L) {
-        int m0, n0, mt;
-        decode(idx, m0, n0, mt);
-        if constexpr (AW && q_has_bias<EPI>()) {
-            if (p.bias) {
-                const __bf16* bp = p.bias + n0 + wn * 128 + 4 * (lane & 15);
-                v_gload_bf16x4(bq[0], bp);
-                v_gload_bf16x4(bq[1], bp + 64);
-            }
-        }
+        int m0, n0, mt, hh;
+        decode(idx, m0, n0, mt, hh);
+        const bool half = HT_ && hh >= 0;
+        auto load_bias = [&](bool hf) __attribute__((always_inline)) {
+            if constexpr (AW && q_has_bias<EPI>()) {
+                if (p.bias) {
+                    const __bf16* bp = p.bias + n0 + (hf ? 64 * wave : 128 * wn) + 4 * (lane & 15);
+                    v_gload_bf16x4(bq[0], bp);
+                    v_gload_bf16x4(bq[1], bp + (hf ? 0 : 64));
+                }
+            }
+        };
+        unsigned nA = 0, nW = 0, nW2 = 0;
+        auto next_bases = [&]() __attribute__((always_inline)) {
+            const bool nh = HT_ && idx + L < count && idx + L >= cm;
+            nA = a_rd + (nh ? a_hoff : 0); nW = w_rd + (nh ? w_hoff : 0); nW2 = nh ? nW : w_rd + 4096;
+            asm volatile("" : "+v"(nA), "+v"(nW), "+v"(nW2));
+        };
+        if constexpr (HT_) {
+            if (half) {
+                load_bias(true);
+                unsigned a_rdh = a_rd + a_hoff, a_rd1h = a_rd1 + a_hoff, w_rdh = w_rd + w_hoff;
+                asm volatile("" : "+v"(a_rdh), "+v"(a_rd1h), "+v"(w_rdh));
+                V_HSTEP(true, xa, wa, xb, wb, V_WAITR, 0);
+                V_HSTEP(false, xb, wb, xa, wa, V_WAITR, 1);
+                for (int kt = 2; kt + 6 < p.nt; kt += 2) {
+                    V_HSTEP(false, xa, wa, xb, wb, V_WAIT16, 0);
+                    V_HSTEP(false, xb, wb, xa, wa, V_WAIT16, 1);
+                }
+                V_HSTEP(false, xa, wa, xb, wb, V_WAIT16, 0);
+                setup_a(idx + L);
+                V_HSTEP(false, xb, wb, xa, wa, V_WAIT16, 1);
+                setup_w(idx + L);
+                V_HSTEP(false, xa, wa, xb, wb, V_WAIT16, 0);
+                V_HSTEP(false, xb, wb, xa, wa, V_WAIT16, 1);
+                V_HSTEP(false, xa, wa, xb, wb, V_WAIT16, 0);
+                next_bases();
+                V_STEP_(false, xb, wb, xa, wa, V_WAIT16, 1, true, true, nA, a_rd1h, nW, nW2);
+                asm volatile("s_nop 15\n\ts_nop 15" ::: "memory");
+                V_PIN();
+                {
+                    int ei = idx;
+                    asm volatile("" : "+s"(ei));
+                    decode(ei, m0, n0, mt, hh);
+                }
+                epilogue(m0, n0, mt, hh, 64 * wave, std::integral_constant<int, 1>{});
+                relax = ((RELAX_OK || (p.dbg & 16)) && !(p.dbg & 3)) ? 2 : 0;
+                continue;
+            }
+        }
+        load_bias(false);
         V_STEP(true, xa, wa, xb, wb, V_WAITR, 0);
         V_STEP(false, xb, wb, xa, wa, V_WAITR, 1);
         if constexpr (AW) {
@@ -520,7 +610,8 @@
             V_STEP(false, xa, wa, xb, wb, V_WAIT16, 0);
             V_STEP(false, xb, wb, xa, wa, V_WAIT16, 1);
             V_STEP(false, xa, wa, xb, wb, V_WAIT16, 0);
-            V_STEP(false, xb, wb, xa, wa, V_WAIT16, 1);
+            next_bases();
+            V_STEP_(false, xb, wb, xa, wa, V_WAIT16, 1, false, true, nA, a_rd1, nW, nW2);
         } else {
             for (int kt = 2; kt + 4 < p.nt; kt += 2) {
                 V_STEP(false, xa, wa, xb, wb, V_WAIT16, 0);
@@ -534,15 +625,31 @@
         }
         asm volatile("s_nop 15\n\ts_nop 15" ::: "memory");
         V_PIN();
-        epilogue(m0, n0, mt);
-        relax = (RELAX_OK || (p.dbg & 16)) && !(p.dbg & 3);
+        {
+            int ei = idx;
+            asm volatile("" : "+s"(ei));
+            decode(ei, m0, n0, mt, hh);
+        }
+        epilogue(m0, n0, mt, wm, 128 * wn, std::integral_constant<int, 2>{});
+        relax = ((RELAX_OK || (p.dbg & 16)) && !(p.dbg & 3)) ? 1 : 0;
     }
     asm volatile("s_waitcnt vmcnt(0)" ::: "memory");
 #undef V_WAITR
 #undef V_WAIT16
 #undef V_STEP
+#undef V_HSTEP
+#undef V_STEP_
+#undef V_HGROUP
 #undef V_GROUP
 #undef V_MFMA32
+}
+
+template <int EPI, int ABL, int AW>
+__global__ __launch_bounds__(256) void gemm_ntw_kernel(const NtwArgs p) { ntw_body<EPI, ABL, AW, false>(p); }
+template <int EPI>
+__global__ __launch_bounds__(256) void gemm_ntw_half_kernel(const NtwArgs p) { ntw_body<EPI, 0, 1, true>(p); }
+template <int EPI> constexpr bool ntw_half_epi() {
+    return !(EPI == VITK_EPI_BIAS_GELU || EPI == VITK_EPI_BIAS_GELU_DG || EPI == VITK_EPI_BIAS_GELU_DG8);
 }
 
 template <typename Kern>
@@ -580,13 +687,43 @@
     return (int)best_tm;
 }
 
+static bool ntw_half_on() {
+    const char* e = vitk_switch("VITK_NTW_HALF");
+    return !(e && e[0] == '0');
+}
+static bool ntw_a128_on() {
+    const char* e = vitk_switch("VITK_NTW_A128");
+    return !(e && e[0] == '0');
+}
+
+NtwPlan gemm_ntw_cover(int64_t M, int64_t N, int64_t K, int grid) {
+    if (M % 256 || grid < 8 || !ntw_half_on() || !ntw_a128_on()) return NtwPlan{0, 0};
+    struct Key { int64_t m, n, k; int g; bool operator==(const Key& o) const { return m == o.m && n == o.n && k == o.k && g == o.g; } };
+    struct KeyHash { size_t operator()(const Key& k) const { return (size_t)(k.m * 1000003 + k.n * 10007 + k.k * 101 + k.g); } };
+    static std::mutex mu;
+    static std::unordered_map<Key, NtwPlan, KeyHash> cache;
+    const Key key{M, N, K, grid};
+    if (vitk_exp("VITK_NTW_TAIL")) {
+        const long long d = atoll(vitk_exp("VITK_NTW_TAIL"));
+        if (d >= 0 && d <= M / 256) return NtwPlan{(int)(M / 256 - d), (int)(2 * d)};
+    }
+    std::lock_guard<std::mutex> g(mu);
+    auto it = cache.find(key);
+    if (it != cache.end()) return it->second;
+    const NtwPlan pl = ntw_half_plan(M, N, K, grid);
+    cache.emplace(key, pl);
+    return pl;
+}
+
 int gemm_ntw_launch(int tiles_m, int grid, const void* A, int64_t lda, const void* W, int64_t ldw, void* C, int64_t ldc,
-                    int64_t N, int64_t K, int epilogue, const void* bias, const void* resid, void* aux, float* csum, int abl, int dbg, void* stream) {
+                    int64_t N, int64_t K, int epilogue, const void* bias, const void* resid, void* aux, float* csum, int abl, int dbg, void* stream,
+                    int tail_tm) {
     NtwArgs a;
     a.A = (const char*)A; a.lda = lda; a.W = (const char*)W; a.ldw = ldw; a.C = C; a.ldc = ldc;
-    a.M = 256 * tiles_m; a.N = (int)N; a.K = (int)K;
+    a.M = 256 * tiles_m + 128 * tail_tm; a.N = (int)N; a.K = (int)K;
     a.bias = (const __bf16*)bias; a.resid = resid; a.aux = (__bf16*)aux; a.csum = csum;
     a.tiles_n = (int)(N / 256); a.tiles_m = tiles_m; a.n_tiles = a.tiles_m * a.tiles_n; a.nt = (int)(K / 32);
+    a.tail_tm = tail_tm; a.n_tail = tail_tm * a.tiles_n;
     a.group_n = a.tiles_n;
     if (a.tiles_n > 8) a.group_n = K <= 768 ? 4 : (a.tiles_n + (a.tiles_n + 5) / 6 - 1) / ((a.tiles_n + 5) / 6);
     if (vitk_exp("VITK_GROUP_N")) { const int g = atoi(vitk_exp("VITK_GROUP_N")); a.group_n = g > 0 && g < a.tiles_n ? g : a.tiles_n; }
@@ -594,10 +731,19 @@
     if (const char* e = vitk_exp("VITK_NTW_RELAX")) a.dbg |= e[0] == 'a' ? 16 : (e[0] == 'n' ? 2 : 0);
     const int lds_bytes = V_RING + a.tiles_n * 512 + 16;
     hipStream_t st = (hipStream_t)stream;
-    if (tiles_m <= 0 || grid < 8) VITK_FAIL(VITK_E_ARG, "gemm_nt_bf16 (w128): nothing to do");
-    const char* aw_e = vitk_switch("VITK_NTW_A128");
-    const bool a128 = !(aw_e && aw_e[0] == '0');
+    if (tiles_m < 0 || tail_tm < 0 || tiles_m + tail_tm <= 0 || grid < 8) VITK_FAIL(VITK_E_ARG, "gemm_nt_bf16 (w128): nothing to do");
+    const bool a128 = ntw_a128_on();
+    if (tail_tm > 0 && (!a128 || abl != 0)) VITK_FAIL(VITK_E_ARG, "gemm_nt_bf16 (w128): 128-row tiles need the 128-byte activation feed and no ablation");
 #define NTW_LAUNCH1(E, AB) do { \
+        if constexpr (AB == 0 && ntw_half_epi<E>()) { \
+            if (tail_tm > 0) { \
+                static const int rch__ = v_set_max_lds(gemm_ntw_half_kernel<E>, X_LDS); \
+                if (rch__ != 0) VITK_FAIL(rch__, "gemm_nt_bf16 (w128): cannot enable %d B of LDS", X_LDS); \
+                hipLaunchKernelGGL((gemm_ntw_half_kernel<E>), dim3((unsigned)grid), dim3(256), X_LDS, st, a); \
+                break; \
+            } \
+        } \
+        if (tail_tm > 0) VITK_FAIL(VITK_E_ARG, "gemm_nt_bf16 (w128): no 128-row tiles with epilogue %d", (int)(E)); \
         if (a128) { \
             static const int rc1__ = v_set_max_lds(gemm_ntw_kernel<E, AB, 1>, X_LDS); \
             if (rc1__ != 0) VITK_FAIL(rc1__, "gemm_nt_bf16 (w128): cannot enable %d B of LDS", X_LDS); \
```

After: 8965, median of 6. +1.9%, better.
